# bxlab/bx-python

Measured on AMD Instinct MI355X. Metric: M overlap-queries/s at 100M x 10M intervals (count-only), higher is better.
Workload: dtype int32

## Files before the change

### bx-python_amd/csrc/count_bitmap.hpp

```cpp
#pragma once

namespace bxmi {

constexpr int BM_NB = PT_NB;
constexpr unsigned BM_REC_ESC = 0xFFFFFFFFu;
constexpr int BM_MIN_SHIFT = 5;
constexpr int BM_GROUP_TILES = 64;
constexpr int BM_CHUNK = 65536;
constexpr int BM_HARD = 127;
constexpr int BM_LONG_CAP = 480;

struct BmGeom {
    int32_t cmin;
    int32_t cmax;
    int32_t shift;
    int32_t nce;
    int32_t ncs;
    int32_t stride;
    int32_t f;
    int32_t rshift;
    int32_t dshift;
};

__device__ __forceinline__ unsigned bm_len_esc(const BmGeom &g) { return (1u << (32 - g.rshift)) - 1u; }
// ... 69 lines not shown
    if ((int)threadIdx.x < npar) {
        po.segs[threadIdx.x] = c.seg[threadIdx.x];
        po.totals[threadIdx.x] = c.total[threadIdx.x];
    }
    for (int i = 0; i < npar; i++)
        for (int64_t t = c.seg[i].tile0 + threadIdx.x; t < c.seg[i].tile_end; t += T) po.tile_seg[t] = (unsigned short)i;
}

__global__ __launch_bounds__(256) void bm_params_kernel(BmSegChunk c, int first, BmSeg *__restrict__ segs, unsigned long long **__restrict__ totals,
                                                        unsigned short *__restrict__ tile_seg, unsigned long long *__restrict__ zero_u64, int n_zero,
                                                        int *__restrict__ n_items, unsigned *__restrict__ probe = nullptr,
                                                        unsigned long long *__restrict__ order_host = nullptr, unsigned long long order_seq = 0)
{
    if (first == 0 && blockIdx.x == 0) {
        for (int i = threadIdx.x; i < n_zero; i += 256) zero_u64[i] = 0ull;
        if (threadIdx.x == 0) *n_items = 0;
        if (probe) {
            const bool d = bm_probe_descent(c.seg[0].qs, c.seg[0].nq);
            if (threadIdx.x == 0) {
                if (d) *probe = 1u;
                if (order_host) *order_host = (order_seq << 1) | (d ? 1ull : 0ull);
            }
        }
    }
    const BmSeg &sg = c.seg[blockIdx.x];
    const int id = first + (int)blockIdx.x;
    if (threadIdx.x == 0) {
        segs[id] = sg;
        totals[id] = c.total[blockIdx.x];
    }
    for (int64_t t = sg.tile0 + threadIdx.x; t < sg.tile_end; t += 256) tile_seg[t] = (unsigned short)id;
}

struct OpMin {
    template <typename T>
    __device__ __forceinline__ T operator()(T a, T b) const
    {
        return a < b ? a : b;
    }
};

__device__ __forceinline__ int bm_rank_lt64(const int32_t *__restrict__ a, int n, long long x)
{
    int l = 0, h = n;
    while (l < h) {
        int mid = (int)(((unsigned)l + (unsigned)h) >> 1);
        if ((long long)a[mid] < x)
            l = mid + 1;
        else
            h = mid;
    }
    return l;
}

struct BmBounds {
    unsigned *bounds;
    int cmin, ulog, units;
};
__device__ __forceinline__ int bm_bounds_upto(const BmBounds &B, int x)
{
    if (x < B.cmin) return 0;
    const unsigned u = (((unsigned)x - (unsigned)B.cmin) >> B.ulog) + 1u;
    return u < (unsigned)(B.units + 1) ? (int)u : B.units + 1;
}

constexpr int BM_CHECK_CH = 256 * 16;
template <bool BOUNDS>
__device__ __forceinline__ bool bm_check_chunk(const int32_t *__restrict__ qs, int64_t nq, int64_t c, const BmBounds &B)
{
    const int64_t base = c * BM_CHECK_CH + 16 * (int64_t)threadIdx.x;
    bool descent = false;
    if (base + 17 <= nq) {
        const int4 *p = reinterpret_cast<const int4 *>(qs + base);
        const int4 a = p[0], b = p[1], d = p[2], e = p[3];
        const int nxt = qs[base + 16];
        descent = a.x > a.y || a.y > a.z || a.z > a.w || a.w > b.x || b.x > b.y || b.y > b.z || b.z > b.w || b.w > d.x || d.x > d.y ||
                  d.y > d.z || d.z > d.w || d.w > e.x || e.x > e.y || e.y > e.z || e.z > e.w || e.w > nxt;
        if (BOUNDS && !descent && bm_bounds_upto(B, a.x) != bm_bounds_upto(B, nxt)) {
            const int v[17] = {a.x, a.y, a.z, a.w, b.x, b.y, b.z, b.w, d.x, d.y, d.z, d.w, e.x, e.y, e.z, e.w, nxt};
#pragma unroll
            for (int i = 0; i < 16; i++)
                for (int u = bm_bounds_upto(B, v[i]); u < bm_bounds_upto(B, v[i + 1]); u++) B.bounds[u] = (unsigned)(base + i + 1);
        }
    } else {
        for (int64_t i = base; i + 1 < nq && i < base + 16; i++) {
            descent |= qs[i] > qs[i + 1];
            if (BOUNDS && qs[i] <= qs[i + 1])
                for (int u = bm_bounds_upto(B, qs[i]); u < bm_bounds_upto(B, qs[i + 1]); u++) B.bounds[u] = (unsigned)(i + 1);
        }
    }
    return descent;
}

__device__ __forceinline__ void bm_bounds_outer(const int32_t *__restrict__ qs, int64_t nq, const BmBounds &B)
{
    const int first = bm_bounds_upto(B, qs[0]), last = bm_bounds_upto(B, qs[nq - 1]);
    for (int u = 0; u < first; u++) B.bounds[u] = 0u;
    for (int u = last; u <= B.units; u++) B.bounds[u] = (unsigned)nq;
}

template <bool BOUNDS>
__global__ __launch_bounds__(256) void bm_sorted_check_kernel(const int32_t *__restrict__ qs, int64_t nq, unsigned *__restrict__ unsorted, BmBounds B)
{
    if (BOUNDS && blockIdx.x == 0 && threadIdx.x == 0) bm_bounds_outer(qs, nq, B);
    for (int64_t c = blockIdx.x; c * BM_CHECK_CH < nq; c += gridDim.x) {
        if (__hip_atomic_load(unsorted, __ATOMIC_RELAXED, __HIP_MEMORY_SCOPE_WORKGROUP) != 0) return;
        const bool descent = bm_check_chunk<BOUNDS>(qs, nq, c, B);
        if (__syncthreads_or(descent)) {
            if (threadIdx.x == 0) __hip_atomic_store(unsorted, 1u, __ATOMIC_RELAXED, __HIP_MEMORY_SCOPE_WORKGROUP);
            return;
        }
    }
}

__device__ __forceinline__ unsigned bm_bucket_of(int qs, const BmGeom &g)
{
    if (qs < g.cmin) return 0;
    const unsigned b = ((unsigned)qs - (unsigned)g.cmin) >> g.shift;
    return b < (unsigned)(BM_NB - 1) ? b : (unsigned)(BM_NB - 1);
}

template <int SUB>
__device__ __forceinline__ unsigned bm_sort_key_of(int qs, const BmGeom &g)
{
    if (SUB == 1) return bm_bucket_of(qs, g);
    if (qs < g.cmin) return 0;
    const unsigned b = ((unsigned)qs - (unsigned)g.cmin) >> (g.shift - 1);
    return b < (unsigned)(2 * BM_NB - 1) ? b : (unsigned)(2 * BM_NB - 1);
}

__device__ __forceinline__ unsigned bm_record_of(int qs, int qe, const BmGeom &g)
{
    const unsigned rel = (unsigned)qs - (unsigned)g.cmin;
    const unsigned len = (unsigned)qe - (unsigned)qs;
    const bool ok = qs >= g.cmin && (rel >> g.shift) < (unsigned)BM_NB && qe > qs && len < bm_len_esc(g);
    return ok ? ((rel & ((1u << (g.shift + g.f)) - 1u)) | (len << g.rshift)) : BM_REC_ESC;
}

constexpr int BM_PAD_ROOM = 4096 + 544;
#ifndef BM_TS_EXP
#define BM_TS_EXP 0
#endif

template <int THREADS, int ITEMS, bool PAD = false, int SUB = 1, bool TOT = false>
__global__ __launch_bounds__(THREADS) void bm_tile_sort_kernel(const BmSeg *__restrict__ segs, const unsigned short *__restrict__ tile_seg,
                                                               unsigned *__restrict__ recs ,
                                                               unsigned short *__restrict__ slots ,
                                                               unsigned short *__restrict__ tbl ,
                                                               const unsigned *__restrict__ gate ,
                                                               unsigned *__restrict__ tend ,
                                                               unsigned short *__restrict__ tbl2 ,
                                                               const BmSegChunk par, const int npar , const BmParOut po,
                                                               unsigned *__restrict__ tesc = nullptr )
{
    constexpr int TILE = THREADS * ITEMS;
    if (gate && *gate == 0) return;
    static_assert(!TOT || (PAD && SUB == 1), "total-only batches: the persistent walk on padded runs");
    constexpr int NBK = BM_NB * SUB;
    constexpr int BPT = NBK / THREADS;
    static_assert(NBK % THREADS == 0 && (BPT == 2 || BPT == 4), "2 or 4 buckets per thread");
    static_assert(SUB == 1 || (SUB == 2 && !PAD && BPT == 4), "half buckets: packed runs, 1024-thread shapes");
    constexpr int STAGED = PAD ? TILE + 3 * THREADS : TILE;
    constexpr int STRIDE = PAD ? TILE + BM_PAD_ROOM : TILE;
    extern __shared__ __attribute__((aligned(16))) int32_t dyn[];
    unsigned *staged = reinterpret_cast<unsigned *>(dyn);
    unsigned *cnt = staged + STAGED;
    unsigned short *toff = reinterpret_cast<unsigned short *>(cnt + NBK);
    unsigned *scan_tmp = reinterpret_cast<unsigned *>(toff + NBK);
    const int64_t tile = blockIdx.x;
    BmGeom g;
    const int32_t BX_GLOBAL *__restrict__ qs, *__restrict__ qe;
    int64_t nq, ltile, ntiles_seg;
    if (npar) {
        if (blockIdx.x == 0) bm_write_params(par, npar, po);
        int i = 0;
        while (i + 1 < npar && tile >= par.seg[i].tile_end) i++;
        g = par.seg[i].g;
        ltile = tile - par.seg[i].tile0, ntiles_seg = par.seg[i].ntiles;
        qs = as_global(par.seg[i].qs) + ltile * TILE, qe = as_global(par.seg[i].qe) + ltile * TILE;
        nq = par.seg[i].nq - ltile * TILE;
    } else {
        const BmSeg &sg = segs[tile_seg[tile]];
        g = sg.g;
        ltile = tile - sg.tile0, ntiles_seg = sg.ntiles;
        qs = as_global(sg.qs) + ltile * TILE, qe = as_global(sg.qe) + ltile * TILE;
        nq = sg.nq - ltile * TILE;
    }
    if (ltile >= ntiles_seg) return;
    recs += tile * STRIDE, slots += tile * TILE;
    const int64_t base = 0;
    const int n = (int)(nq < TILE ? nq : TILE);
    int n_out = n;
    for (int i = threadIdx.x; i < NBK; i += THREADS) cnt[i] = 0;
    __syncthreads();
    unsigned br[ITEMS];
    int4 vs[ITEMS / 4], ve[ITEMS / 4];
    if (n == TILE) {
#pragma unroll
        for (int j = 0; j < ITEMS / 4; j++) vs[j] = load_int4(qs + base + 4 * (j * THREADS + (int)threadIdx.x));
#pragma unroll
        for (int j = 0; j < ITEMS / 4; j++) ve[j] = load_int4(qe + base + 4 * (j * THREADS + (int)threadIdx.x));
#pragma unroll
        for (int j = 0; j < ITEMS / 4; j++) {
            const unsigned bx = bm_sort_key_of<SUB>(vs[j].x, g), by = bm_sort_key_of<SUB>(vs[j].y, g), bz = bm_sort_key_of<SUB>(vs[j].z, g),
                           bw = bm_sort_key_of<SUB>(vs[j].w, g);
            const unsigned b0 = (unsigned)__builtin_amdgcn_readfirstlane((int)bx);
            if (__all(bx == b0 && by == b0 && bz == b0 && bw == b0)) {
                unsigned r0 = 0;
                if (lane_id() == 0) r0 = atomicAdd(&cnt[b0], 256u);
                r0 = (unsigned)__builtin_amdgcn_readfirstlane((int)r0) + 4u * (unsigned)lane_id();
                br[4 * j + 0] = (b0 << 16) | (r0 + 0);
                br[4 * j + 1] = (b0 << 16) | (r0 + 1);
                br[4 * j + 2] = (b0 << 16) | (r0 + 2);
                br[4 * j + 3] = (b0 << 16) | (r0 + 3);
            } else {
                if (BM_TS_EXP == 1) {
                    const unsigned fake = 4u * (unsigned)(j * THREADS + (int)threadIdx.x);
                    br[4 * j + 0] = (bx << 16) | (fake + 0u), br[4 * j + 1] = (by << 16) | (fake + 1u);
                    br[4 * j + 2] = (bz << 16) | (fake + 2u), br[4 * j + 3] = (bw << 16) | (fake + 3u);
                } else {
                br[4 * j + 0] = (bx << 16) | atomicAdd(&cnt[bx], 1u);
                br[4 * j + 1] = (by << 16) | atomicAdd(&cnt[by], 1u);
                br[4 * j + 2] = (bz << 16) | atomicAdd(&cnt[bz], 1u);
                br[4 * j + 3] = (bw << 16) | atomicAdd(&cnt[bw], 1u);
                }
            }
        }
    } else {
#pragma unroll
        for (int j = 0; j < ITEMS; j++) {
            const int k = j * THREADS + threadIdx.x;
            if (k < n) {
                const unsigned b = bm_sort_key_of<SUB>(qs[base + k], g);
                br[j] = (b << 16) | atomicAdd(&cnt[b], 1u);
            }
        }
    }
    __syncthreads();
    {
        unsigned c[BPT], sum = 0;
#pragma unroll
        for (int u = 0; u < BPT; u++) {
            c[u] = cnt[BPT * threadIdx.x + u];
            sum += c[u];
        }
        unsigned tot;
        unsigned exc;
        if (PAD) {
            const int lane = lane_id();
            const int lanes = (1 << g.f) / BPT;
            unsigned usum = sum;
            for (int d = 1; d < lanes; d <<= 1) usum += (unsigned)__shfl_xor((int)usum, d, 64);
            const unsigned padded = (usum + 3u) & ~3u;
            const bool leader = (lane & (lanes - 1)) == 0;
            const unsigned before = block_exclusive_scan(leader ? padded : 0u, OpSum(), 0u, scan_tmp, &tot);
            const unsigned ubase = (unsigned)__shfl((int)before, lane & ~(lanes - 1), 64);
            unsigned inc = sum;
            for (int d = 1; d < lanes; d <<= 1) {
                const unsigned up = (unsigned)__shfl_up((int)inc, d, 64);
                if ((lane & (lanes - 1)) >= d) inc += up;
            }
            exc = ubase + inc - sum;
            if (leader)
                for (unsigned k = usum; k < padded; k++) staged[ubase + k] = BM_REC_ESC;
            n_out = BM_TS_EXP == 1 ? n : (int)tot;
            if (threadIdx.x == 0) tend[tile] = tot;
        } else {
            exc = block_exclusive_scan(sum, OpSum(), 0u, scan_tmp, &tot);
        }
        unsigned short o[BPT];
#pragma unroll
        for (int u = 0; u < BPT; u++) {
            o[u] = (unsigned short)exc;
            toff[BPT * threadIdx.x + u] = o[u];
            exc += c[u];
        }
        if (SUB == 2) {
            *reinterpret_cast<unsigned *>(tbl + tile * BM_NB + 2 * threadIdx.x) = (unsigned)o[0] | ((unsigned)o[2 % BPT] << 16);
            *reinterpret_cast<uint2 *>(tbl2 + tile * NBK + BPT * threadIdx.x) =
                make_uint2((unsigned)o[0] | ((unsigned)o[1] << 16), (unsigned)o[2 % BPT] | ((unsigned)o[BPT - 1] << 16));
        } else {
        unsigned short *row = tbl + tile * BM_NB + BPT * threadIdx.x;
        if (BPT == 4)
            *reinterpret_cast<uint2 *>(row) = make_uint2((unsigned)o[0] | ((unsigned)o[1] << 16), (unsigned)o[2] | ((unsigned)o[BPT - 1] << 16));
        else
            *reinterpret_cast<unsigned *>(row) = (unsigned)o[0] | ((unsigned)o[1] << 16);
        }
    }
    __syncthreads();
    bool esc = false;
    if (n == TILE) {
        uint2 *l4 = reinterpret_cast<uint2 *>(slots + base);
#pragma unroll
        for (int j = 0; j < ITEMS / 4; j++) {
            const unsigned s0 = toff[br[4 * j + 0] >> 16] + (br[4 * j + 0] & 0xffffu), s1 = toff[br[4 * j + 1] >> 16] + (br[4 * j + 1] & 0xffffu);
            const unsigned s2 = toff[br[4 * j + 2] >> 16] + (br[4 * j + 2] & 0xffffu), s3 = toff[br[4 * j + 3] >> 16] + (br[4 * j + 3] & 0xffffu);
            if (BM_TS_EXP == 3) {
                if ((s0 ^ s1 ^ s2 ^ s3 ^ (unsigned)vs[j].x ^ (unsigned)ve[j].y) == 0x9e3779b9u) staged[0] = s0;
                continue;
            }
            const unsigned r0 = bm_record_of(vs[j].x, ve[j].x, g), r1 = bm_record_of(vs[j].y, ve[j].y, g);
            const unsigned r2 = bm_record_of(vs[j].z, ve[j].z, g), r3 = bm_record_of(vs[j].w, ve[j].w, g);
            staged[s0] = r0, staged[s1] = r1, staged[s2] = r2, staged[s3] = r3;
            if (TOT)
                esc |= r0 == BM_REC_ESC || r1 == BM_REC_ESC || r2 == BM_REC_ESC || r3 == BM_REC_ESC;
            else
                l4[j * THREADS + threadIdx.x] = make_uint2(s0 | (s1 << 16), s2 | (s3 << 16));
        }
    } else {
#pragma unroll
        for (int j = 0; j < ITEMS; j++) {
            const int k = j * THREADS + threadIdx.x;
            if (k < n) {
                const unsigned s = toff[br[j] >> 16] + (br[j] & 0xffffu);
                const unsigned r = bm_record_of(qs[base + k], qe[base + k], g);
                staged[s] = r;
                if (TOT)
                    esc |= r == BM_REC_ESC;
                else
                    slots[base + k] = (unsigned short)s;
            }
        }
    }
    if (TOT) {
        const int any = __syncthreads_or(esc ? 1 : 0);
        if (threadIdx.x == 0) tesc[tile] = (unsigned)(any != 0);
    } else {
        __syncthreads();
    }
    int4 *out = reinterpret_cast<int4 *>(recs + base);
    const int n4 = BM_TS_EXP == 2 ? 0 : (n_out + 3) >> 2;
    for (int i = threadIdx.x; i < n4; i += THREADS) out[i] = reinterpret_cast<const int4 *>(staged)[i];
}


template <int NBK = BM_NB>
__global__ __launch_bounds__(256) void bm_transpose_kernel(const unsigned short *__restrict__ tbl, const BmSeg *__restrict__ segs,
                                                           const unsigned short *__restrict__ tile_seg, int tile_log2,
                                                           unsigned *__restrict__ runT , int64_t ntp,
                                                           unsigned *__restrict__ grpcnt , const unsigned *__restrict__ gate)
{
    __shared__ unsigned short t[BM_GROUP_TILES][66];
    if (gate && *gate == 0) return;
    const int grp = blockIdx.x, b0 = blockIdx.y * 64;
    {
        const int r = threadIdx.x >> 2, q = threadIdx.x & 3;
        const int64_t tile = (int64_t)grp * BM_GROUP_TILES + r;
        const BmSeg &sg = segs[tile_seg[tile]];
        const bool live = tile - sg.tile0 < sg.ntiles;
        const int64_t left = sg.nq - ((tile - sg.tile0) << tile_log2);
        const unsigned ntile = !live ? 0u : (left < ((int64_t)1 << tile_log2) ? (unsigned)left : 1u << tile_log2);
        const unsigned short *row = tbl + tile * NBK + b0 + 16 * q;
        uint4 a = make_uint4(0, 0, 0, 0), c = a;
        if (live) {
            a = *reinterpret_cast<const uint4 *>(row);
            c = *reinterpret_cast<const uint4 *>(row + 8);
        }
        const unsigned w[8] = {a.x, a.y, a.z, a.w, c.x, c.y, c.z, c.w};
#pragma unroll
        for (int i = 0; i < 8; i++) {
            t[r][16 * q + 2 * i] = (unsigned short)(w[i] & 0xffffu);
            t[r][16 * q + 2 * i + 1] = (unsigned short)(w[i] >> 16);
        }
        if (q == 3) t[r][64] = (unsigned short)(b0 + 64 < NBK ? (live ? row[16] : 0) : ntile);
    }
    __syncthreads();
    {
        const int c = threadIdx.x >> 2, q = threadIdx.x & 3;
        unsigned *dst = runT + (int64_t)(b0 + c) * ntp + (int64_t)grp * BM_GROUP_TILES + 16 * q;
        unsigned sum = 0;
        unsigned v[16];
#pragma unroll
        for (int i = 0; i < 16; i++) {
            const unsigned off = t[16 * q + i][c], len = (unsigned)(unsigned short)(t[16 * q + i][c + 1] - t[16 * q + i][c]);
            v[i] = off | (len << 16);
            sum += len;
        }
#pragma unroll
        for (int i = 0; i < 4; i++) reinterpret_cast<uint4 *>(dst)[i] = make_uint4(v[4 * i], v[4 * i + 1], v[4 * i + 2], v[4 * i + 3]);
        sum += __shfl_xor(sum, 1, 64);
        sum += __shfl_xor(sum, 2, 64);
        if (q == 0 && grpcnt) grpcnt[(int64_t)grp * NBK + b0 + c] = sum;
    }
}

constexpr int BM_PLAN_BATCH = 16;
template <bool EMIT, int UNITS>
__device__ __forceinline__ void bm_plan_walk(const unsigned *__restrict__ grpcnt, int ngroups, const BmSeg *__restrict__ segs,
                                             const unsigned short *__restrict__ tile_seg, int b0, int chunk, int (&cnt)[2], int4 *__restrict__ items,
                                             int out0, int out1)
{
    unsigned acc[2] = {0, 0};
    int g_first[2] = {0, 0};
    int out[2] = {out0, out1};
    int seg = tile_seg[0];
    int64_t t_last = EMIT ? segs[seg].tile0 + segs[seg].ntiles : 0;
    cnt[0] = cnt[1] = 0;
    auto close = [&](int u, int g_end) {
        if (EMIT) {
            const int64_t t_end = (int64_t)g_end * BM_GROUP_TILES;
            items[out[u]++] = make_int4((b0 + u) | (seg << 16), g_first[u] * BM_GROUP_TILES, (int)(t_end < t_last ? t_end : t_last), (int)acc[u]);
        }
        cnt[u]++;
        acc[u] = 0;
    };
    for (int g0 = 0; g0 < ngroups; g0 += BM_PLAN_BATCH) {
        uint2 v[BM_PLAN_BATCH];
        int sg[BM_PLAN_BATCH];
#pragma unroll
        for (int i = 0; i < BM_PLAN_BATCH; i++) {
            const int gi = g0 + i < ngroups ? g0 + i : ngroups - 1;
            v[i] = *reinterpret_cast<const uint2 *>(grpcnt + (int64_t)gi * BM_NB + b0);
            sg[i] = tile_seg[(int64_t)gi * BM_GROUP_TILES];
        }
#pragma unroll
        for (int i = 0; i < BM_PLAN_BATCH; i++) {
            const int gi = g0 + i;
            if (gi >= ngroups) break;
            const unsigned cc[2] = {UNITS == 1 ? v[i].x + v[i].y : v[i].x, v[i].y};
            if (sg[i] != seg) {
#pragma unroll
                for (int u = 0; u < UNITS; u++)
                    if (acc[u] > 0) close(u, gi);
                seg = sg[i];
                if (EMIT) t_last = segs[seg].tile0 + segs[seg].ntiles;
            }
#pragma unroll
            for (int u = 0; u < UNITS; u++) {
                if (acc[u] > 0 && acc[u] + cc[u] > (unsigned)chunk) close(u, gi);
                if (acc[u] == 0) g_first[u] = gi;
                acc[u] += cc[u];
            }
        }
    }
#pragma unroll
    for (int u = 0; u < UNITS; u++)
        if (acc[u] > 0) close(u, ngroups);
}

constexpr int BM_PLAN_BLOCKS = 8, BM_PLAN_THREADS = BM_NB / 2 / BM_PLAN_BLOCKS;

template <int UNITS>
__global__ __launch_bounds__(BM_PLAN_THREADS) void bm_plan_kernel(const unsigned *__restrict__ grpcnt, int ngroups, const BmSeg *__restrict__ segs,
                                                                  const unsigned short *__restrict__ tile_seg, int chunk, int4 *__restrict__ items,
                                                                  int *__restrict__ n_items, const unsigned *__restrict__ gate)
{
    __shared__ int scan_tmp[16];
    __shared__ int s_base;
    if (gate && *gate == 0) return;
    const int b0 = 2 * (int)(blockIdx.x * BM_PLAN_THREADS + threadIdx.x);
    int cnt[2], again[2];
    bm_plan_walk<false, UNITS>(grpcnt, ngroups, segs, tile_seg, b0, chunk, cnt, nullptr, 0, 0);
    int tot;
    const int at = block_exclusive_scan(cnt[0] + cnt[1], OpSum(), 0, scan_tmp, &tot);
    if (threadIdx.x == 0) s_base = atomicAdd(n_items, tot);
    __syncthreads();
    const int base = s_base;
    bm_plan_walk<true, UNITS>(grpcnt, ngroups, segs, tile_seg, b0, chunk, again, items, base + at, base + at + cnt[0]);
}

typedef __attribute__((address_space(3))) const unsigned long long *lds_cell_p;

__device__ __forceinline__ int bm_hard_rank(lds_cell_p cells, unsigned rel, const int32_t *__restrict__ a, int slice_lo, long long lo)
{
    const unsigned c = rel >> 5;
    const int r0 = slice_lo + (int)((unsigned)(cells[c] >> 32) & 0xFFFFFu), r1 = slice_lo + (int)((unsigned)(cells[c + 1] >> 32) & 0xFFFFFu);
    const long long key = lo + (long long)rel;
    if (key > INT_MAX) return r1 - slice_lo;
    return global_rank_lt(a, r0, r1, (int)key) - slice_lo;
}

typedef int bm_v4i __attribute__((ext_vector_type(4)));

template <int U>
struct BmRound {
    unsigned first[U];
    unsigned lens[U];
    unsigned rec[U];
    unsigned lf_at;
    unsigned lf_rec;
    unsigned lf_total;
    unsigned listed;
    bool lf_second;
};

__device__ __forceinline__ int bm_escape_count(const IndexDev &ix, const int32_t *__restrict__ e_sorted, const BmGeom &g, int qs, int qe)
{
    if (qs < qe && (qe <= g.cmin || qs >= g.cmax)) return 0;
    return count_one_global(ix, e_sorted, qs, qe);
}

__device__ __forceinline__ void bm_wave_rank2_lt(const int32_t *__restrict__ a, int keyA, const int32_t *__restrict__ b, int keyB, int n, int &rankA, int &rankB)
{
    const int lane = lane_id();
    int loA = 0, hiA = n, loB = 0, hiB = n;
    while (hiA - loA > 64 || hiB - loB > 64) {
        const int stepA = (hiA - loA + 64) / 65, stepB = (hiB - loB + 64) / 65;
        const long long pA = (long long)loA + (long long)(lane + 1) * stepA - 1, pB = (long long)loB + (long long)(lane + 1) * stepB - 1;
        const bool inA = hiA - loA > 64 && pA < hiA, inB = hiB - loB > 64 && pB < hiB;
        const int vA = inA ? a[pA] : INT_MAX, vB = inB ? b[pB] : INT_MAX;
        const int kA = __popcll(__ballot(inA && vA < keyA)), kB = __popcll(__ballot(inB && vB < keyB));
        if (hiA - loA > 64) {
            const long long probe_k = (long long)loA + (long long)(kA + 1) * stepA - 1;
            if (probe_k < hiA) hiA = (int)probe_k;
            loA += kA * stepA;
        }
        if (hiB - loB > 64) {
            const long long probe_k = (long long)loB + (long long)(kB + 1) * stepB - 1;
            if (probe_k < hiB) hiB = (int)probe_k;
            loB += kB * stepB;
        }
    }
    const bool ltA = loA + lane < hiA && a[loA + lane] < keyA, ltB = loB + lane < hiB && b[loB + lane] < keyB;
    rankA = loA + __popcll(__ballot(ltA)), rankB = loB + __popcll(__ballot(ltB));
}

__global__ __launch_bounds__(1024) void bm_escape_totals_kernel(const BmSeg *__restrict__ segs, const unsigned short *__restrict__ tile_seg,
                                                                const unsigned *__restrict__ tesc, int64_t ntp, int tile_log2,
                                                                unsigned long long *__restrict__ total_slots ,
                                                                const unsigned *__restrict__ gate)
{
    __shared__ long long red[1024 / 64];
    if (gate && *gate == 0) return;
    const int64_t tile = blockIdx.x;
    const int seg = tile_seg[tile];
    const BmSeg &sg = segs[seg];
    const int64_t ltile = tile - sg.tile0;
    if (ltile >= sg.ntiles || tesc[tile] == 0u) return;
    const BmGeom g = sg.g;
    const IndexDev ix = sg.ix;
    const int32_t *__restrict__ e_sorted = sg.e_sorted;
    const int64_t q0 = ltile << tile_log2;
    const int64_t left = sg.nq - q0;
    const int n = (int)(left < ((int64_t)1 << tile_log2) ? left : (int64_t)1 << tile_log2);
    long long acc = 0;
    auto one = [&](bool live, int s, int e) {
        const bool esc = live && bm_record_of(s, e, g) == BM_REC_ESC;
        const unsigned long long m = __ballot(esc);
        if (m == 0ull) return;
        if (__popcll(m) > 8 || __any(esc && s >= e)) {
            if (esc) acc += (long long)bm_escape_count(ix, e_sorted, g, s, e);
            return;
        }
        for (unsigned long long rest = m; rest; rest &= rest - 1ull) {
            const int src = __ffsll((long long)rest) - 1;
            const int S = __shfl(s, src, 64), E = __shfl(e, src, 64);
            if (E <= g.cmin || S >= g.cmax) continue;
            int rS, rE;
            bm_wave_rank2_lt(ix.s_ord, E, e_sorted, S + 1, ix.n, rS, rE);
            if (lane_id() == 0) acc += (long long)(rS - rE);
        }
    };
    const int n4 = n >> 2;
    const int4 *__restrict__ s4 = reinterpret_cast<const int4 *>(sg.qs + q0), *__restrict__ e4 = reinterpret_cast<const int4 *>(sg.qe + q0);
    for (int k0 = 0; k0 < n4; k0 += 8 * 1024) {
        int4 vs[8], ve[8];
#pragma unroll
        for (int u = 0; u < 8; u++) {
            const int k = k0 + u * 1024 + (int)threadIdx.x;
            vs[u] = s4[k < n4 ? k : 0], ve[u] = e4[k < n4 ? k : 0];
        }
#pragma unroll
        for (int u = 0; u < 8; u++) {
            const bool live = k0 + u * 1024 + (int)threadIdx.x < n4;
            one(live, vs[u].x, ve[u].x), one(live, vs[u].y, ve[u].y), one(live, vs[u].z, ve[u].z), one(live, vs[u].w, ve[u].w);
        }
    }
    for (int k0 = 4 * n4; k0 < n; k0 += 1024) {
        const int k = k0 + (int)threadIdx.x;
        const bool live = k < n;
        one(live, live ? sg.qs[q0 + k] : 0, live ? sg.qe[q0 + k] : 0);
    }
    block_accumulate_i64(acc, red, total_slots + (int64_t)seg * PT_SLOTS + (tile & (PT_SLOTS - 1)));
}

constexpr int BM_PART_Q = 1024;
template <int THREADS, int ITEMS, int FIND = 0>
__global__ __launch_bounds__(THREADS) void bm_unpermute_kernel(const unsigned *__restrict__ cnt ,
                                                               const unsigned short *__restrict__ slots, const BmSeg *__restrict__ segs,
                                                               const unsigned short *__restrict__ tile_seg,
                                                               unsigned long long *__restrict__ total_slots ,
                                                               const unsigned *__restrict__ gate, unsigned *__restrict__ loff = nullptr,
                                                               unsigned *__restrict__ svq = nullptr ,
                                                               unsigned long long *__restrict__ parts = nullptr ,
                                                               unsigned long long *__restrict__ tile_tot = nullptr )
{
    constexpr int TILE = THREADS * ITEMS;
    constexpr int PARTS = TILE / BM_PART_Q;
    static_assert(FIND < 2 || (THREADS == 1024 && TILE % BM_PART_Q == 0), "parts of 1024 queries = 256 threads' four-query groups");
    extern __shared__ __attribute__((aligned(16))) int32_t dyn[];
    if (gate && *gate == 0) return;
    unsigned *vals = reinterpret_cast<unsigned *>(dyn);
    __shared__ long long red[THREADS / 64];
    __shared__ unsigned long long s_part[FIND >= 2 ? PARTS : 1];
    if (FIND >= 2 && threadIdx.x < PARTS) s_part[threadIdx.x] = 0ull;
    const int64_t tile = blockIdx.x;
    const int seg_id = tile_seg[tile];
    const BmSeg &sg = segs[seg_id];
    const int64_t ltile = tile - sg.tile0;
    if (ltile >= sg.ntiles) return;
    const IndexDev ix = sg.ix;
    const BmGeom g = sg.g;
    const int32_t *__restrict__ e_sorted = sg.e_sorted;
    const int32_t BX_GLOBAL *__restrict__ qs_arr = as_global(sg.qs) + ltile * TILE, *__restrict__ qe_arr = as_global(sg.qe) + ltile * TILE;
    int32_t BX_GLOBAL *__restrict__ out = as_global(sg.counts) + ltile * TILE;
    cnt += tile * TILE, slots += tile * TILE;
    const int64_t nq = sg.nq - ltile * TILE;
    const int64_t base = 0;
    const int n = (int)(nq < TILE ? nq : TILE);
    {
        const int4 *src = reinterpret_cast<const int4 *>(cnt + base);
        if (n == TILE) {
            int4 v[ITEMS / 4];
#pragma unroll
            for (int j = 0; j < ITEMS / 4; j++) v[j] = src[j * THREADS + threadIdx.x];
#pragma unroll
            for (int j = 0; j < ITEMS / 4; j++) reinterpret_cast<int4 *>(vals)[j * THREADS + threadIdx.x] = v[j];
        } else {
            const int n4 = (n + 3) >> 2;
            for (int i = threadIdx.x; i < n4; i += THREADS) reinterpret_cast<int4 *>(vals)[i] = src[i];
        }
    }
    __syncthreads();
    long long acc = 0;
    if (n == TILE) {
        const uint2 *l4 = reinterpret_cast<const uint2 *>(slots + base);
        int32_t BX_GLOBAL *o4 = out + base;
// ... 123 lines not shown
```

### bx-python_amd/csrc/count_dense.hpp

```cpp
#pragma once
#include "offset_cells.hpp"

namespace bxmi {

constexpr int BD_UNIT_LOG2 = 19;
constexpr int BD_RSHIFT = 19;
constexpr int BD_MARGIN = 8192;
constexpr int BD_MAX_F = 6;
constexpr int BD_MAX_SHIFT = 19;
constexpr int BD_OV_MAX = 32704;
constexpr int BD_TABLE_FROM_FIRST = 2, BD_TABLE_FROM_LAST = 6;
constexpr int BD_THREADS = 1024;
constexpr int BD_LONG_SLOTS = 64;
constexpr int BD_LONG_CAP = 320;
constexpr int BD_HDR_QS = 6;

struct BdLayout {
    int nce, ncs;
    int bitsE, bitsS, metaE, metaS, hdr, ov, bytes;
    int ov_cap;
};

__host__ __device__ inline BdLayout bd_layout(int unit_log2)
{
    BdLayout L;
    const int UW = 1 << unit_log2;
    L.nce = (UW >> 7) + 1;
    L.ncs = ((UW + BD_MARGIN) >> 7) + 1;
    L.bitsE = 0;
    L.bitsS = L.nce * 16;
    L.metaE = L.bitsS + L.ncs * 16;
    L.metaS = L.metaE + ((L.nce * 2 + 15) & ~15);
    L.hdr = L.metaS + ((L.ncs * 2 + 15) & ~15);
    L.ov = L.hdr + 64;
    const int room = (160 * 1024 - 3072  - L.ov) / 2;
    L.ov_cap = (room < BD_OV_MAX ? room : BD_OV_MAX) & ~7;
    L.bytes = L.ov + L.ov_cap * 2;
    return L;
}

__device__ __forceinline__ int bd_lower_bound(const int32_t *__restrict__ a, int lo, int hi, int key)
{
    while (lo < hi) {
        const int mid = (int)(((unsigned)lo + (unsigned)hi) >> 1);
        if (a[mid] < key)
            lo = mid + 1;
        else
            hi = mid;
    }
    return lo;
}

__global__ __launch_bounds__(BD_THREADS) void bd_image_kernel(const int32_t *__restrict__ s_ord, const int32_t *__restrict__ e_sorted, int n,
                                                              BmGeom g, int bshift, unsigned char *__restrict__ images, unsigned *__restrict__ stats, int table_from)
{
    const int bmask = (1 << bshift) - 1;
    extern __shared__ __attribute__((aligned(16))) int32_t dyn[];
    __shared__ int s_r[2];
    __shared__ unsigned scan_tmp[16];
    const int unit = blockIdx.x;
    const int ulog = g.shift + g.f;
    const BdLayout L = bd_layout(ulog);
    const long long UW = 1ll << ulog;
    const long long lo = (long long)g.cmin + (long long)unit * UW;
    unsigned char *__restrict__ img = images + (size_t)unit * L.bytes;
    unsigned *hdr = reinterpret_cast<unsigned *>(img + L.hdr);
    unsigned short *ov = reinterpret_cast<unsigned short *>(img + L.ov);
    unsigned *bits = reinterpret_cast<unsigned *>(dyn);
    unsigned *cnt = bits + 4 * L.ncs, *ecnt = cnt + L.ncs, *ovoff = ecnt + L.ncs, *ecur = ovoff + L.ncs;
    unsigned ov_base = 3;
    unsigned worst_block = 0;
    if (threadIdx.x < 2 * BD_HDR_QS) hdr[threadIdx.x] = 0u;
    if (threadIdx.x < 3) ov[threadIdx.x] = 0;
    for (int arr = 0; arr < 2; arr++) {
        const int32_t *__restrict__ A = arr == 0 ? e_sorted : s_ord;
        const int nc = arr == 0 ? L.nce : L.ncs;
        const long long cover = arr == 0 ? UW : UW + BD_MARGIN;
        if (threadIdx.x < 2) s_r[threadIdx.x] = bm_rank_lt64(A, n, threadIdx.x == 0 ? lo : lo + cover);
        for (int c = threadIdx.x; c < nc; c += BD_THREADS) {
            bits[4 * c] = bits[4 * c + 1] = bits[4 * c + 2] = bits[4 * c + 3] = 0u;
            cnt[c] = ecnt[c] = ecur[c] = 0u;
        }
        __syncthreads();
        const int r0 = s_r[0], r1 = s_r[1];
        if (threadIdx.x == 0) hdr[arr == 0 ? 13 : 14] = (unsigned)r0;
        for (int r = r0 + (int)threadIdx.x; r < r1; r += BD_THREADS) {
            const int k = A[r];
            const unsigned rel = (unsigned)((long long)k - lo);
            const unsigned c = rel >> 7, p = rel & 127u;
            atomicAdd(&cnt[c], 1u);
            const bool first = r == r0 || A[r - 1] != k, last = r + 1 == r1 || A[r + 1] != k;
            if (first) atomicOr(&bits[4 * c + (p >> 5)], 1u << (p & 31u));
            if (last && !first) {
                const unsigned extras = (unsigned)(r - bd_lower_bound(A, r0, r, k));
                atomicAdd(&ecnt[c], (extras + 254u) / 255u);
            }
        }
        __syncthreads();
        const int K = (nc + BD_THREADS - 1) / BD_THREADS;
        const int c_lo = (int)threadIdx.x * K, c_hi = c_lo + K < nc ? c_lo + K : nc;
        auto ov_words = [table_from](unsigned entries, unsigned keys) {
            if (entries == 0u) return 0u;
            if (entries >= (unsigned)table_from) return keys < 256u ? 66u : 130u;
            return 1u + (entries > 2u ? entries : 2u);
        };
        unsigned ksum = 0, osum = 0;
        for (int c = c_lo; c < c_hi; c++) {
            ksum += cnt[c];
            osum += ov_words(ecnt[c], cnt[c]);
        }
        unsigned ktot, otot;
        unsigned kexc = block_exclusive_scan(ksum, OpSum(), 0u, scan_tmp, &ktot);
        unsigned oexc = block_exclusive_scan(osum, OpSum(), 0u, scan_tmp, &otot);
        for (int c = c_lo; c < c_hi; c++) {
            const unsigned k = cnt[c], o = ov_words(ecnt[c], cnt[c]);
            cnt[c] = kexc;
            ovoff[c] = oexc;
            kexc += k;
            oexc += o;
        }
        __syncthreads();
        unsigned short *meta = reinterpret_cast<unsigned short *>(img + (arr == 0 ? L.metaE : L.metaS));
        for (int c = threadIdx.x; c < nc; c += BD_THREADS) {
            const int blk = c >> bshift;
            const unsigned qb = cnt[blk << bshift];
            const unsigned base = cnt[c] - qb;
            if ((c & bmask) == 0) hdr[(arr == 0 ? 0 : BD_HDR_QS) + blk] = qb;
            if ((c & bmask) == bmask || c == nc - 1) {
                const unsigned in_block = base + ((c == nc - 1) ? ktot - cnt[c] : cnt[c + 1] - cnt[c]);
                worst_block = in_block > worst_block ? in_block : worst_block;
            }
            unsigned m = base & 0x7FFFu;
            if (ecnt[c]) {
                const unsigned at = ov_base + ovoff[c];
                m = 0x8000u | (at & 0x7FFFu);
                const unsigned table = ecnt[c] >= (unsigned)table_from ? 0x8000u : 0u;
                if (at < (unsigned)L.ov_cap) ov[at] = (unsigned short)((base & 0x7FFFu) | table);
                if (ecnt[c] == 1u && at + 2u < (unsigned)L.ov_cap) ov[at + 2u] = 0;
            }
            meta[c] = (unsigned short)m;
        }
        for (int c = (int)(threadIdx.x >> 7); c < nc; c += BD_THREADS >> 7) {
            if (ecnt[c] < (unsigned)table_from) continue;
            const unsigned p = threadIdx.x & 127u;
            const int k0 = r0 + (int)cnt[c], k1 = r0 + (int)(c + 1 < nc ? cnt[c + 1] : ktot);
            const long long key = lo + (long long)c * 128 + (long long)p;
            const unsigned below = (unsigned)(key > INT_MAX ? k1 - k0 : bd_lower_bound(A, k0, k1, (int)key) - k0);
            const bool wide = k1 - k0 >= 256;
            const unsigned at = ov_base + ovoff[c] + 1u;
            if (p == 0 && at < (unsigned)L.ov_cap) ov[at] = wide ? 1 : 0;
            if (wide) {
                if (at + 1u + p < (unsigned)L.ov_cap) ov[at + 1u + p] = (unsigned short)below;
            } else {
                const unsigned nb = (unsigned)__shfl_down((int)below, 1, 64);
                if ((p & 1u) == 0u && at + 1u + (p >> 1) < (unsigned)L.ov_cap) ov[at + 1u + (p >> 1)] = (unsigned short)(below | (nb << 8));
            }
        }
        for (int r = r0 + (int)threadIdx.x; r < r1; r += BD_THREADS) {
            const int k = A[r];
            const bool first = r == r0 || A[r - 1] != k, last = r + 1 == r1 || A[r + 1] != k;
            if (last && !first) {
                const unsigned rel = (unsigned)((long long)k - lo);
                const unsigned c = rel >> 7, p = rel & 127u;
                if (ecnt[c] >= (unsigned)table_from) continue;
                unsigned extras = (unsigned)(r - bd_lower_bound(A, r0, r, k));
                const unsigned ne = (extras + 254u) / 255u;
                unsigned j = atomicAdd(&ecur[c], ne);
                const unsigned at0 = ov_base + ovoff[c] + 1u;
                for (unsigned i = 0; i < ne; i++, j++) {
                    const unsigned chunk = extras < 255u ? extras : 255u;
                    extras -= chunk;
                    const unsigned more = j + 1u < ecnt[c] ? 0x8000u : 0u;
                    if (at0 + j < (unsigned)L.ov_cap) ov[at0 + j] = (unsigned short)(p | (chunk << 7) | more);
                }
            }
        }
        {
            int4 *dst = reinterpret_cast<int4 *>(img + (arr == 0 ? L.bitsE : L.bitsS));
            for (int c = threadIdx.x; c < nc; c += BD_THREADS) dst[c] = reinterpret_cast<const int4 *>(bits)[c];
        }
        ov_base += otot;
        __syncthreads();
    }
    if (threadIdx.x == 0) {
        hdr[12] = ov_base;
        hdr[15] = 0u;
        atomicMax(&stats[1], ov_base);
    }
    for (int off = 32; off > 0; off >>= 1) {
        const unsigned o = __shfl_down(worst_block, off, 64);
        worst_block = o > worst_block ? o : worst_block;
    }
    if (lane_id() == 0) atomicMax(&stats[0], worst_block);
}

constexpr int BP_UNIT_LOG2 = 18;
constexpr int BP_RSHIFT = 18;
constexpr int BP_MARGIN = 16384;

constexpr int BP_TABLES = 190;
constexpr unsigned BP_NO_TABLE = 0xFFFFFFFFu;

struct BpLayout {
    int nce, ncs;
    int cellsE, cellsS, hdr, ov, bytes;
};

__host__ __device__ inline BpLayout bp_layout(int unit_log2, int cell_log2 = 5, int bytes16 = 0)
{
    BpLayout L;
    const int UW = 1 << unit_log2;
    const int margin = cell_log2 == 5 ? BP_MARGIN : bo_margin(cell_log2);
    L.nce = (UW >> cell_log2) + 2;
    L.ncs = ((UW + margin) >> cell_log2) + 1;
    L.cellsE = 0;
    L.cellsS = L.nce * 8;
    L.hdr = (L.cellsS + L.ncs * 8 + 15) & ~15;
    L.ov = L.hdr + 16;
    L.bytes = L.ov + (cell_log2 == 5 ? BP_TABLES : BO_TABLES) * 64;
    if (bytes16 && cell_log2 != 5) L.bytes = bytes16 << 4;
    return L;
}

__global__ __launch_bounds__(BD_THREADS) void bp_image_kernel(const int32_t *__restrict__ s_ord, const int32_t *__restrict__ e_sorted, int n,
                                                              BmGeom g, unsigned char *__restrict__ images, unsigned *__restrict__ stats)
{
    extern __shared__ __attribute__((aligned(16))) int32_t dyn[];
    __shared__ int s_r[2];
    __shared__ int scan_tmp[16];
    __shared__ int s_ntab;
    if (threadIdx.x == 0) s_ntab = 0;
    const int unit = blockIdx.x;
    const int ulog = g.shift + g.f;
    const BpLayout L = bp_layout(ulog);
    const long long UW = 1ll << ulog;
    const long long lo = (long long)g.cmin + (long long)unit * UW;
    unsigned char *__restrict__ img = images + (size_t)unit * L.bytes;
    unsigned hard = 0;
    int r0s[2];
    for (int arr = 0; arr < 2; arr++) {
        const int32_t *__restrict__ A = arr == 0 ? e_sorted : s_ord;
        const int nc = arr == 0 ? L.nce : L.ncs;
        const long long span = arr == 0 ? UW + 1 : UW + BP_MARGIN;
        unsigned *bm = reinterpret_cast<unsigned *>(dyn);
        int *first = dyn + nc;
        unsigned *dmask = reinterpret_cast<unsigned *>(dyn + 2 * nc), *dcnt = reinterpret_cast<unsigned *>(dyn + 3 * nc);
        if (threadIdx.x < 2) s_r[threadIdx.x] = bm_rank_lt64(A, n, threadIdx.x == 0 ? lo : lo + span);
        __syncthreads();
        const int r0 = s_r[0], r1 = s_r[1], ns = r1 - r0;
        r0s[arr] = r0;
        for (int c = threadIdx.x; c < nc; c += BD_THREADS) {
            bm[c] = 0u;
            first[c] = ns;
            dmask[c] = 0u;
            dcnt[c] = 0u;
        }
        __syncthreads();
        for (int r = r0 + (int)threadIdx.x; r < r1; r += BD_THREADS) {
            const int k = A[r];
            const unsigned rel = (unsigned)((long long)k - lo);
            const int c = (int)(rel >> 5), p = (int)(rel & 31);
            if (r == r0 || A[r - 1] != k) {
                atomicOr(&bm[c], 1u << p);
                atomicMin(&first[c], r - r0);
            } else {
                atomicAdd(&dcnt[c], 1u);
                atomicOr(&dmask[c], 1u << p);
            }
        }
        __syncthreads();
        const int K = (nc + BD_THREADS - 1) / BD_THREADS;
        const int chunk = BD_THREADS - 1 - (int)threadIdx.x;
        const int c_lo = chunk * K < nc ? chunk * K : nc, c_hi = c_lo + K < nc ? c_lo + K : nc;
        int run = INT_MAX;
        for (int c = c_hi - 1; c >= c_lo; c--) {
            run = first[c] < run ? first[c] : run;
            first[c] = run;
        }
        int tot;
        const int above = block_exclusive_scan(run, OpMin(), INT_MAX, scan_tmp, &tot);
        uint2 *out = reinterpret_cast<uint2 *>(img + (arr == 0 ? L.cellsE : L.cellsS));
        for (int c = c_lo; c < c_hi; c++) {
            const int base = first[c] < above ? first[c] : above;
            unsigned meta = (unsigned)base & 0xFFFFFu;
            unsigned word = bm[c];
            if (dcnt[c] > 0u) {
                if (__popc(dmask[c]) == 1 && dcnt[c] < (unsigned)BM_HARD)
                    meta |= ((unsigned)(__ffs((int)dmask[c]) - 1) << 20) | (dcnt[c] << 25);
                else {
                    meta |= (unsigned)BM_HARD << 25;
                    hard++;
                    int next = c + 1 < c_hi ? (first[c + 1] < above ? first[c + 1] : above) : above;
                    next = next < ns ? next : ns;
                    word = BP_NO_TABLE;
                    if (next - base < 65536) {
                        const int slot = atomicAdd(&s_ntab, 1);
                        if (slot < BP_TABLES) {
                            word = (unsigned)(L.ov + slot * 64);
                            unsigned short *tab = reinterpret_cast<unsigned short *>(img + word);
                            const long long cell0 = lo + (long long)c * 32;
                            for (int p = 0; p < 32; p++) {
                                const long long key = cell0 + p;
                                tab[p] = (unsigned short)(key > INT_MAX ? next - base : bd_lower_bound(A, r0 + base, r0 + next, (int)key) - (r0 + base));
                            }
                        }
                    }
                }
            }
            out[c] = make_uint2(word, meta);
        }
        if (threadIdx.x == 0 && ns >= (1 << 20)) atomicAdd(&stats[1], 1u);
        __syncthreads();
    }
    if (hard) atomicAdd(&stats[0], hard);
    if (threadIdx.x == 0) {
        unsigned *hdr = reinterpret_cast<unsigned *>(img + L.hdr);
        hdr[0] = (unsigned)r0s[0], hdr[1] = (unsigned)r0s[1];
        hdr[2] = (unsigned)(unsigned long long)lo, hdr[3] = (unsigned)((unsigned long long)lo >> 32);
    }
}

constexpr unsigned BO_TABLE = 0x40000000u, BO_TABLE_WIDE = 0x80000000u;
template <bool TABLES = false>
__global__ __launch_bounds__(BD_THREADS) void bo_image_kernel(const int32_t *__restrict__ s_ord, const int32_t *__restrict__ e_sorted, int n,
                                                              BmGeom g, unsigned char *__restrict__ images, unsigned *__restrict__ stats)
{
    extern __shared__ __attribute__((aligned(16))) int32_t dyn[];
    __shared__ int s_r[2];
    __shared__ int scan_tmp[16];
    __shared__ int s_ntab;
    if (threadIdx.x == 0) s_ntab = 0;
    const int unit = blockIdx.x;
    const int k = 5 + g.dshift;
    const int ulog = g.shift + g.f;
    const BpLayout L = bp_layout(ulog, k, TABLES ? g.stride : 0);
    const long long UW = 1ll << ulog;
    const long long lo = (long long)g.cmin + (long long)unit * UW;
    unsigned char *__restrict__ img = images + (size_t)unit * L.bytes;
    unsigned hard = 0, homeless = 0;
    int r0s[2];
    for (int arr = 0; arr < 2; arr++) {
        const int32_t *__restrict__ A = arr == 0 ? e_sorted : s_ord;
        const int nc = arr == 0 ? L.nce : L.ncs;
        const long long span = arr == 0 ? UW + 1 : UW + bo_margin(k);
        unsigned *cnt = reinterpret_cast<unsigned *>(dyn);
        if (threadIdx.x < 2) s_r[threadIdx.x] = bm_rank_lt64(A, n, threadIdx.x == 0 ? lo : lo + span);
        for (int c = threadIdx.x; c < nc; c += BD_THREADS) cnt[c] = 0u;
        __syncthreads();
        const int r0 = s_r[0], r1 = s_r[1], ns = r1 - r0;
        r0s[arr] = r0;
        for (int r = r0 + (int)threadIdx.x; r < r1; r += BD_THREADS) {
            const unsigned rel = (unsigned)((long long)A[r] - lo);
            atomicAdd(&cnt[rel >> k], 1u);
        }
        __syncthreads();
        const int K = (nc + BD_THREADS - 1) / BD_THREADS;
        const int c_lo = (int)threadIdx.x * K < nc ? (int)threadIdx.x * K : nc, c_hi = c_lo + K < nc ? c_lo + K : nc;
        int sum = 0;
        for (int c = c_lo; c < c_hi; c++) sum += (int)cnt[c];
        int tot;
        int base = block_exclusive_scan(sum, OpSum(), 0, scan_tmp, &tot);
        uint2 *out = reinterpret_cast<uint2 *>(img + (arr == 0 ? L.cellsE : L.cellsS));
        for (int c = c_lo; c < c_hi; c++) {
            const int m = (int)cnt[c];
            const long long cell0 = lo + ((long long)c << k);
            const int32_t *keys = A + r0 + base;
            unsigned lo_w, hi_w;
            if (m <= BO_INLINE) {
                unsigned char offs[BO_INLINE];
#pragma unroll
                for (int i = 0; i < BO_INLINE; i++) offs[i] = i < m ? (unsigned char)((long long)keys[i] - cell0) : (unsigned char)0xFF;
                bo_pack(offs, m, (unsigned)base, lo_w, hi_w);
            } else {
                hard++;
                lo_w = BP_NO_TABLE, hi_w = ((unsigned)base & 0xFFFFFu) | BO_HARD;
                if (TABLES) {
                    const bool wide = m >= 256;
                    const int bytes = (wide ? 2 : 1) << k;
                    const int at = m <= 65535 ? atomicAdd(&s_ntab, bytes) : L.bytes;
                    if (L.ov + at + bytes <= L.bytes) {
                        lo_w = (unsigned)(L.ov + at) | BO_TABLE | (wide ? BO_TABLE_WIDE : 0u);
                        int i = 0;
                        for (int p = 0; p < (1 << k); p++) {
                            while (i < m && (long long)keys[i] - cell0 < (long long)p) i++;
                            if (wide)
                                reinterpret_cast<unsigned short *>(img + L.ov + at)[p] = (unsigned short)i;
                            else
                                img[L.ov + at + p] = (unsigned char)i;
                        }
                    } else {
                        homeless++;
                    }
                } else if (m <= BO_LIST) {
                    const int slot = atomicAdd(&s_ntab, 1);
                    if (slot < BO_TABLES) {
                        lo_w = (unsigned)(L.ov + slot * 64);
                        unsigned char *list = img + lo_w;
                        for (int i = 0; i < BO_LIST; i++) list[i] = i < m ? (unsigned char)((long long)keys[i] - cell0) : (unsigned char)0xFF;
                    }
                }
            }
            out[c] = make_uint2(lo_w, hi_w);
            base += m;
        }
        if (threadIdx.x == 0 && ns >= (1 << 20)) atomicAdd(&stats[1], 1u);
        __syncthreads();
    }
    if (hard) atomicAdd(&stats[0], hard);
    if (homeless) atomicAdd(&stats[2], homeless);
    if (threadIdx.x == 0) {
        unsigned *hdr = reinterpret_cast<unsigned *>(img + L.hdr);
        hdr[0] = (unsigned)r0s[0], hdr[1] = (unsigned)r0s[1];
        hdr[2] = (unsigned)(unsigned long long)lo, hdr[3] = (unsigned)((unsigned long long)lo >> 32);
    }
}

__global__ __launch_bounds__(256) void bd_transpose_kernel(const unsigned short *__restrict__ tbl, const BmSeg *__restrict__ segs,
                                                           const unsigned short *__restrict__ tile_seg, int tile_log2,
                                                           unsigned short *__restrict__ unitT , int64_t ntp,
                                                           unsigned *__restrict__ unitcnt , const unsigned *__restrict__ gate,
                                                           const unsigned *__restrict__ tend )
{
    __shared__ unsigned short t[BM_GROUP_TILES][66];
    if (gate && *gate == 0) return;
    const int grp = blockIdx.x, b0 = blockIdx.y * 64;
    const int f = segs[tile_seg[(int64_t)grp * BM_GROUP_TILES]].g.f;
    if (blockIdx.y == 0)
        for (int u = (BM_NB >> f) + (int)threadIdx.x; u < BM_NB; u += 256) unitcnt[(int64_t)grp * BM_NB + u] = 0u;
    {
        const int r = threadIdx.x >> 2, q = threadIdx.x & 3;
        const int64_t tile = (int64_t)grp * BM_GROUP_TILES + r;
        const BmSeg &sg = segs[tile_seg[tile]];
        const bool live = tile - sg.tile0 < sg.ntiles;
        const int64_t left = sg.nq - ((tile - sg.tile0) << tile_log2);
        unsigned ntile = !live ? 0u : (left < ((int64_t)1 << tile_log2) ? (unsigned)left : 1u << tile_log2);
        if (tend && live) ntile = tend[tile];
        const unsigned short *row = tbl + tile * BM_NB + b0 + 16 * q;
        uint4 a = make_uint4(0, 0, 0, 0), c = a;
        if (live) {
            a = *reinterpret_cast<const uint4 *>(row);
            c = *reinterpret_cast<const uint4 *>(row + 8);
        }
        const unsigned w[8] = {a.x, a.y, a.z, a.w, c.x, c.y, c.z, c.w};
#pragma unroll
        for (int i = 0; i < 8; i++) {
            t[r][16 * q + 2 * i] = (unsigned short)(w[i] & 0xffffu);
            t[r][16 * q + 2 * i + 1] = (unsigned short)(w[i] >> 16);
        }
        if (q == 3) {
            t[r][64] = (unsigned short)(b0 + 64 < BM_NB ? (live ? row[16] : 0) : ntile);
            if (b0 + 64 >= BM_NB) unitT[(int64_t)(BM_NB >> f) * ntp + tile] = (unsigned short)ntile;
        }
    }
    __syncthreads();
    {
        const int nu = 64 >> f;
        const int per_unit = 256 / nu;
        const int u = threadIdx.x / per_unit, k = threadIdx.x % per_unit;
        const int tiles_per_thread = 64 / per_unit;
        const int c0 = u << f, c1 = c0 + (1 << f);
        unsigned sum = 0;
        if (tiles_per_thread >= 1) {
            unsigned short *dst = unitT + (int64_t)((b0 >> f) + u) * ntp + (int64_t)grp * BM_GROUP_TILES + k * tiles_per_thread;
            for (int i = 0; i < tiles_per_thread; i++) {
                const int r = k * tiles_per_thread + i;
                dst[i] = t[r][c0];
                sum += (unsigned)(unsigned short)(t[r][c1] - t[r][c0]);
            }
        } else if (k < 64) {
            unitT[(int64_t)((b0 >> f) + u) * ntp + (int64_t)grp * BM_GROUP_TILES + k] = t[k][c0];
            sum = (unsigned)(unsigned short)(t[k][c1] - t[k][c0]);
        }
        __shared__ unsigned s_sum[256];
        s_sum[threadIdx.x] = sum;
        __syncthreads();
        if (k == 0) {
            unsigned tot = 0;
            for (int i = 0; i < per_unit; i++) tot += s_sum[threadIdx.x + i];
            unitcnt[(int64_t)grp * BM_NB + (b0 >> f) + u] = tot;
        }
    }
}

constexpr int BD_PLAN_SEGS = 32;
__global__ __launch_bounds__(1024) void bd_plan_kernel(const unsigned *__restrict__ unitcnt , int n_segs, const BmSeg *__restrict__ segs,
                                                       int chunk, int4 *__restrict__ items, int *__restrict__ n_items, const unsigned *__restrict__ gate)
{
    __shared__ int scan_tmp[16];
    __shared__ int s_first[BD_PLAN_SEGS + 1], s_glo[BD_PLAN_SEGS], s_ghi[BD_PLAN_SEGS], s_tlast[BD_PLAN_SEGS];
    if (gate && *gate == 0) return;
    if (threadIdx.x == 0) {
        int at = 0;
        for (int i = 0; i < n_segs; i++) {
            s_first[i] = at;
            at += segs[i].tile_end > segs[i].tile0 ? (BM_NB >> segs[i].g.f) : 0;
            s_glo[i] = (int)(segs[i].tile0 / BM_GROUP_TILES), s_ghi[i] = (int)(segs[i].tile_end / BM_GROUP_TILES);
            s_tlast[i] = (int)(segs[i].tile0 + segs[i].ntiles);
        }
        s_first[n_segs] = at;
    }
    __syncthreads();
    const int total_units = s_first[n_segs];
    int carry = 0;
    for (int j0 = 0; j0 < total_units; j0 += 1024) {
        const int j = j0 + (int)threadIdx.x;
        const bool live = j < total_units;
        int seg = 0;
        while (seg + 1 < n_segs && (live ? j : 0) >= s_first[seg + 1]) seg++;
        const int u = live ? j - s_first[seg] : 0;
        const int g_lo = s_glo[seg], ng = live ? s_ghi[seg] - g_lo : 0, t_last = s_tlast[seg];
        const unsigned *__restrict__ col = unitcnt + (int64_t)g_lo * BM_NB + u;
        int fb[6], fe[6];
        unsigned fq[6];
        int cnt = 0;
        auto walk = [&](bool emit, int at) {
            unsigned acc = 0;
            int g_first = 0, k = 0;
            auto close = [&](int g_end) {
                if (emit) {
                    const int t_end = (g_lo + g_end) * BM_GROUP_TILES;
                    items[at + k] = make_int4(u | (seg << 16), (g_lo + g_first) * BM_GROUP_TILES, t_end < t_last ? t_end : t_last, (int)acc);
                } else {
#pragma unroll
                    for (int i = 0; i < 6; i++)
                        if (k == i) fb[i] = g_first, fe[i] = g_end, fq[i] = acc;
                }
                k++;
                acc = 0;
            };
            for (int g0 = 0; g0 < ng; g0 += 16) {
                unsigned v[16];
#pragma unroll
                for (int i = 0; i < 16; i++) {
                    const int gi = g0 + i < ng ? g0 + i : ng - 1;
                    v[i] = col[(int64_t)gi * BM_NB];
                }
#pragma unroll
                for (int i = 0; i < 16; i++) {
                    const int gi = g0 + i;
                    if (gi >= ng) break;
                    const unsigned c = v[i];
                    if (acc > 0 && acc + c > (unsigned)chunk) close(gi);
                    if (acc == 0) g_first = gi;
                    acc += c;
                }
            }
            if (acc > 0) close(ng);
            return k;
        };
        cnt = walk(false, 0);
        int tot;
        const int at = carry + block_exclusive_scan(cnt, OpSum(), 0, scan_tmp, &tot);
        if (cnt <= 6) {
#pragma unroll
            for (int i = 0; i < 6; i++)
                if (i < cnt) {
                    const int t_end = (g_lo + fe[i]) * BM_GROUP_TILES;
                    items[at + i] = make_int4(u | (seg << 16), (g_lo + fb[i]) * BM_GROUP_TILES, t_end < t_last ? t_end : t_last, (int)fq[i]);
                }
        } else {
            (void)walk(true, at);
        }
        carry += tot;
    }
    if (threadIdx.x == 0) *n_items = carry;
}

typedef unsigned bd_v4u __attribute__((ext_vector_type(4)));
typedef unsigned bd_v2u __attribute__((ext_vector_type(2)));
typedef __attribute__((address_space(3))) const bd_v4u *lds_v4u_p;
typedef __attribute__((address_space(3))) const unsigned *lds_u32_p;
typedef __attribute__((address_space(3))) const unsigned char *lds_u8_p;

struct BdImage {
    lds_v4u_p bitsE, bitsS;
    lds_u16_p metaE, metaS, ov;
    lds_u32_p qbE, qbS;
    int bias;
    unsigned off_mask;
    lds_cell_p cE, cS;
    lds_u16_p img16;
    lds_u8_p img8;
    int rshift, cell_log2;
    unsigned cell_mask;
    int eLo, sLo;
    long long lo;
    const int32_t *s_ord, *e_sorted;
    SlUnit sl;
    BmGeom g;
};

__device__ __forceinline__ unsigned bp_cell_rank(lds_cell_p cells, unsigned rel, unsigned &meta_out)
{
    const unsigned long long c = cells[rel >> 5];
    const unsigned bits = (unsigned)c, meta = (unsigned)(c >> 32);
    meta_out = meta;
    const unsigned below = ~(0xFFFFFFFFu << (rel & 31u));
    const unsigned dup = __builtin_amdgcn_ubfe(below, (meta >> 20) & 31u, 1u);
    return (meta & 0xFFFFFu) + (unsigned)__popc(bits & below) + (meta >> 25) * dup;
}

__device__ __forceinline__ int bp_hard_rank(const BdImage &I, lds_cell_p cells, unsigned rel, const int32_t *__restrict__ a, int slice_lo)
{
    const bd_v2u c = __builtin_bit_cast(bd_v2u, cells[rel >> 5]);
    if (c.x != BP_NO_TABLE) return (int)(c.y & 0xFFFFFu) + (int)I.img16[(c.x >> 1) + (rel & 31u)];
    return bm_hard_rank(cells, rel, a, slice_lo, I.lo);
}

template <bool RAW = false>
__device__ __forceinline__ unsigned bp_count_record(const BdImage &I, unsigned rec)
{
    const unsigned off = rec & I.off_mask, len = rec >> BP_RSHIFT;
    const unsigned relE = off + 1u, relS = off + len;
    unsigned mE, mS;
    const unsigned rE = bp_cell_rank(I.cE, relE, mE);
    const unsigned rS = bp_cell_rank(I.cS, relS, mS);
    unsigned c = (unsigned)I.bias + (rS - rE);
    if ((mE > mS ? mE : mS) >= ((unsigned)BM_HARD << 25)) {
        int hE = (int)rE, hS = (int)rS;
        if ((mE >> 25) == (unsigned)BM_HARD) hE = bp_hard_rank(I, I.cE, relE, I.e_sorted, I.eLo);
        if ((mS >> 25) == (unsigned)BM_HARD) hS = bp_hard_rank(I, I.cS, relS, I.s_ord, I.sLo);
        c = (unsigned)(I.bias + (hS - hE));
    }
    if (RAW) return rec == BM_REC_ESC ? 0u : c;
    c = c < 0xFFFFu ? c : 0xFFFFu;
    return rec == BM_REC_ESC ? 0xFFFFu : c;
}

template <bool QB>
__device__ __forceinline__ int bd_rank(lds_v4u_p bits, lds_u16_p meta, lds_u32_p qb, lds_u16_p ov, unsigned rel)
{
    const unsigned c = rel >> 7, p = rel & 127u;
    const bd_v4u w = bits[c];
    unsigned m = meta[c];
    unsigned q = 0u;
    if (QB) q = qb[c >> 10];
    const unsigned long long lo = (unsigned long long)w.x | ((unsigned long long)w.y << 32);
    const unsigned long long hi = (unsigned long long)w.z | ((unsigned long long)w.w << 32);
    const bool up = p >= 64u;
    const unsigned long long below = (1ull << (p & 63u)) - 1ull;
    int r = __popcll((up ? hi : lo) & below) + (up ? __popcll(lo) : 0);
    if (m & 0x8000u) {
        unsigned i = m & 0x7FFFu;
        m = ov[i];
        if (m & 0x8000u) {
            m &= 0x7FFFu;
            const unsigned wide = ov[i + 1u];
            const unsigned w = ov[i + 2u + (wide ? p : p >> 1)];
            r = (int)(wide ? w : (w >> ((p & 1u) << 3)) & 255u);
        } else {
            unsigned e;
            do {
                e = ov[++i];
                r += (e & 127u) < p ? (int)((e >> 7) & 255u) : 0;
            } while (e & 0x8000u);
        }
    }
    return (int)(q + m) + r;
}

__device__ __forceinline__ unsigned bd_count16(int bias, int rS, int rE, unsigned rec)
{
    unsigned c = (unsigned)(bias + (rS - rE));
    c = c < 0xFFFFu ? c : 0xFFFFu;
    return rec == BM_REC_ESC ? 0xFFFFu : c;
}

template <int FMT, bool QB, int EXP, bool W8 = false>
__device__ __forceinline__ void bd_answer_slot(const BdImage &I, unsigned short *__restrict__ out, unsigned idx4, unsigned valid, bd_v4u v)
{
    if (valid == 0u) return;
    const unsigned rec[4] = {v.x, v.y, v.z, v.w};
    unsigned c[4];
    if (EXP == 1) {
#pragma unroll
        for (int j = 0; j < 4; j++) c[j] = rec[j] & 0xffu;
    } else if (FMT == 2) {
        sl_count_slot(I.sl, I.g, rec, c);
#pragma unroll
        for (int j = 0; j < 4; j++) c[j] = c[j] < 0xFFFFu ? c[j] : 0xFFFFu;
    } else {
#pragma unroll
        for (int j = 0; j < 4; j++) {
            const unsigned off = rec[j] & I.off_mask;
            const int rE = bd_rank<QB>(I.bitsE, I.metaE, I.qbE, I.ov, off + 1u);
            const int rS = bd_rank<QB>(I.bitsS, I.metaS, I.qbS, I.ov, off + (rec[j] >> BD_RSHIFT));
            c[j] = bd_count16(I.bias, rS, rE, rec[j]);
        }
    }
    unsigned short *p = out + 4 * (size_t)idx4;
    if (EXP == 3) {
        if ((c[0] & c[1] & c[2] & c[3]) == 0x12345u) p[0] = 1;
        return;
    }
    if (W8) {
        unsigned char *p8 = reinterpret_cast<unsigned char *>(out) + 4 * (size_t)idx4;
#pragma unroll
        for (int j = 0; j < 4; j++) c[j] = c[j] < 0xFFu ? c[j] : 0xFFu;
        if (valid == 15u) {
            *reinterpret_cast<unsigned *>(p8) = c[0] | (c[1] << 8) | (c[2] << 16) | (c[3] << 24);
        } else {
#pragma unroll
            for (int j = 0; j < 4; j++)
                if (valid & (1u << j)) p8[j] = (unsigned char)c[j];
        }
        return;
    }
    if (valid == 15u) {
        bd_v2u o;
        o.x = c[0] | (c[1] << 16), o.y = c[2] | (c[3] << 16);
        *reinterpret_cast<bd_v2u *>(p) = o;
    } else {
        if (valid & 1u) p[0] = (unsigned short)c[0];
        if (valid & 2u) p[1] = (unsigned short)c[1];
        if (valid & 4u) p[2] = (unsigned short)c[2];
        if (valid & 8u) p[3] = (unsigned short)c[3];
    }
}

__device__ __forceinline__ unsigned bd_valid_mask(unsigned f0, unsigned ra, unsigned re)
{
    const int lo = max((int)(ra - f0), 0), hi = min((int)(re - f0), 4);
    return ((1u << hi) - 1u) & ~((1u << lo) - 1u);
}

#ifndef BD_LOAD_NT
#define BD_LOAD_NT 0
#endif
__device__ __forceinline__ void bd_issue_load(bd_v4u &v, const unsigned *recs, unsigned idx4)
{
    const bd_v4u *p = reinterpret_cast<const bd_v4u *>(recs) + idx4;
#if BD_LOAD_NT == 1
    asm volatile("global_load_dwordx4 %0, %1, off nt" : "=v"(v) : "v"(p) : "memory");
#elif BD_LOAD_NT == 2
    asm volatile("global_load_dwordx4 %0, %1, off sc1 nt" : "=v"(v) : "v"(p) : "memory");
#elif BD_LOAD_NT == 3
    asm volatile("global_load_dwordx4 %0, %1, off sc0 sc1" : "=v"(v) : "v"(p) : "memory");
#else
    asm volatile("global_load_dwordx4 %0, %1, off" : "=v"(v) : "v"(p) : "memory");
#endif
}

template <int K>
__device__ __forceinline__ void bd_wait(bd_v4u &v)
{
    asm volatile("s_waitcnt vmcnt(%1) ; ring %0" : "+v"(v) : "n"(K) : "memory");
}

__device__ __forceinline__ void bd_dummy_store(unsigned short *slot)
{
    asm volatile("global_store_dword %0, %1, off" : : "v"(slot), "v"(0u) : "memory");
}

template <int FMT, bool QB, int EXP = 0, int DEPTH = 2, bool PIPE = false, bool PAD = false, bool W8 = false>
__global__ __launch_bounds__(BD_THREADS) void bd_search_kernel(const BmSeg *__restrict__ segs, const int4 *__restrict__ items,
                                                               const int *__restrict__ n_items, const unsigned short *__restrict__ unitT, int64_t ntp,
                                                               const unsigned *__restrict__ recs ,
                                                               unsigned short *__restrict__ out , int tile_log2,
                                                               const unsigned *__restrict__ gate)
{
    if (gate && *gate == 0) return;
    extern __shared__ __attribute__((aligned(16))) int32_t dyn[];
    __shared__ uint2 s_long[BD_LONG_CAP];
    __shared__ int s_nlong, s_next;
    __shared__ int s_tmp[20];
    const int nit = *n_items;
    const int per_xcd = (nit + 7) >> 3;
    const int slot = (int)(blockIdx.x >> 3);
    const int it = (int)(blockIdx.x & 7) * per_xcd + slot;
    if (slot >= per_xcd || it >= nit) return;
    const int4 item = items[it];
    const int unit = item.x & 0xffff, t0 = item.y, t1 = item.z;
    const BmSeg &sg = segs[item.x >> 16];
    const BmGeom g = sg.g;
    const BdLayout L = bd_layout(g.shift + g.f);
    const int image_bytes = L.bytes;
    const unsigned short *__restrict__ runs0 = unitT + (int64_t)unit * ntp;
    const unsigned short *__restrict__ runs1 = runs0 + ntp;
    const int lane = lane_id();
    const unsigned tile_slots = ((1u << tile_log2) + (PAD ? (unsigned)BM_PAD_ROOM : 0u)) >> 2;
    int B = 64;
    while (B > 8 && (t1 - t0) < 2 * (BD_THREADS / 64) * B) B >>= 1;
    if (threadIdx.x == 0) s_nlong = 0, s_next = B * (BD_THREADS / 64);
    int tb = t0 + B * (int)(threadIdx.x >> 6);
    unsigned a_nx, e_nx;
    auto load_runs = [&](int tbase) {
        const int t = tbase + lane;
        const int tc = t < t1 && lane < B ? t : t0;
        const unsigned a = runs0[tc];
        const unsigned e = runs1[tc];
        a_nx = t < t1 && lane < B ? a : 0u;
        e_nx = t < t1 && lane < B ? e : 0u;
    };
    load_runs(tb);
    BdImage I;
    if (FMT == 2) {
        I.sl = sl_stage_unit(sg, unit, dyn, s_tmp);
        I.g = g;
    } else {
        const bm_v4i BX_GLOBAL *src = reinterpret_cast<const bm_v4i BX_GLOBAL *>(as_global(sg.dimages) + (size_t)unit * image_bytes);
        const int n4 = L.ov >> 4;
        constexpr int SWEEPS = 5;
        for (int i0 = 0; i0 < n4; i0 += SWEEPS * BD_THREADS) {
            bm_v4i v[SWEEPS];
#pragma unroll
            for (int k = 0; k < SWEEPS; k++) {
                const int i = i0 + k * BD_THREADS + (int)threadIdx.x;
                v[k] = __builtin_nontemporal_load(src + (i < n4 ? i : n4 - 1));
            }
#pragma unroll
            for (int k = 0; k < SWEEPS; k++) {
                const int i = i0 + k * BD_THREADS + (int)threadIdx.x;
                if (i < n4) reinterpret_cast<bm_v4i *>(dyn)[i] = v[k];
            }
        }
    }
    __syncthreads();
    if (FMT == 0) {
        const bm_v4i BX_GLOBAL *src = reinterpret_cast<const bm_v4i BX_GLOBAL *>(as_global(sg.dimages) + (size_t)unit * image_bytes + L.ov);
        const int used = (int)reinterpret_cast<const unsigned *>(reinterpret_cast<unsigned char *>(dyn) + L.hdr)[12];
        const int n4 = (used * 2 + 15) >> 4;
        for (int i = threadIdx.x; i < n4; i += BD_THREADS) reinterpret_cast<bm_v4i *>(reinterpret_cast<unsigned char *>(dyn) + L.ov)[i] = __builtin_nontemporal_load(src + i);
        __syncthreads();
    }
    if (FMT == 2) {
    } else {
        unsigned char *base = reinterpret_cast<unsigned char *>(dyn);
        I.bitsE = (lds_v4u_p) reinterpret_cast<bd_v4u *>(base + L.bitsE);
        I.bitsS = (lds_v4u_p) reinterpret_cast<bd_v4u *>(base + L.bitsS);
        I.metaE = (lds_u16_p) reinterpret_cast<unsigned short *>(base + L.metaE);
        I.metaS = (lds_u16_p) reinterpret_cast<unsigned short *>(base + L.metaS);
        I.ov = (lds_u16_p) reinterpret_cast<unsigned short *>(base + L.ov);
        I.qbE = (lds_u32_p) reinterpret_cast<unsigned *>(base + L.hdr);
        I.qbS = I.qbE + BD_HDR_QS;
        const unsigned *hdr = reinterpret_cast<const unsigned *>(base + L.hdr);
        I.bias = (int)hdr[14] - (int)hdr[13];
        I.off_mask = (1u << (g.shift + g.f)) - 1u;
    }
    while (tb < t1) {
        const int t = tb + lane;
        const unsigned a = a_nx, e = e_nx;
        int tn = 0;
        if (lane == 0) tn = atomicAdd(&s_next, B);
        tn = t0 + __builtin_amdgcn_readfirstlane(tn);
        load_runs(tn);
        unsigned n4 = e > a ? ((e + 3u) >> 2) - (a >> 2) : 0u;
        if (n4 > (unsigned)BD_LONG_SLOTS) {
            const int k = atomicAdd(&s_nlong, 1);
            if (k < BD_LONG_CAP) {
                s_long[k] = make_uint2(((unsigned)t * tile_slots << 2) + a, e - a);
                n4 = 0u;
            }
        }
        const unsigned incl = wave_inclusive_scan(n4, OpSum());
        const unsigned total = (unsigned)__builtin_amdgcn_readlane((int)incl, 63);
        const unsigned delta = ((unsigned)t * tile_slots + (a >> 2)) - (incl - n4);
        const unsigned ae = a | (e << 15);
        bd_v4u ring_v[DEPTH];
        unsigned ring_idx[DEPTH], ring_valid[DEPTH];
        auto prep = [&](unsigned s0, unsigned &idx4, unsigned &valid, bd_v4u &v, bool by_hand = false) {
            unsigned at = 0u, ok = 0u;
            if (!PAD || s0 < total) {
                const unsigned s = s0 + (unsigned)lane;
                int k = (int)__popcll(__ballot(incl <= s0));
                unsigned r = (unsigned)k;
                for (; k < 63; k++) {
                    const unsigned c = (unsigned)__builtin_amdgcn_readlane((int)incl, k);
                    if (c > s0 + 63u) break;
                    r += s >= c ? 1u : 0u;
                }
                r = r < 63u ? r : 63u;
                const unsigned d = (unsigned)__shfl((int)delta, (int)r, 64), x = (unsigned)__shfl((int)ae, (int)r, 64);
                const bool active = s < total;
                at = active ? d + s : 0u;
                if (PAD)
                    ok = active ? 15u : 0u;
                else
                    ok = active ? bd_valid_mask((at & ((1u << (tile_log2 - 2)) - 1u)) << 2, x & 0x7fffu, x >> 15) : 0u;
            }
            idx4 = at, valid = ok;
            if (EXP == 3) {
                const unsigned h = idx4 * 2654435761u;
                v = bd_v4u{(h & 0x3ffffu) | (500u << 18), ((h >> 3) & 0x3ffffu) | (100u << 18), ((h >> 7) & 0x3ffffu) | (900u << 18),
                           ((h >> 11) & 0x3ffffu) | (300u << 18)};
            } else if (by_hand)
                bd_issue_load(v, recs, idx4);
            else
                v = reinterpret_cast<const bd_v4u *>(recs)[idx4];
        };
        if (PIPE && PAD) {
            unsigned short *nobody = W8 ? reinterpret_cast<unsigned short *>(reinterpret_cast<unsigned char *>(out) + (((size_t)tb + 1) * tile_slots << 2) - 4)
                                        : out + (((size_t)tb + 1) * tile_slots << 2) - 2;
#pragma unroll
            for (int d = 0; d < DEPTH; d++) {
                if (d > 0) bd_dummy_store(nobody);
                prep(64u * d, ring_idx[d], ring_valid[d], ring_v[d], true);
            }
            for (unsigned s0 = 0; s0 < total; s0 += 64u * DEPTH) {
#pragma unroll
                for (int d = 0; d < DEPTH; d++) {
                    bd_wait<2 * DEPTH - 2>(ring_v[d]);
                    if (s0 + 64u * d < total)
                        bd_answer_slot<FMT, QB, EXP, W8>(I, out, ring_idx[d], ring_valid[d], ring_v[d]);
                    else
                        bd_dummy_store(nobody);
                    prep(s0 + 64u * (d + DEPTH), ring_idx[d], ring_valid[d], ring_v[d], true);
                }
            }
#pragma unroll
            for (int d = 0; d < DEPTH; d++) bd_wait<0>(ring_v[d]);
        } else if (PIPE) {
            bd_v4u y_v[DEPTH];
            unsigned y_idx[DEPTH], y_valid[DEPTH];
#pragma unroll
            for (int d = 0; d < DEPTH; d++) prep(64u * d, ring_idx[d], ring_valid[d], ring_v[d], true);
            for (unsigned s0 = 0; s0 < total; s0 += 128u * DEPTH) {
#pragma unroll
                for (int d = 0; d < DEPTH; d++) prep(s0 + 64u * (DEPTH + d), y_idx[d], y_valid[d], y_v[d], true);
                if (DEPTH > 0) { bd_wait<2 * DEPTH - 1>(ring_v[0]); bd_answer_slot<FMT, QB, EXP, W8>(I, out, ring_idx[0], ring_valid[0], ring_v[0]); }
                if (DEPTH > 1) { bd_wait<2 * DEPTH - 2>(ring_v[1 % DEPTH]); bd_answer_slot<FMT, QB, EXP, W8>(I, out, ring_idx[1 % DEPTH], ring_valid[1 % DEPTH], ring_v[1 % DEPTH]); }
                if (DEPTH > 2) { bd_wait<2 * DEPTH - 3>(ring_v[2 % DEPTH]); bd_answer_slot<FMT, QB, EXP, W8>(I, out, ring_idx[2 % DEPTH], ring_valid[2 % DEPTH], ring_v[2 % DEPTH]); }
                if (DEPTH > 3) { bd_wait<2 * DEPTH - 4>(ring_v[3 % DEPTH]); bd_answer_slot<FMT, QB, EXP, W8>(I, out, ring_idx[3 % DEPTH], ring_valid[3 % DEPTH], ring_v[3 % DEPTH]); }
#pragma unroll
                for (int d = 0; d < DEPTH; d++) prep(s0 + 64u * (2 * DEPTH + d), ring_idx[d], ring_valid[d], ring_v[d], true);
                if (DEPTH > 0) { bd_wait<2 * DEPTH - 1>(y_v[0]); bd_answer_slot<FMT, QB, EXP, W8>(I, out, y_idx[0], y_valid[0], y_v[0]); }
                if (DEPTH > 1) { bd_wait<2 * DEPTH - 2>(y_v[1 % DEPTH]); bd_answer_slot<FMT, QB, EXP, W8>(I, out, y_idx[1 % DEPTH], y_valid[1 % DEPTH], y_v[1 % DEPTH]); }
                if (DEPTH > 2) { bd_wait<2 * DEPTH - 3>(y_v[2 % DEPTH]); bd_answer_slot<FMT, QB, EXP, W8>(I, out, y_idx[2 % DEPTH], y_valid[2 % DEPTH], y_v[2 % DEPTH]); }
                if (DEPTH > 3) { bd_wait<2 * DEPTH - 4>(y_v[3 % DEPTH]); bd_answer_slot<FMT, QB, EXP, W8>(I, out, y_idx[3 % DEPTH], y_valid[3 % DEPTH], y_v[3 % DEPTH]); }
            }
#pragma unroll
            for (int d = 0; d < DEPTH; d++) bd_wait<0>(ring_v[d]);
        } else
        for (unsigned s0 = 0; s0 < total; s0 += 64u * DEPTH) {
#pragma unroll
            for (int d = 0; d < DEPTH; d++) prep(s0 + 64u * d, ring_idx[d], ring_valid[d], ring_v[d]);
#pragma unroll
            for (int d = 0; d < DEPTH; d++) bd_answer_slot<FMT, QB, EXP, W8>(I, out, ring_idx[d], ring_valid[d], ring_v[d]);
        }
        tb = tn;
    }
    __syncthreads();
    {
        const int nl = s_nlong < BD_LONG_CAP ? s_nlong : BD_LONG_CAP;
        for (int k = 0; k < nl; k++) {
            const uint2 lr = s_long[k];
            const unsigned first = lr.x, end = lr.x + lr.y;
            const unsigned q0 = first >> 2, nq4 = ((end + 3u) >> 2) - q0;
            for (unsigned q = threadIdx.x; q < nq4; q += BD_THREADS) {
                const unsigned idx4 = q0 + q;
                bd_answer_slot<FMT, QB, EXP, W8>(I, out, idx4, bd_valid_mask(4u * idx4, first, end), reinterpret_cast<const bd_v4u *>(recs)[idx4]);
            }
        }
    }
}

constexpr int BW_MASK_WORDS = 128;
constexpr int BW_PF = 9;
constexpr unsigned BW_IDLE = 0xFFFFFFFFu;
#ifndef BW_EXP
#define BW_EXP 0
#endif
#ifndef BW_B
#define BW_B 64
#endif
#ifndef BS_UNROLL
#define BS_UNROLL 1
#endif

__device__ __forceinline__ unsigned bw_wave_inclusive_sum(unsigned v)
{
    v += (unsigned)__builtin_amdgcn_update_dpp(0, (int)v, 0x111, 0xf, 0xf, false);
    v += (unsigned)__builtin_amdgcn_update_dpp(0, (int)v, 0x112, 0xf, 0xf, false);
    v += (unsigned)__builtin_amdgcn_update_dpp(0, (int)v, 0x114, 0xf, 0xf, false);
    v += (unsigned)__builtin_amdgcn_update_dpp(0, (int)v, 0x118, 0xf, 0xf, false);
    v += (unsigned)__builtin_amdgcn_update_dpp(0, (int)v, 0x142, 0xa, 0xf, false);
    v += (unsigned)__builtin_amdgcn_update_dpp(0, (int)v, 0x143, 0xc, 0xf, false);
    return v;
}

template <bool RAW = false>
__device__ __forceinline__ void bp_count_slot(const BdImage &I, bd_v4u v, unsigned (&c)[4])
{
    const unsigned rec[4] = {v.x, v.y, v.z, v.w};
    unsigned relE[4], relS[4];
    unsigned long long cellE[4], cellS[4];
#pragma unroll
    for (int j = 0; j < 4; j++) {
        const unsigned off = rec[j] & I.off_mask;
        relE[j] = off + 1u, relS[j] = off + (rec[j] >> BP_RSHIFT);
        cellE[j] = I.cE[relE[j] >> 5];
        cellS[j] = I.cS[relS[j] >> 5];
    }
    unsigned worst = 0u;
#pragma unroll
    for (int j = 0; j < 4; j++) {
        const bd_v2u ce = __builtin_bit_cast(bd_v2u, cellE[j]), cs = __builtin_bit_cast(bd_v2u, cellS[j]);
        const unsigned bE = ce.x, mE = ce.y, bS = cs.x, mS = cs.y;
        const unsigned geE = 0xFFFFFFFFu << (relE[j] & 31u), geS = 0xFFFFFFFFu << (relS[j] & 31u);
        const unsigned rE = (mE & 0xFFFFFu) + (unsigned)__popc(bE & ~geE) + (mE >> 25) * __builtin_amdgcn_ubfe(~geE, (mE >> 20) & 31u, 1u);
        const unsigned rS = (mS & 0xFFFFFu) + (unsigned)__popc(bS & ~geS) + (mS >> 25) * __builtin_amdgcn_ubfe(~geS, (mS >> 20) & 31u, 1u);
        c[j] = (unsigned)I.bias + (rS - rE);
        const unsigned m = mE > mS ? mE : mS;
        worst = worst > m ? worst : m;
    }
    if (worst >= ((unsigned)BM_HARD << 25)) {
#pragma unroll
        for (int j = 0; j < 4; j++) {
            const unsigned mE = __builtin_bit_cast(bd_v2u, cellE[j]).y, mS = __builtin_bit_cast(bd_v2u, cellS[j]).y;
            if ((mE > mS ? mE : mS) >= ((unsigned)BM_HARD << 25)) c[j] = bp_count_record<RAW>(I, rec[j]);
        }
    }
#pragma unroll
    for (int j = 0; j < 4; j++) {
        if (RAW) {
            c[j] = rec[j] == BM_REC_ESC ? 0u : c[j];
        } else {
            c[j] = c[j] < 0xFFFFu ? c[j] : 0xFFFFu;
            c[j] = rec[j] == BM_REC_ESC ? 0xFFFFu : c[j];
        }
    }
}

__device__ __forceinline__ int bo_hard_rank(const BdImage &I, lds_cell_p cells, unsigned rel, const int32_t *__restrict__ a, int slice_lo)
{
    const unsigned ci = rel >> I.cell_log2, p = rel & I.cell_mask;
    const bd_v2u c = __builtin_bit_cast(bd_v2u, cells[ci]);
    const unsigned base = c.y & 0xFFFFFu, next = (unsigned)(cells[ci + 1u] >> 32) & 0xFFFFFu;
    if (c.x != BP_NO_TABLE && (c.x & BO_TABLE)) {
        const unsigned at = c.x & 0x3FFFFFFFu;
        return (int)(base + ((c.x & BO_TABLE_WIDE) ? (unsigned)I.img16[(at >> 1) + p] : (unsigned)I.img8[at + p]));
    }
    if (c.x != BP_NO_TABLE) {
        unsigned r = base;
        for (unsigned i = 0; i < next - base; i++) r += (unsigned)I.img8[c.x + i] < p ? 1u : 0u;
        return (int)r;
    }
    const long long key = I.lo + (long long)rel;
    if (key > INT_MAX) return (int)next;
    return global_rank_lt(a, slice_lo + (int)base, slice_lo + (int)next, (int)key) - slice_lo;
}

template <bool RAW = false>
__device__ __forceinline__ unsigned bo_count_record(const BdImage &I, unsigned rec)
{
    const unsigned off = rec & I.off_mask, len = rec >> I.rshift;
    const unsigned relE = off + 1u, relS = off + len;
    const bd_v2u ce = __builtin_bit_cast(bd_v2u, I.cE[relE >> I.cell_log2]), cs = __builtin_bit_cast(bd_v2u, I.cS[relS >> I.cell_log2]);
    const int rE = ce.y >= BO_HARD ? bo_hard_rank(I, I.cE, relE, I.e_sorted, I.eLo) : (int)bo_rank(ce.x, ce.y, relE & I.cell_mask);
    const int rS = cs.y >= BO_HARD ? bo_hard_rank(I, I.cS, relS, I.s_ord, I.sLo) : (int)bo_rank(cs.x, cs.y, relS & I.cell_mask);
    unsigned c = (unsigned)(I.bias + (rS - rE));
    if (RAW) return rec == BM_REC_ESC ? 0u : c;
    c = c < 0xFFFFu ? c : 0xFFFFu;
    return rec == BM_REC_ESC ? 0xFFFFu : c;
}

template <bool RAW = false>
__device__ __forceinline__ void bo_count_slot_lists(const BdImage &I, bd_v4u v, unsigned (&c)[4])
{
    const unsigned rec[4] = {v.x, v.y, v.z, v.w};
    unsigned relE[4], relS[4];
    unsigned long long cellE[4], cellS[4];
#pragma unroll
    for (int j = 0; j < 4; j++) {
        const unsigned off = rec[j] & I.off_mask;
        relE[j] = off + 1u, relS[j] = off + (rec[j] >> I.rshift);
        cellE[j] = I.cE[relE[j] >> I.cell_log2];
        cellS[j] = I.cS[relS[j] >> I.cell_log2];
    }
    unsigned worst = 0u;
#pragma unroll
    for (int j = 0; j < 4; j++) {
        const bd_v2u ce = __builtin_bit_cast(bd_v2u, cellE[j]), cs = __builtin_bit_cast(bd_v2u, cellS[j]);
        const unsigned rE = bo_rank(ce.x, ce.y, relE[j] & I.cell_mask), rS = bo_rank(cs.x, cs.y, relS[j] & I.cell_mask);
        c[j] = (unsigned)I.bias + (rS - rE);
        const unsigned m = ce.y > cs.y ? ce.y : cs.y;
        worst = worst > m ? worst : m;
    }
    if (worst >= BO_HARD) {
#pragma unroll
        for (int j = 0; j < 4; j++) {
            const unsigned mE = __builtin_bit_cast(bd_v2u, cellE[j]).y, mS = __builtin_bit_cast(bd_v2u, cellS[j]).y;
            if ((mE > mS ? mE : mS) >= BO_HARD) c[j] = bo_count_record<RAW>(I, rec[j]);
        }
    }
#pragma unroll
    for (int j = 0; j < 4; j++) {
        if (RAW) {
            c[j] = rec[j] == BM_REC_ESC ? 0u : c[j];
        } else {
            c[j] = c[j] < 0xFFFFu ? c[j] : 0xFFFFu;
            c[j] = rec[j] == BM_REC_ESC ? 0xFFFFu : c[j];
        }
    }
}

template <bool RAW = false, bool TAB = false>
__device__ __forceinline__ void bo_count_slot(const BdImage &I, bd_v4u v, unsigned (&c)[4])
{
    if (!TAB) {
        bo_count_slot_lists<RAW>(I, v, c);
        return;
    }
    const unsigned rec[4] = {v.x, v.y, v.z, v.w};
    unsigned relE[4], relS[4];
    unsigned long long cellE[4], cellS[4];
#pragma unroll
    for (int j = 0; j < 4; j++) {
        const unsigned off = rec[j] & I.off_mask;
        relE[j] = off + 1u, relS[j] = off + (rec[j] >> I.rshift);
        cellE[j] = I.cE[relE[j] >> I.cell_log2];
        cellS[j] = I.cS[relS[j] >> I.cell_log2];
    }
    auto rank_of = [&](bd_v2u cell, unsigned p, bool &slow) -> unsigned {
        unsigned r = bo_rank(cell.x, cell.y, p);
        const bool hard = cell.y >= BO_HARD;
        const bool tab = hard && cell.x != BP_NO_TABLE && (cell.x & BO_TABLE) != 0u;
        if (tab) {
            const unsigned at = cell.x & 0x3FFFFFFFu;
            r = (cell.y & 0xFFFFFu) + ((cell.x & BO_TABLE_WIDE) ? (unsigned)I.img16[(at >> 1) + p] : (unsigned)I.img8[at + p]);
        }
        slow |= hard && !tab;
        return r;
    };
    bool any_slow = false;
    bool slow[4];
#pragma unroll
    for (int j = 0; j < 4; j++) {
        const bd_v2u ce = __builtin_bit_cast(bd_v2u, cellE[j]), cs = __builtin_bit_cast(bd_v2u, cellS[j]);
        slow[j] = false;
        const unsigned rE = rank_of(ce, relE[j] & I.cell_mask, slow[j]), rS = rank_of(cs, relS[j] & I.cell_mask, slow[j]);
        c[j] = (unsigned)I.bias + (rS - rE);
        any_slow |= slow[j];
    }
    if (any_slow) {
#pragma unroll
        for (int j = 0; j < 4; j++)
            if (slow[j]) c[j] = bo_count_record<true>(I, rec[j]);
    }
#pragma unroll
    for (int j = 0; j < 4; j++) {
        if (RAW) {
            c[j] = rec[j] == BM_REC_ESC ? 0u : c[j];
        } else {
            c[j] = c[j] < 0xFFFFu ? c[j] : 0xFFFFu;
            c[j] = rec[j] == BM_REC_ESC ? 0xFFFFu : c[j];
        }
    }
}

template <bool W8>
__device__ __forceinline__ void bw_store_slot(unsigned short *__restrict__ out, unsigned idx4, const unsigned (&c)[4])
{
    if (W8) {
        unsigned b[4];
#pragma unroll
        for (int j = 0; j < 4; j++) b[j] = c[j] < 0xFFu ? c[j] : 0xFFu;
        reinterpret_cast<unsigned *>(out)[idx4] = b[0] | (b[1] << 8) | (b[2] << 16) | (b[3] << 24);
    } else {
        bd_v2u o;
        o.x = c[0] | (c[1] << 16), o.y = c[2] | (c[3] << 16);
        reinterpret_cast<bd_v2u *>(out)[idx4] = o;
    }
}

template <bool W8, int DEPTH, bool WIDE = false, int THREADS = BD_THREADS, bool TOT = false>
__global__ __launch_bounds__(THREADS) void bw_search_kernel(const BmSeg *__restrict__ segs, const int4 *__restrict__ items,
                                                               const int *__restrict__ n_items, const unsigned short *__restrict__ unitT, int64_t ntp,
                                                               const unsigned *__restrict__ recs ,
                                                               unsigned short *__restrict__ out , int tile_log2,
                                                               const unsigned *__restrict__ gate, unsigned *__restrict__ xcd_next ,
                                                               unsigned long long *__restrict__ total_slots = nullptr )
{
    if (gate && *gate == 0) return;
    extern __shared__ __attribute__((aligned(16))) int32_t dyn[];
    __shared__ long long s_red[TOT ? THREADS / 64 : 1];
    unsigned long long acc = 0ull;
    int acc_seg = -1;
    constexpr int LONG_CAP = THREADS == BD_THREADS ? BD_LONG_CAP : BD_LONG_CAP / 2;
    constexpr int PF = THREADS == BD_THREADS ? BW_PF : 10;
    __shared__ uint2 s_long[LONG_CAP];
    __shared__ int s_nlong, s_next, s_item_next;
    __shared__ __attribute__((aligned(8))) unsigned s_mask[THREADS / 64][BW_MASK_WORDS];
    const int nit = *n_items;
    const int per_xcd = (nit + 7) >> 3;
    const int xcd = (int)(blockIdx.x & 7);
    const int it_lo = xcd * per_xcd, it_hi = it_lo + per_xcd < nit ? it_lo + per_xcd : nit;
    const int lane = lane_id(), wave = __builtin_amdgcn_readfirstlane((int)(threadIdx.x >> 6));
    unsigned *const wmask = s_mask[wave];
    wmask[lane] = 0u, wmask[64 + lane] = 0u;
    if (threadIdx.x == 0) s_item_next = it_lo + (int)atomicAdd(&xcd_next[xcd], 1u);
    __syncthreads();
    int it = __builtin_amdgcn_readfirstlane(s_item_next);
    __syncthreads();
    const unsigned tile_slots = ((1u << tile_log2) + (unsigned)BM_PAD_ROOM) >> 2;
    while (it < it_hi) {
        const int4 item = items[it];
        const int unit = item.x & 0xffff, t0 = item.y, t1 = item.z;
        const BmSeg &sg = segs[item.x >> 16];
        if (TOT && (item.x >> 16) != acc_seg) {
            if (acc_seg >= 0) {
                block_accumulate_i64((long long)acc, s_red, total_slots + (int64_t)acc_seg * PT_SLOTS + (blockIdx.x & (PT_SLOTS - 1)));
                __syncthreads();
            }
            acc = 0ull, acc_seg = item.x >> 16;
        }
        const BmGeom g = sg.g;
        const int cell_log2 = WIDE ? 5 + g.dshift : 5;
        const BpLayout LP = bp_layout(g.shift + g.f, cell_log2, WIDE ? g.stride : 0);
        const unsigned short *__restrict__ runs0 = unitT + (int64_t)unit * ntp;
        const unsigned short *__restrict__ runs1 = runs0 + ntp;
        int B = BW_B;
        while (B > 8 && (t1 - t0) < 2 * (THREADS / 64) * B) B >>= 1;
        if (WIDE) {
            const int mean4 = item.w / (t1 - t0) / 4 + 2;
            while (B > 8 && B * (mean4 + (mean4 >> 1)) > BW_MASK_WORDS * 32) B >>= 1;
        }
        const unsigned long_slots = WIDE ? (unsigned)(BW_MASK_WORDS * 32 / B) : (unsigned)BD_LONG_SLOTS;
        if (threadIdx.x == 0) {
            s_nlong = 0, s_next = B * (THREADS / 64);
            s_item_next = it_lo + (int)atomicAdd(&xcd_next[xcd], 1u);
        }
        unsigned a_nx = 0u, e_nx = 0u;
        bool nx_in = false;
        auto load_runs = [&](int tbase) {
            const int t = tbase + lane;
            nx_in = t < t1 && lane < B;
            const int tc = nx_in ? t : t0;
            asm volatile("global_load_ushort %0, %1, off" : "=v"(a_nx) : "v"(runs0 + tc) : "memory");
            asm volatile("global_load_ushort %0, %1, off" : "=v"(e_nx) : "v"(runs1 + tc) : "memory");
        };
        int tb_next = t0 + B * wave;
        load_runs(tb_next);
        {
            const bm_v4i BX_GLOBAL *src = reinterpret_cast<const bm_v4i BX_GLOBAL *>(as_global(sg.pimages) + (size_t)unit * LP.bytes);
            const int n4 = LP.bytes >> 4;
            bm_v4i v[PF];
#pragma unroll
            for (int k = 0; k < PF; k++) {
                const int i = k * THREADS + (int)threadIdx.x;
                v[k] = __builtin_nontemporal_load(src + (i < n4 ? i : n4 - 1));
            }
#pragma unroll
            for (int k = 0; k < PF; k++) {
                const int i = k * THREADS + (int)threadIdx.x;
                if (i < n4) reinterpret_cast<bm_v4i *>(dyn)[i] = v[k];
            }
        }
        __syncthreads();
        const int it_nx = __builtin_amdgcn_readfirstlane(s_item_next);
        BdImage I;
        {
            unsigned char *base = reinterpret_cast<unsigned char *>(dyn);
            I.img16 = (lds_u16_p) reinterpret_cast<unsigned short *>(base);
            I.cE = (lds_cell_p) reinterpret_cast<unsigned long long *>(base + LP.cellsE);
            I.cS = (lds_cell_p) reinterpret_cast<unsigned long long *>(base + LP.cellsS);
            const unsigned *hdr = reinterpret_cast<const unsigned *>(base + LP.hdr);
            I.eLo = (int)hdr[0], I.sLo = (int)hdr[1];
            I.bias = I.sLo - I.eLo;
            I.lo = (long long)((unsigned long long)hdr[2] | ((unsigned long long)hdr[3] << 32));
            I.s_ord = sg.ix.s_ord, I.e_sorted = sg.e_sorted;
            I.off_mask = (1u << (g.shift + g.f)) - 1u;
            I.img8 = (lds_u8_p)base;
            I.rshift = g.rshift, I.cell_log2 = cell_log2, I.cell_mask = (1u << cell_log2) - 1u;
        }
        unsigned *const nobody = reinterpret_cast<unsigned *>(reinterpret_cast<unsigned char *>(out) +
                                                              (((size_t)(t0 + (unit * 7 + wave * 64) % (t1 - t0)) + 1) * tile_slots - 1) * (W8 ? 4 : 8));
        unsigned total = 0u, s0 = 0u;
        unsigned delta_c = 0u;
        unsigned win_lo = 0u, win_hi = 0u, win_before = 0u;
        bool live = true;
        auto advance = [&]() -> bool {
            while (tb_next < t1) {
                const int t = tb_next + lane;
                if (((total + 63u) >> 6) < (unsigned)(DEPTH - 1)) asm volatile("s_waitcnt vmcnt(0)" : : : "memory");
                asm volatile("s_waitcnt vmcnt(%2) ; runs %0 %1" : "+v"(a_nx), "+v"(e_nx) : "n"(2 * DEPTH - 2) : "memory");
                const unsigned a = nx_in ? a_nx : 0u, e = nx_in ? e_nx : 0u;
                total = 0u;
                int tn = 0;
                if (lane == 0) tn = atomicAdd(&s_next, B);
                tb_next = t0 + __builtin_amdgcn_readfirstlane(tn);
                load_runs(tb_next);
                unsigned n4 = e > a ? ((e + 3u) >> 2) - (a >> 2) : 0u;
                if (n4 > long_slots) {
                    const int k = atomicAdd(&s_nlong, 1);
                    const unsigned first = ((unsigned)t * tile_slots << 2) + a;
                    if (k < LONG_CAP) {
                        s_long[k] = make_uint2(first, e - a);
                    } else if (TOT) {
                        for (unsigned q = first >> 2; q < ((first + (e - a) + 3u) >> 2); q++) {
                            unsigned c[4];
                            if (WIDE)
                                bo_count_slot<true, THREADS == BD_THREADS>(I, reinterpret_cast<const bd_v4u *>(recs)[q], c);
                            else
                                bp_count_slot<true>(I, reinterpret_cast<const bd_v4u *>(recs)[q], c);
                            acc += (unsigned long long)c[0] + c[1] + c[2] + c[3];
                        }
                    } else {
                        const unsigned esc[4] = {0xFFFFu, 0xFFFFu, 0xFFFFu, 0xFFFFu};
                        for (unsigned q = first >> 2; q < ((first + (e - a) + 3u) >> 2); q++) bw_store_slot<W8>(out, q, esc);
                    }
                    n4 = 0u;
                }
                const unsigned incl = bw_wave_inclusive_sum(n4);
                total = (unsigned)__builtin_amdgcn_readlane((int)incl, 63);
                if (total == 0u) continue;
                const unsigned delta = ((unsigned)t * tile_slots + (a >> 2)) - (incl - n4);
                const bool ne = n4 != 0u;
                const unsigned long long bal = __ballot(ne);
                const unsigned below = __builtin_amdgcn_mbcnt_hi((unsigned)(bal >> 32), __builtin_amdgcn_mbcnt_lo((unsigned)bal, 0u));
                const unsigned dest = ne ? below : 63u - ((unsigned)lane - below);
                delta_c = (unsigned)__builtin_amdgcn_ds_permute((int)(dest << 2), (int)delta);
                if (ne) atomicOr(&wmask[(incl - 1u) >> 5], 1u << ((incl - 1u) & 31u));
                const uint2 w = reinterpret_cast<uint2 *>(wmask)[lane];
                reinterpret_cast<uint2 *>(wmask)[lane] = make_uint2(0u, 0u);
                win_lo = w.x, win_hi = w.y;
                const unsigned ends = (unsigned)__popc(w.x) + (unsigned)__popc(w.y);
                win_before = bw_wave_inclusive_sum(ends) - ends;
                s0 = 0u;
                return true;
            }
            return false;
        };
        bd_v4u ring_v[DEPTH];
        unsigned ring_idx[DEPTH];
        int inflight = 0;
        auto issue = [&](unsigned &idx4, bd_v4u &v) {
            if (live && s0 >= total) live = advance();
            unsigned at = BW_IDLE;
            if (live) {
                const int p = (int)(s0 >> 6);
                const unsigned lo = (unsigned)__builtin_amdgcn_readlane((int)win_lo, p), hi = (unsigned)__builtin_amdgcn_readlane((int)win_hi, p);
                const unsigned before = (unsigned)__builtin_amdgcn_readlane((int)win_before, p);
                const unsigned r = before + __builtin_amdgcn_mbcnt_hi(hi, __builtin_amdgcn_mbcnt_lo(lo, 0u));
                const unsigned dl = (unsigned)__builtin_amdgcn_ds_bpermute((int)(r << 2), (int)delta_c);
                const unsigned s = s0 + (unsigned)lane;
                at = s < total ? dl + s : BW_IDLE;
                s0 += 64u;
            }
            idx4 = at;
            if (live) inflight++;
            bd_issue_load(v, recs, at == BW_IDLE || (BW_EXP & 4) ? 0u : at);
        };
#pragma unroll
        for (int d = 0; d < DEPTH; d++) {
            if (d > 0) bd_dummy_store(reinterpret_cast<unsigned short *>(nobody));
            ring_idx[d] = BW_IDLE;
            bd_issue_load(ring_v[d], recs, 0u);
        }
        for (;;) {
#pragma unroll
            for (int d = 0; d < DEPTH; d++) {
                bd_wait<2 * DEPTH - 2>(ring_v[d]);
                if (__any(ring_idx[d] != BW_IDLE)) {
                    inflight--;
                    if (ring_idx[d] != BW_IDLE) {
                        unsigned c[4];
                        bd_v4u rv = ring_v[d];
                        if (BW_EXP & 4) {
                            const unsigned h = ring_idx[d] * 2654435761u;
                            rv = bd_v4u{(h & 0x3ffffu) | (500u << 18), ((h >> 3) & 0x3ffffu) | (100u << 18), ((h >> 7) & 0x3ffffu) | (900u << 18),
                                        ((h >> 11) & 0x3ffffu) | (300u << 18)};
                        }
                        if (BW_EXP & 1)
                            c[0] = rv.x & 0xffu, c[1] = rv.y & 0xffu, c[2] = rv.z & 0xffu, c[3] = rv.w & 0xffu;
                        else if (WIDE)
                            bo_count_slot<TOT, THREADS == BD_THREADS>(I, rv, c);
                        else
                            bp_count_slot<TOT>(I, rv, c);
                        if (TOT) acc += (unsigned long long)c[0] + c[1] + c[2] + c[3];
                        else if (!(BW_EXP & 2) || (c[0] & c[1] & c[2] & c[3]) == 0x12345u) bw_store_slot<W8>(out, ring_idx[d], c);
                        else bd_dummy_store(reinterpret_cast<unsigned short *>(nobody));
                    }
                    if (TOT) bd_dummy_store(reinterpret_cast<unsigned short *>(nobody));
                } else {
                    bd_dummy_store(reinterpret_cast<unsigned short *>(nobody));
                }
                issue(ring_idx[d], ring_v[d]);
            }
            if (!live && inflight == 0) break;
        }
#pragma unroll
        for (int d = 0; d < DEPTH; d++) bd_wait<0>(ring_v[d]);
        __syncthreads();
        {
            const int nl = s_nlong < LONG_CAP ? s_nlong : LONG_CAP;
            for (int k = 0; k < nl; k++) {
                const uint2 lr = s_long[k];
                const unsigned q0 = lr.x >> 2, nq4 = ((lr.x + lr.y + 3u) >> 2) - q0;
                for (unsigned q = threadIdx.x; q < nq4; q += THREADS) {
                    unsigned c[4];
                    if (WIDE)
                        bo_count_slot<TOT, THREADS == BD_THREADS>(I, reinterpret_cast<const bd_v4u *>(recs)[q0 + q], c);
                    else
                        bp_count_slot<TOT>(I, reinterpret_cast<const bd_v4u *>(recs)[q0 + q], c);
                    if (TOT) acc += (unsigned long long)c[0] + c[1] + c[2] + c[3];
                    else bw_store_slot<W8>(out, q0 + q, c);
                }
            }
        }
        __syncthreads();
        it = it_nx;
    }
    if (TOT && acc_seg >= 0) block_accumulate_i64((long long)acc, s_red, total_slots + (int64_t)acc_seg * PT_SLOTS + (blockIdx.x & (PT_SLOTS - 1)));
}

__global__ __launch_bounds__(1024) void bs_plan_kernel(const unsigned *__restrict__ bounds , int units, unsigned nq, unsigned chunk,
                                                       int4 *__restrict__ items, int *__restrict__ n_items, const unsigned *__restrict__ gate)
{
    __shared__ int scan_tmp[16];
    if (gate && *gate != 0) return;
    int carry = 0;
    for (int s0 = -1; s0 <= units; s0 += 1024) {
        const int s = s0 + (int)threadIdx.x;
        unsigned lo = 0u, hi = 0u;
        if (s <= units) {
            lo = s < 0 ? 0u : bounds[s];
            hi = s == units ? nq : bounds[s + 1];
        }
        const unsigned n = hi > lo ? hi - lo : 0u;
        const int cnt = (int)((n + chunk - 1u) / chunk);
        int tot;
        const int at = carry + block_exclusive_scan(cnt, OpSum(), 0, scan_tmp, &tot);
        for (int k = 0; k < cnt; k++) {
            const unsigned a = lo + (unsigned)k * chunk, b = a + chunk < hi ? a + chunk : hi;
            items[at + k] = make_int4(s >= 0 && s < units ? s : -1, (int)a, (int)b, 0);
        }
        carry += tot;
    }
    if (threadIdx.x == 0) *n_items = carry;
}

constexpr int BS_BOUNDS_ROW = BM_NB + 2;
__global__ __launch_bounds__(256) void bs_check_multi_kernel(const BmSeg *__restrict__ segs, const unsigned short *__restrict__ tile_seg, int64_t ntp, int tile_log2,
                                                             unsigned *__restrict__ unsorted, unsigned *__restrict__ bounds_all)
{
    for (int64_t tile = blockIdx.x; tile < ntp; tile += gridDim.x) {
        if (__hip_atomic_load(unsorted, __ATOMIC_RELAXED, __HIP_MEMORY_SCOPE_WORKGROUP) != 0) return;
        const int seg = tile_seg[tile];
        const BmSeg &sg = segs[seg];
        const int64_t ltile = tile - sg.tile0;
        if (ltile >= sg.ntiles) continue;
        BmBounds B;
        B.bounds = bounds_all + (int64_t)seg * BS_BOUNDS_ROW, B.cmin = sg.g.cmin, B.ulog = sg.g.shift + sg.g.f, B.units = BM_NB >> sg.g.f;
        if (ltile == 0 && threadIdx.x == 0) bm_bounds_outer(sg.qs, sg.nq, B);
        const int64_t c0 = (ltile << tile_log2) / BM_CHECK_CH, c1 = ((ltile + 1) << tile_log2) / BM_CHECK_CH;
        bool descent = false;
        for (int64_t c = c0; c < c1 && c * BM_CHECK_CH < sg.nq; c++) descent |= bm_check_chunk<true>(sg.qs, sg.nq, c, B);
        if (__syncthreads_or(descent)) {
            if (threadIdx.x == 0) __hip_atomic_store(unsorted, 1u, __ATOMIC_RELAXED, __HIP_MEMORY_SCOPE_WORKGROUP);
            return;
        }
    }
}

__global__ __launch_bounds__(1024) void bs_plan_multi_kernel(const BmSeg *__restrict__ segs, const unsigned *__restrict__ bounds_all, unsigned chunk,
                                                             int4 *__restrict__ items, int *__restrict__ n_items, const unsigned *__restrict__ gate)
{
    __shared__ int scan_tmp[16];
    __shared__ int s_at;
    if (gate && *gate != 0) return;
    const int seg = blockIdx.x;
    const BmSeg &sg = segs[seg];
    const int units = BM_NB >> sg.g.f;
    const unsigned nq = (unsigned)sg.nq;
    if (nq == 0u) return;
    const unsigned *bounds = bounds_all + (int64_t)seg * BS_BOUNDS_ROW;
    for (int s0 = -1; s0 <= units; s0 += 1024) {
        const int s = s0 + (int)threadIdx.x;
        unsigned lo = 0u, hi = 0u;
        if (s <= units) {
            lo = s < 0 ? 0u : bounds[s];
            hi = s == units ? nq : bounds[s + 1];
        }
        const unsigned n = hi > lo ? hi - lo : 0u;
        const int cnt = (int)((n + chunk - 1u) / chunk);
        int tot;
        const int rel = block_exclusive_scan(cnt, OpSum(), 0, scan_tmp, &tot);
        if (threadIdx.x == 0) s_at = tot ? atomicAdd(n_items, tot) : 0;
        __syncthreads();
        const int at = s_at + rel;
        for (int k = 0; k < cnt; k++) {
            const unsigned a = lo + (unsigned)k * chunk, b = a + chunk < hi ? a + chunk : hi;
            items[at + k] = make_int4(s >= 0 && s < units ? s : -1, (int)a, (int)b, seg);
        }
        __syncthreads();
    }
}

template <bool WIDE, int THREADS>
__global__ __launch_bounds__(THREADS) void bs_walk_kernel(const BmSeg *__restrict__ segs, const int4 *__restrict__ items, const int *__restrict__ n_items,
                                                          unsigned long long *__restrict__ total_slots , const unsigned *__restrict__ gate,
                                                          unsigned *__restrict__ xcd_next ,
                                                          unsigned long long *__restrict__ order_host, unsigned long long seq)
{
    if (order_host && blockIdx.x == 0 && threadIdx.x == 0) *order_host = (seq << 1) | (*gate != 0 ? 1ull : 0ull);
    if (*gate != 0) return;
    constexpr int PF = THREADS == BD_THREADS ? BW_PF : 10;
    extern __shared__ __attribute__((aligned(16))) int32_t dyn[];
    __shared__ int s_item_next;
    __shared__ long long red[THREADS / 64];
    const int nit = *n_items;
    const int per_xcd = (nit + 7) >> 3;
    const int xcd = (int)(blockIdx.x & 7);
    const int it_lo = xcd * per_xcd, it_hi = it_lo + per_xcd < nit ? it_lo + per_xcd : nit;
    long long acc = 0;
    int acc_seg = -1;
    int loaded = -1;
    if (threadIdx.x == 0) s_item_next = it_lo + (int)atomicAdd(&xcd_next[xcd], 1u);
    __syncthreads();
    int it = s_item_next;
    __syncthreads();
    while (it < it_hi) {
        const int4 item = items[it];
        const int unit = item.x;
        const int seg = item.w;
        if (seg != acc_seg) {
            if (acc_seg >= 0 && total_slots) {
                block_accumulate_i64(acc, red, total_slots + (int64_t)acc_seg * PT_SLOTS + (blockIdx.x & (PT_SLOTS - 1)));
                __syncthreads();
            }
            acc = 0, acc_seg = seg;
        }
        const BmSeg &sg = segs[seg];
        const BmGeom g = sg.g;
        const int cell_log2 = WIDE ? 5 + g.dshift : 5;
        const BpLayout LP = bp_layout(g.shift + g.f, cell_log2, WIDE ? g.stride : 0);
        if (threadIdx.x == 0) s_item_next = it_lo + (int)atomicAdd(&xcd_next[xcd], 1u);
        if (unit >= 0 && ((seg << 16) | unit) != loaded) {
            const bm_v4i BX_GLOBAL *src = reinterpret_cast<const bm_v4i BX_GLOBAL *>(as_global(sg.pimages) + (size_t)unit * LP.bytes);
            const int n4 = LP.bytes >> 4;
            bm_v4i v[PF];
#pragma unroll
            for (int k = 0; k < PF; k++) {
                const int i = k * THREADS + (int)threadIdx.x;
                v[k] = __builtin_nontemporal_load(src + (i < n4 ? i : n4 - 1));
            }
#pragma unroll
            for (int k = 0; k < PF; k++) {
                const int i = k * THREADS + (int)threadIdx.x;
                if (i < n4) reinterpret_cast<bm_v4i *>(dyn)[i] = v[k];
            }
            loaded = (seg << 16) | unit;
        }
        __syncthreads();
        const int it_nx = s_item_next;
        BdImage I;
        {
            unsigned char *base = reinterpret_cast<unsigned char *>(dyn);
            I.img16 = (lds_u16_p) reinterpret_cast<unsigned short *>(base);
            I.cE = (lds_cell_p) reinterpret_cast<unsigned long long *>(base + LP.cellsE);
            I.cS = (lds_cell_p) reinterpret_cast<unsigned long long *>(base + LP.cellsS);
            const unsigned *hdr = reinterpret_cast<const unsigned *>(base + LP.hdr);
            I.eLo = (int)hdr[0], I.sLo = (int)hdr[1];
            I.bias = I.sLo - I.eLo;
            I.lo = (long long)((unsigned long long)hdr[2] | ((unsigned long long)hdr[3] << 32));
            I.s_ord = sg.ix.s_ord, I.e_sorted = sg.e_sorted;
            I.off_mask = (1u << (g.shift + g.f)) - 1u;
            I.img8 = (lds_u8_p)base;
            I.rshift = g.rshift, I.cell_log2 = cell_log2, I.cell_mask = (1u << cell_log2) - 1u;
        }
        const int64_t lo = (unsigned)item.y, hi = (unsigned)item.z;
        const int64_t q0 = lo >> 2, q1 = (hi + 3) >> 2;
        for (int64_t qb = q0 + threadIdx.x; qb < q1; qb += (int64_t)BS_UNROLL * THREADS) {
            int s[BS_UNROLL][4], e[BS_UNROLL][4];
            bool whole[BS_UNROLL];
#pragma unroll
            for (int u = 0; u < BS_UNROLL; u++) {
                const int64_t q = qb + (int64_t)u * THREADS, k0 = 4 * q;
                whole[u] = q < q1 && k0 >= lo && k0 + 4 <= hi;
                if (whole[u]) {
                    const int4 vs = load_int4(as_global(sg.qs) + 4 * q), ve = load_int4(as_global(sg.qe) + 4 * q);
                    s[u][0] = vs.x, s[u][1] = vs.y, s[u][2] = vs.z, s[u][3] = vs.w;
                    e[u][0] = ve.x, e[u][1] = ve.y, e[u][2] = ve.z, e[u][3] = ve.w;
                } else {
#pragma unroll
                    for (int j = 0; j < 4; j++) {
                        const bool in = q < q1 && k0 + j >= lo && k0 + j < hi;
                        s[u][j] = in ? as_global(sg.qs)[k0 + j] : 0, e[u][j] = in ? as_global(sg.qe)[k0 + j] : 0;
                    }
                }
            }
#pragma unroll
            for (int u = 0; u < BS_UNROLL; u++) {
                const int64_t q = qb + (int64_t)u * THREADS, k0 = 4 * q;
                if (q >= q1) break;
                unsigned c[4];
                if (unit >= 0) {
                    bd_v4u rec;
                    rec.x = bm_record_of(s[u][0], e[u][0], g), rec.y = bm_record_of(s[u][1], e[u][1], g);
                    rec.z = bm_record_of(s[u][2], e[u][2], g), rec.w = bm_record_of(s[u][3], e[u][3], g);
                    if (WIDE)
                        bo_count_slot<false, THREADS == BD_THREADS>(I, rec, c);
                    else
                        bp_count_slot(I, rec, c);
                } else {
                    c[0] = c[1] = c[2] = c[3] = 0xFFFFu;
                }
                if (c[0] == 0xFFFFu || c[1] == 0xFFFFu || c[2] == 0xFFFFu || c[3] == 0xFFFFu || !whole[u]) {
#pragma unroll
                    for (int j = 0; j < 4; j++) {
                        const bool in = k0 + j >= lo && k0 + j < hi;
                        if (in && c[j] == 0xFFFFu) c[j] = (unsigned)bm_escape_count(sg.ix, sg.e_sorted, g, s[u][j], e[u][j]);
                        if (!in) c[j] = 0u;
                    }
                }
                if (sg.counts) {
                    if (whole[u]) {
                        store_int4(as_global(sg.counts) + 4 * q, (int)c[0], (int)c[1], (int)c[2], (int)c[3]);
                    } else {
#pragma unroll
                        for (int j = 0; j < 4; j++)
                            if (k0 + j >= lo && k0 + j < hi) as_global(sg.counts)[k0 + j] = (int)c[j];
                    }
                }
                acc += (long long)c[0] + c[1] + c[2] + c[3];
            }
        }
        __syncthreads();
        it = it_nx;
    }
    if (total_slots && acc_seg >= 0) block_accumulate_i64(acc, red, total_slots + (int64_t)acc_seg * PT_SLOTS + (blockIdx.x & (PT_SLOTS - 1)));
}

template <int THREADS, int ITEMS, bool PAD, bool W8>
__device__ __forceinline__ void bd_unpermute_tile(const unsigned short *__restrict__ cnt ,
                                                  const unsigned short *__restrict__ slots, const BmSeg *__restrict__ segs,
                                                  const unsigned short *__restrict__ tile_seg,
                                                  unsigned long long *__restrict__ total_slots ,
                                                  const unsigned *__restrict__ gate, const unsigned *__restrict__ tend,
                                                  unsigned long long *__restrict__ fb_dev ,
                                                  unsigned long long *__restrict__ fb_host )
{
    constexpr int TILE = THREADS * ITEMS;
    constexpr int STRIDE = PAD ? TILE + BM_PAD_ROOM : TILE;
    static_assert(ITEMS % 8 == 0, "whole 16-byte vectors of 16-bit counts per thread");
    extern __shared__ __attribute__((aligned(16))) int32_t dyn[];
    if (gate && *gate == 0) return;
    unsigned short *vals = reinterpret_cast<unsigned short *>(dyn);
    __shared__ long long red[THREADS / 64];
    const int64_t tile = blockIdx.x;
    const int seg_id = tile_seg[tile];
    const BmSeg &sg = segs[seg_id];
    const int64_t ltile = tile - sg.tile0;
    if (ltile >= sg.ntiles) return;
    unsigned long long *const acc_to = total_slots ? total_slots + (int64_t)seg_id * PT_SLOTS + (blockIdx.x & (PT_SLOTS - 1)) : nullptr;
    const IndexDev ix = sg.ix;
    const BmGeom g = sg.g;
    const int32_t *__restrict__ e_sorted = sg.e_sorted;
    const int32_t BX_GLOBAL *__restrict__ qs_arr = as_global(sg.qs) + ltile * TILE, *__restrict__ qe_arr = as_global(sg.qe) + ltile * TILE;
    int32_t BX_GLOBAL *__restrict__ out = as_global(sg.counts) + ltile * TILE;
    static_assert(!W8 || PAD, "8-bit counts come with the padded layout");
    const unsigned char *vals8 = reinterpret_cast<const unsigned char *>(dyn);
    cnt = W8 ? reinterpret_cast<const unsigned short *>(reinterpret_cast<const unsigned char *>(cnt) + tile * STRIDE) : cnt + tile * STRIDE;
    slots += tile * TILE;
    const int64_t nq = sg.nq - ltile * TILE;
    const int n = (int)(nq < TILE ? nq : TILE);
    constexpr unsigned ESC = W8 ? 0xFFu : 0xFFFFu;
    if (PAD) {
        const int n8 = W8 ? ((int)tend[tile] + 15) >> 4 : ((int)tend[tile] + 7) >> 3;
        const int4 *src = reinterpret_cast<const int4 *>(cnt);
        for (int i = threadIdx.x; i < n8; i += THREADS) reinterpret_cast<int4 *>(vals)[i] = src[i];
    } else {
        const int4 *src = reinterpret_cast<const int4 *>(cnt);
        if (n == TILE) {
            int4 v[ITEMS / 8];
#pragma unroll
            for (int j = 0; j < ITEMS / 8; j++) v[j] = src[j * THREADS + threadIdx.x];
#pragma unroll
            for (int j = 0; j < ITEMS / 8; j++) reinterpret_cast<int4 *>(vals)[j * THREADS + threadIdx.x] = v[j];
        } else {
            const int n8 = (n + 7) >> 3;
            for (int i = threadIdx.x; i < n8; i += THREADS) reinterpret_cast<int4 *>(vals)[i] = src[i];
        }
    }
    __syncthreads();
    long long acc = 0;
    unsigned wide = 0;
    if (PAD && W8 && !sg.counts) {
        const int n8 = ((int)tend[tile] + 15) >> 4;
        unsigned sum = 0, nff = 0;
        for (int i = threadIdx.x; i < n8; i += THREADS) {
            const int4 v = reinterpret_cast<const int4 *>(vals)[i];
            const unsigned w[4] = {(unsigned)v.x, (unsigned)v.y, (unsigned)v.z, (unsigned)v.w};
#pragma unroll
            for (int k = 0; k < 4; k++) {
                const int first = 16 * i + 4 * k, used = (int)tend[tile] - first;
                const unsigned keep = used >= 4 ? 0xFFFFFFFFu : (used <= 0 ? 0u : (1u << (8 * used)) - 1u);
                const unsigned x = w[k] & keep;
                const unsigned ff = ((x & 0x7F7F7F7Fu) + 0x01010101u) & x & 0x80808080u;
                const unsigned c = (unsigned)__popc(ff);
                nff += c;
                sum += __builtin_amdgcn_sad_u8(x, 0u, 0u) - 255u * c;
            }
        }
        __shared__ unsigned s_tot[2];
        if (threadIdx.x < 2) s_tot[threadIdx.x] = 0u;
        __syncthreads();
#pragma unroll
        for (int off = 32; off > 0; off >>= 1) {
            sum += (unsigned)__shfl_down((int)sum, off, 64);
            nff += (unsigned)__shfl_down((int)nff, off, 64);
        }
        if (lane_id() == 0) {
            atomicAdd(&s_tot[0], sum);
            atomicAdd(&s_tot[1], nff);
        }
        __syncthreads();
        if (s_tot[1] == tend[tile] - (unsigned)n) {
            if (acc_to && threadIdx.x == 0 && s_tot[0]) atomicAdd(acc_to, (unsigned long long)s_tot[0]);
            return;
        }
    }
    if (n == TILE) {
        const uint2 *l4 = reinterpret_cast<const uint2 *>(slots);
        int32_t BX_GLOBAL *o4 = out;
        uint2 sl[ITEMS / 4];
#pragma unroll
        for (int j = 0; j < ITEMS / 4; j++) sl[j] = l4[j * THREADS + threadIdx.x];
#pragma unroll
        for (int j = 0; j < ITEMS / 4; j++) {
            unsigned c[4];
            if (W8) {
                c[0] = vals8[sl[j].x & 0xffffu], c[1] = vals8[sl[j].x >> 16], c[2] = vals8[sl[j].y & 0xffffu], c[3] = vals8[sl[j].y >> 16];
            } else {
                c[0] = vals[sl[j].x & 0xffffu], c[1] = vals[sl[j].x >> 16], c[2] = vals[sl[j].y & 0xffffu], c[3] = vals[sl[j].y >> 16];
            }
            if (c[0] == ESC || c[1] == ESC || c[2] == ESC || c[3] == ESC) {
                const int64_t k0 = 4 * (int64_t)(j * THREADS + threadIdx.x);
#pragma unroll
                for (int u = 0; u < 4; u++)
                    if (c[u] == ESC) {
                        c[u] = (unsigned)bm_escape_count(ix, e_sorted, g, qs_arr[k0 + u], qe_arr[k0 + u]);
                        wide++;
                    }
            }
            if (sg.counts) store_int4(o4 + 4 * (j * THREADS + (int)threadIdx.x), (int)c[0], (int)c[1], (int)c[2], (int)c[3]);
            acc += (long long)c[0] + c[1] + c[2] + c[3];
        }
    } else {
        for (int k = threadIdx.x; k < n; k += THREADS) {
            unsigned c = W8 ? (unsigned)vals8[slots[k]] : (unsigned)vals[slots[k]];
            if (c == ESC) {
                c = (unsigned)bm_escape_count(ix, e_sorted, g, qs_arr[k], qe_arr[k]);
                wide++;
            }
            if (sg.counts) out[k] = (int)c;
            acc += c;
        }
    }
    if (acc_to) block_accumulate_i64(acc, red, acc_to);
    if (W8 && fb_dev) {
        if (__any(wide != 0u)) {
            unsigned w = wide;
#pragma unroll
            for (int off = 32; off > 0; off >>= 1) w += (unsigned)__shfl_down((int)w, off, 64);
            if (lane_id() == 0 && w) atomicAdd(fb_dev, (unsigned long long)w);
        }
        if (blockIdx.x == 0 && threadIdx.x == 0 && fb_host) *fb_host = __hip_atomic_load(fb_dev, __ATOMIC_RELAXED, __HIP_MEMORY_SCOPE_AGENT);
    }
}

template <int THREADS, int ITEMS, bool PAD = false, bool W8 = false>
__global__ __launch_bounds__(THREADS) void bd_unpermute_kernel(const unsigned short *__restrict__ cnt, const unsigned short *__restrict__ slots,
                                                               const BmSeg *__restrict__ segs, const unsigned short *__restrict__ tile_seg,
                                                               unsigned long long *__restrict__ total_slots, const unsigned *__restrict__ gate,
                                                               const unsigned *__restrict__ tend = nullptr, unsigned long long *__restrict__ fb_dev = nullptr,
                                                               unsigned long long *__restrict__ fb_host = nullptr)
{
    bd_unpermute_tile<THREADS, ITEMS, PAD, W8>(cnt, slots, segs, tile_seg, total_slots, gate, tend, fb_dev, fb_host);
}

}
```

### bx-python_amd/csrc/intervals.hip

```cpp
#include <climits>
#include <vector>
#include <algorithm>
#include <atomic>
#include <condition_variable>
#include <mutex>
#include <thread>

#include "primitives.hpp"

#include "count_direct.hpp"
#include "count_parts.hpp"
#include "count_bitmap.hpp"
#include "count_slices.hpp"
#include "find_exchange.hpp"
#include "count_dense.hpp"
#include "find_sorted.hpp"
#include "find_direct.hpp"
#include "find_neighbors.hpp"
#include "liftover.hpp"
#include "cluster.hpp"

namespace bxmi {

static int64_t g_opt_partition = -1;
// ... 254 lines not shown
    return ivl_count_part_sub(h, 0, 0, qs, qe, nq, counts, total_dev, st);
}


static int sl_ensure_eid(bxmi_ivl *h, hipStream_t st)
{
    if (h->sl_eid_ready) return BXMI_OK;
    BXMI_TRY(h->sl_eid.reserve(((size_t)h->n + SL_WALK) * sizeof(int2)));
    hipLaunchKernelGGL(sl_pack_eid_kernel, dim3((unsigned)div_up(h->n + SL_WALK, 256)), dim3(256), 0, st, h->e_ord.as<int32_t>(), h->idx.as<int32_t>(),
                       (int)h->n, h->sl_eid.as<int2>());
    BXMI_LAUNCH_CHECK();
    h->sl_eid_ready = true;
    return BXMI_OK;
}

static int ivl_find_local(bxmi_ivl *h, const int32_t *qs, const int32_t *qe, int64_t nq, int64_t *offsets, int32_t *hits, int64_t cap,
                          int64_t *total_host, hipStream_t st, const unsigned *gate = nullptr, bool *stood_down = nullptr)
{
    BXMI_TRY(h->p_lo.reserve((size_t)(nq + 4) * 4));
    BXMI_TRY(h->p_hi.reserve((size_t)(nq + 4) * 4));
    BXMI_TRY(h->q_cnt.reserve((size_t)(nq + 4) * 4));
    const bool chunk_scan = ((uintptr_t)offsets & 15) == 0;
    {
        TreeDev S = h->treeS.dev, E = h->treeE.dev;
        S.lds_from = S.nlev, S.lds_ints = 0, E.lds_from = E.nlev, E.lds_ints = 0;
        const int64_t nchunks = div_up(nq, LC_CHUNK);
        if (chunk_scan) BXMI_TRY(h->lf_state.reserve((size_t)(2 * nchunks + 4) * 8));
        hipLaunchKernelGGL(ivl_local_count_kernel, dim3((unsigned)nchunks), dim3(LC_THREADS), 0, st, S, E, index_dev(h),
                           h->e_sorted.as<int32_t>(), qs, qe, nq, h->q_cnt.as<int32_t>(), (unsigned long long *)nullptr, gate,
                           h->p_hi.as<int32_t>(), (unsigned long long *)nullptr, 0ull, chunk_scan ? h->lf_state.as<unsigned long long>() : nullptr);
        if (chunk_scan) {
            long long *chunk_base = h->lf_state.as<long long>() + nchunks;
            hipLaunchKernelGGL(fx_tile_scan_kernel, dim3(1), dim3(1024), 0, st, h->lf_state.as<unsigned long long>(), nchunks, chunk_base,
                               reinterpret_cast<long long *>(offsets) + nq, (long long *)nullptr, gate);
            hipLaunchKernelGGL(lf_offsets_kernel, dim3((unsigned)nchunks), dim3(LC_THREADS), 0, st, h->q_cnt.as<int32_t>(), chunk_base, nq,
                               reinterpret_cast<long long *>(offsets), gate);
        }
    }
    BXMI_LAUNCH_CHECK();
    if (!chunk_scan)
        BXMI_TRY((device_scan<int32_t, long long, OpSum, false>(h->q_cnt.as<int32_t>(), reinterpret_cast<long long *>(offsets), nq, 0ll,
                                                               reinterpret_cast<long long *>(offsets) + nq, h->scan_scratch, st)));
    int64_t total = 0;
    if (hits && cap > 0) {
        BXMI_TRY(sl_ensure_eid(h, st));
        BXMI_TRY(h->fx_work.reserve(128));
        hipLaunchKernelGGL(part_fill_pipe_kernel, dim3(device_props().cus * 8), dim3(FIND_THREADS), 0, st, h->sl_eid.as<int2>() + SL_WALK, qs, nq,
                           h->p_hi.as<int32_t>(), h->q_cnt.as<int32_t>(), reinterpret_cast<const long long *>(offsets), hits, (long long)cap,
                           h->fx_work.as<int32_t>() + 12, gate);
        BXMI_LAUNCH_CHECK();
    }
    unsigned gate_host = 0;
    if (gate) BXMI_HIP(hipMemcpyAsync(&gate_host, gate, sizeof(unsigned), hipMemcpyDeviceToHost, st));
    BXMI_HIP(hipMemcpyAsync(&total, offsets + nq, 8, hipMemcpyDeviceToHost, st));
    BXMI_HIP(hipStreamSynchronize(st));
    if (gate_host) {
        if (stood_down) *stood_down = true;
        return BXMI_OK;
    }
    if (total_host) *total_host = total;
    if (total > cap) return fail(BXMI_ERANGE, "bxmi_ivl_find: %lld hits need a larger buffer than cap=%lld", (long long)total, (long long)cap);
    return BXMI_OK;
}

static int ivl_find_partitioned(bxmi_ivl *h, const int32_t *qs, const int32_t *qe, int64_t nq, int64_t *offsets, int32_t *hits,
                                int64_t cap, int64_t *total_host, hipStream_t st)
{
    if (nq >= ((int64_t)1 << 31)) return fail(BXMI_EINVAL, "bxmi_ivl_find: more than 2^31 queries in one batch");
    BXMI_TRY(part_reserve(h, nq, true));
    BXMI_TRY(h->p_lo.reserve((size_t)(nq + 4) * 4));
    BXMI_TRY(h->p_hi.reserve((size_t)(nq + 4) * 4));
    BXMI_TRY(h->q_cnt.reserve((size_t)(nq + 4) * 4));
    BXMI_TRY(h->p_boffs.reserve((size_t)(nq + 4) * 8));
    PartPlan pp;
    unsigned *unsorted = reinterpret_cast<unsigned *>(h->p_slots.as<unsigned long long>() + PT_SLOTS);
    BXMI_HIP(hipMemsetAsync(unsorted, 0, sizeof(unsigned), st));
    BXMI_TRY(part_prepare(h, 0, 0, qs, qe, nq, true, st, &pp, unsorted, false));
    const int64_t ntiles = pp.ntiles;
    const unsigned tgrid = pp.tgrid;
    unsigned *table = pp.table;
    unsigned short *lpos = pp.lpos;
    const size_t lds_bytes = (size_t)PT_LDS_INTS * 4;
    BXMI_TRY(allow_big_lds(part_window_kernel, lds_bytes));
    const unsigned grid = (unsigned)(div_up(nq, PT_CHUNK) + PT_NB);
    hipLaunchKernelGGL(part_window_kernel, dim3(grid), dim3(PT_THREADS), lds_bytes, st, index_dev(h), h->slice_bounds.as<SliceBound>(), pp.plan,
                       table, pp.bq, nq, h->p_lo.as<int32_t>(), h->p_hi.as<int32_t>(), h->p_cnt.as<int32_t>());
    hipLaunchKernelGGL(part_gather_kernel<int32_t>, dim3(tgrid), dim3(PT_THREADS), 0, st, h->p_cnt.as<int32_t>(), lpos, table, ntiles, nq,
                       h->q_cnt.as<int32_t>(), (const unsigned *)nullptr, index_dev(h), (const int32_t *)nullptr, (const int32_t *)nullptr,
                       (const int32_t *)nullptr);
    BXMI_LAUNCH_CHECK();
    BXMI_TRY((device_scan<int32_t, long long, OpSum, false>(h->q_cnt.as<int32_t>(), reinterpret_cast<long long *>(offsets), nq, 0ll,
                                                           reinterpret_cast<long long *>(offsets) + nq, h->scan_scratch, st)));
    int64_t total = 0;
    BXMI_HIP(hipMemcpyAsync(&total, offsets + nq, 8, hipMemcpyDeviceToHost, st));
    BXMI_HIP(hipStreamSynchronize(st));
    if (total_host) *total_host = total;
    if (total > cap) return fail(BXMI_ERANGE, "bxmi_ivl_find: %lld hits need a larger buffer than cap=%lld", (long long)total, (long long)cap);
    if (total == 0) return BXMI_OK;
    const size_t perm_lds = (size_t)PT_TILE * 8 + (PT_NB + 2) * 2 + PT_NB * 4 + 64;
    BXMI_TRY(allow_big_lds(part_permute_i64_kernel, perm_lds));
    hipLaunchKernelGGL(part_permute_i64_kernel, dim3(tgrid), dim3(PT_THREADS), perm_lds, st, reinterpret_cast<const long long *>(offsets), lpos,
                       table, ntiles, nq, h->p_boffs.as<long long>());
    int fgrid = device_props().cus * 8;
    hipLaunchKernelGGL(part_fill_kernel, dim3(fgrid), dim3(FIND_THREADS), 0, st, index_dev(h), reinterpret_cast<const int32_t *>(pp.bq), 2, nq,
                       h->p_lo.as<int32_t>(),
                       h->p_hi.as<int32_t>(), h->p_cnt.as<int32_t>(), h->p_boffs.as<long long>(), hits);
    BXMI_LAUNCH_CHECK();
    return BXMI_OK;
}

static int bp_prepare_index(bxmi_ivl *h, hipStream_t st)
{
    h->bp_state = -1;
    h->bp_hard_cells = 0;
    const int shift = h->geom.shift;
    if (h->has_reversed || h->n < 4096 || shift > BP_UNIT_LOG2 - 1 || shift < BM_MIN_SHIFT) return BXMI_OK;
    BmGeom g;
    g.cmin = h->geom.cmin;
    g.cmax = h->cmax;
    g.shift = shift;
    const int f = BP_UNIT_LOG2 - shift;
    g.f = f > BD_MAX_F ? BD_MAX_F : f;
    g.rshift = BP_RSHIFT;
    g.dshift = 0;
    const BpLayout L = bp_layout(g.shift + g.f);
    g.nce = L.nce, g.ncs = L.ncs;
    g.stride = L.bytes >> 4;
    const int units = BM_NB >> g.f;
    BXMI_TRY(h->bp_images.reserve((size_t)units * L.bytes));
    BXMI_TRY(h->bp_stats.reserve(64));
    BXMI_HIP(hipMemsetAsync(h->bp_stats.p, 0, 64, st));
    const size_t lds = (size_t)4 * L.ncs * sizeof(int32_t);
    BXMI_TRY(allow_big_lds(bp_image_kernel, lds));
    hipLaunchKernelGGL(bp_image_kernel, dim3((unsigned)units), dim3(BD_THREADS), lds, st, h->s_ord.as<int32_t>(), h->e_sorted.as<int32_t>(), (int)h->n, g,
                       h->bp_images.as<unsigned char>(), h->bp_stats.as<unsigned>());
    BXMI_LAUNCH_CHECK();
    unsigned stats[2] = {0, 0};
    BXMI_HIP(hipMemcpyAsync(stats, h->bp_stats.p, sizeof(stats), hipMemcpyDeviceToHost, st));
    BXMI_HIP(hipStreamSynchronize(st));
    h->bp_geom = g;
    h->bp_hard_cells = stats[0];
    const int64_t cells = 2 * ((((int64_t)h->cmax - (int64_t)h->geom.cmin) >> 5) + 1);
    if (stats[1] == 0 && (int64_t)stats[0] * 1000000 <= cells * g_opt_bm_hard_ppm) h->bp_state = 1;
    return BXMI_OK;
}

static int bo_prepare_index(bxmi_ivl *h, hipStream_t st, bool clumped = false)
{
    h->bo_state = -1;
    h->bo_hard_cells = 0;
    const int shift = h->geom.shift;
    int64_t span = (int64_t)h->cmax - (int64_t)h->geom.cmin + 1;
    const int k = g_opt_bo_cell_log2 ? (int)g_opt_bo_cell_log2 : (clumped ? BO_MIN_K : bo_cell_log2_for(span, h->n));
    if (h->has_reversed || h->n < 4096 || k == 0 || shift > bo_rshift(k) - 1 || shift < BM_MIN_SHIFT) return BXMI_OK;
    BmGeom g;
    g.cmin = h->geom.cmin;
    g.cmax = h->cmax;
    g.shift = shift;
    const int f = bo_rshift(k) - shift;
    g.f = f > BD_MAX_F ? BD_MAX_F : f;
    g.rshift = bo_rshift(k);
    g.dshift = k - 5;
    const int big16 = BW_PF * BD_THREADS;
    const BpLayout L = bp_layout(g.shift + g.f, k, clumped ? big16 : 0);
    if (clumped && L.ov + 4096 > L.bytes) return BXMI_OK;
    g.nce = L.nce, g.ncs = L.ncs;
    g.stride = L.bytes >> 4;
    const int units = BM_NB >> g.f;
    BXMI_TRY(h->bo_images.reserve((size_t)units * L.bytes));
    BXMI_TRY(h->bp_stats.reserve(64));
    BXMI_HIP(hipMemsetAsync(h->bp_stats.p, 0, 64, st));
    const size_t lds = (size_t)L.ncs * sizeof(int32_t);
    if (clumped) {
        BXMI_TRY(allow_big_lds(bo_image_kernel<true>, lds));
        hipLaunchKernelGGL(bo_image_kernel<true>, dim3((unsigned)units), dim3(BD_THREADS), lds, st, h->s_ord.as<int32_t>(), h->e_sorted.as<int32_t>(), (int)h->n, g,
                           h->bo_images.as<unsigned char>(), h->bp_stats.as<unsigned>());
    } else {
        BXMI_TRY(allow_big_lds(bo_image_kernel<false>, lds));
        hipLaunchKernelGGL(bo_image_kernel<false>, dim3((unsigned)units), dim3(BD_THREADS), lds, st, h->s_ord.as<int32_t>(), h->e_sorted.as<int32_t>(), (int)h->n, g,
                           h->bo_images.as<unsigned char>(), h->bp_stats.as<unsigned>());
    }
    BXMI_LAUNCH_CHECK();
    unsigned stats[3] = {0, 0, 0};
    BXMI_HIP(hipMemcpyAsync(stats, h->bp_stats.p, sizeof(stats), hipMemcpyDeviceToHost, st));
    BXMI_HIP(hipStreamSynchronize(st));
    h->bo_geom = g;
    h->bo_hard_cells = stats[0];
    const int64_t cells = 2 * ((span >> k) + 1);
    if (clumped) {
        if (stats[1] == 0 && stats[2] == 0) h->bo_state = 2;
    } else if (stats[1] == 0 && (int64_t)stats[0] * 1000000 <= cells * g_opt_bm_hard_ppm)
        h->bo_state = 1;
    return BXMI_OK;
}

static int bd_prepare_index(bxmi_ivl *h, hipStream_t st)
{
    h->bd_state = -1;
    h->bd_worst[0] = h->bd_worst[1] = 0;
    const int shift = h->geom.shift;
    if (h->has_reversed || h->n < 4096 || shift > BD_MAX_SHIFT || shift < BM_MIN_SHIFT) return BXMI_OK;
    int tried = -1;
    for (int ulog = g_opt_bd_unit_log2 ? (int)g_opt_bd_unit_log2 : BD_UNIT_LOG2; ulog >= 18 || ulog == (int)g_opt_bd_unit_log2; ulog--) {
        BmGeom g;
        g.cmin = h->geom.cmin;
        g.cmax = h->cmax;
        g.shift = shift;
        const int f = ulog - shift;
        g.f = f < 0 ? 0 : (f > BD_MAX_F ? BD_MAX_F : f);
        if (g.shift + g.f == tried) break;
        tried = g.shift + g.f;
        g.rshift = BD_RSHIFT;
        g.dshift = 0;
        const BdLayout L = bd_layout(g.shift + g.f);
        g.nce = L.nce, g.ncs = L.ncs;
        g.stride = L.bytes >> 4;
        const int units = BM_NB >> g.f;
        BXMI_TRY(h->bd_images.reserve((size_t)units * L.bytes));
        BXMI_TRY(h->bd_stats.reserve(64));
        const size_t lds = (size_t)8 * L.ncs * sizeof(int32_t);
        BXMI_TRY(allow_big_lds(bd_image_kernel, lds));
        h->bd_geom = g;
        const int tf_first = g_opt_bd_table_from ? (int)g_opt_bd_table_from : BD_TABLE_FROM_FIRST;
        const int tf_last = g_opt_bd_table_from ? (int)g_opt_bd_table_from : BD_TABLE_FROM_LAST;
        for (int table_from = tf_first; table_from <= tf_last; table_from += BD_TABLE_FROM_LAST - BD_TABLE_FROM_FIRST)
        for (int bshift = g_opt_bd_blocks ? 10 : 13; bshift >= 10; bshift -= 3) {
            BXMI_HIP(hipMemsetAsync(h->bd_stats.p, 0, 64, st));
            hipLaunchKernelGGL(bd_image_kernel, dim3((unsigned)units), dim3(BD_THREADS), lds, st, h->s_ord.as<int32_t>(), h->e_sorted.as<int32_t>(),
                               (int)h->n, g, bshift, h->bd_images.as<unsigned char>(), h->bd_stats.as<unsigned>(), table_from);
            BXMI_LAUNCH_CHECK();
            BXMI_HIP(hipMemcpyAsync(h->bd_worst, h->bd_stats.p, sizeof(h->bd_worst), hipMemcpyDeviceToHost, st));
            BXMI_HIP(hipStreamSynchronize(st));
            h->bd_blocks = bshift == 10;
            if (h->bd_worst[1] > (unsigned)L.ov_cap) break;
            if (h->bd_worst[0] <= 32767u) {
                h->bd_state = 1;
                return BXMI_OK;
            }
        }
        if (g_opt_bd_unit_log2 || g.shift + g.f < ulog) break;
    }
    return BXMI_OK;
}

static int sl_prepare_index(bxmi_ivl *h, hipStream_t st)
{
    h->sl_state = -1;
    for (unsigned &need : h->sl_need) need = 0;
    if (h->has_reversed || h->n < 1) return BXMI_OK;
    BXMI_TRY(h->sl_meta.reserve((size_t)(BM_NB + 1) * sizeof(int4)));
    BXMI_TRY(h->sl_stats.reserve(64));
    BXMI_HIP(hipMemsetAsync(h->sl_stats.p, 0, 64, st));
    hipLaunchKernelGGL(sl_meta_kernel, dim3((BM_NB + 1 + 255) / 256), dim3(256), 0, st, h->s_ord.as<int32_t>(), h->e_sorted.as<int32_t>(), (int)h->n,
                       h->geom.cmin, h->geom.shift, h->sl_meta.as<int4>());
    hipLaunchKernelGGL(sl_fit_kernel, dim3(1), dim3(1024), 0, st, h->sl_meta.as<int4>(), h->sl_stats.as<unsigned>());
    BXMI_LAUNCH_CHECK();
    BXMI_HIP(hipMemcpyAsync(h->sl_need, h->sl_stats.p, sizeof(h->sl_need), hipMemcpyDeviceToHost, st));
    BXMI_HIP(hipStreamSynchronize(st));
    if (h->sl_need[0] <= (unsigned)SL_CAP) h->sl_state = 1;
    return BXMI_OK;
}

static BmGeom sl_geom(const bxmi_ivl *h, int64_t tile, size_t *lds_bytes, int64_t *run_len)
{
    BmGeom g;
    g.cmin = h->geom.cmin, g.cmax = h->cmax, g.shift = h->geom.shift;
    const int64_t span = (int64_t)h->cmax - (int64_t)h->geom.cmin;
    const int64_t nb_used = ((span > 0 ? span : 0) >> g.shift) + 1;
    int f = 0;
    if (g_opt_sl_f >= 0) {
        for (f = (int)g_opt_sl_f; f > 0 && h->sl_need[f] > (unsigned)SL_CAP; f--) {}
    } else {
        for (int k = 1; k <= SL_MAX_F; k++) {
            if (h->sl_need[k] > (unsigned)SL_CAP || g.shift + k > g_opt_sl_rbits || (tile << k) / nb_used > g_opt_sl_run_cap) break;
            f = k;
        }
    }
    g.f = f;
    g.rshift = g.shift + f > 17 ? g.shift + f : 17;
    const int64_t Wu = (int64_t)1 << (g.shift + f);
    int d = 0;
    while (((Wu + SL_MARGIN) >> d) + 1 > SL_DIR_CELLS) d++;
    g.dshift = d;
    g.ncs = (int32_t)((Wu + SL_MARGIN) >> d) + 1;
    g.nce = (int32_t)(Wu >> d) + 1;
    g.stride = 0;
    *lds_bytes = 2 * ((size_t)h->sl_need[f] + 16) + 2 * (size_t)((g.ncs + 2 + 7) & ~7) + 2 * (size_t)(g.nce + 2 + 8);
    *run_len = (tile << f) / nb_used;
    return g;
}

struct BmLaunch {
    const BmSeg *segs;
    const unsigned short *tile_seg;
    bxmi_ivl *owner;
    int64_t ntp;
    int ngroups, tile_log2;
    size_t search_lds;
    const unsigned *gate;
    bool pad = false;
    bool w8 = false;
    bool wide = false;
    bool big = false;
    bool tot = false;
    unsigned long long *tot_slots = nullptr;
    unsigned *descent = nullptr;
    unsigned *xcd_next = nullptr;
    BmSegChunk par;
    int npar = 0;
    BmParOut par_out;
    int n_segs = 1;
};

template <int THREADS, int ITEMS>
static int bm_launch_tiles(const BmLaunch &L, hipStream_t st, bool sub = false)
{
    constexpr int TILE = THREADS * ITEMS;
    bxmi_ivl *h = L.owner;
    if (sub) {
        if (THREADS != 1024 || L.pad) return fail(BXMI_ESTATE, "bm_launch_tiles: half buckets need a 1024-thread shape on packed runs");
        constexpr int T2 = THREADS == 1024 ? THREADS : 1024;
        constexpr int I2 = TILE / T2;
        const size_t lds = (size_t)TILE * 4 + FX_NBK * 4 + FX_NBK * 2 + 64;
        BXMI_TRY(allow_big_lds((bm_tile_sort_kernel<T2, I2, false, 2>), lds));
        hipLaunchKernelGGL((bm_tile_sort_kernel<T2, I2, false, 2>), dim3((unsigned)L.ntp), dim3(T2), lds, st, L.segs, L.tile_seg,
                           h->bm_recs.as<unsigned>(), h->bm_slots.as<unsigned short>(), h->bm_tbl.as<unsigned short>(), L.gate, (unsigned *)nullptr,
                           h->fx_tbl2.as<unsigned short>(), L.par, L.npar, L.par_out);
        BXMI_LAUNCH_CHECK();
        return BXMI_OK;
    }
    if (L.pad && L.tot) {
        const size_t lds = (size_t)(TILE + 3 * THREADS) * 4 + BM_NB * 4 + BM_NB * 2 + 64;
        BXMI_TRY(allow_big_lds((bm_tile_sort_kernel<THREADS, ITEMS, true, 1, true>), lds));
        hipLaunchKernelGGL((bm_tile_sort_kernel<THREADS, ITEMS, true, 1, true>), dim3((unsigned)L.ntp), dim3(THREADS), lds, st, L.segs, L.tile_seg,
                           h->bm_recs.as<unsigned>(), h->bm_slots.as<unsigned short>(), h->bm_tbl.as<unsigned short>(), L.gate, h->bd_tend.as<unsigned>(),
                           (unsigned short *)nullptr, L.par, L.npar, L.par_out, h->bm_tesc.as<unsigned>());
    } else if (L.pad) {
        const size_t lds = (size_t)(TILE + 3 * THREADS) * 4 + BM_NB * 4 + BM_NB * 2 + 64;
        BXMI_TRY(allow_big_lds((bm_tile_sort_kernel<THREADS, ITEMS, true>), lds));
        hipLaunchKernelGGL((bm_tile_sort_kernel<THREADS, ITEMS, true>), dim3((unsigned)L.ntp), dim3(THREADS), lds, st, L.segs, L.tile_seg,
                           h->bm_recs.as<unsigned>(), h->bm_slots.as<unsigned short>(), h->bm_tbl.as<unsigned short>(), L.gate, h->bd_tend.as<unsigned>(),
                           (unsigned short *)nullptr, L.par, L.npar, L.par_out);
    } else {
        const size_t lds = (size_t)TILE * 4 + BM_NB * 4 + BM_NB * 2 + 64;
        BXMI_TRY(allow_big_lds((bm_tile_sort_kernel<THREADS, ITEMS, false>), lds));
        hipLaunchKernelGGL((bm_tile_sort_kernel<THREADS, ITEMS, false>), dim3((unsigned)L.ntp), dim3(THREADS), lds, st, L.segs, L.tile_seg,
                           h->bm_recs.as<unsigned>(), h->bm_slots.as<unsigned short>(), h->bm_tbl.as<unsigned short>(), L.gate, (unsigned *)nullptr,
                           (unsigned short *)nullptr, L.par, L.npar, L.par_out);
    }
    BXMI_LAUNCH_CHECK();
    return BXMI_OK;
}

template <int THREADS, int ITEMS>
static int bm_launch_unpermute(const BmLaunch &L, unsigned long long *slots, hipStream_t st, const unsigned *cnt = nullptr, unsigned *loff = nullptr,
                               int fx = 0 )
{
    bxmi_ivl *h = L.owner;
    const size_t lds = (size_t)THREADS * ITEMS * sizeof(unsigned);
    if (!cnt) cnt = h->bm_recs.as<unsigned>();
    if (loff && fx == 3) {
        BXMI_TRY(allow_big_lds((bm_unpermute_kernel<THREADS, ITEMS, 3>), lds));
        hipLaunchKernelGGL((bm_unpermute_kernel<THREADS, ITEMS, 3>), dim3((unsigned)L.ntp), dim3(THREADS), lds, st, cnt,
                           h->bm_slots.as<unsigned short>(), L.segs, L.tile_seg, slots, L.gate, loff, h->fx_svq.as<unsigned>(),
                           h->fx_parts.as<unsigned long long>(), h->fx_tile_tot.as<unsigned long long>());
    } else if (loff && fx) {
        BXMI_TRY(allow_big_lds((bm_unpermute_kernel<THREADS, ITEMS, 2>), lds));
        hipLaunchKernelGGL((bm_unpermute_kernel<THREADS, ITEMS, 2>), dim3((unsigned)L.ntp), dim3(THREADS), lds, st, cnt,
                           h->bm_slots.as<unsigned short>(), L.segs, L.tile_seg, slots, L.gate, loff, h->fx_svq.as<unsigned>(),
                           h->fx_parts.as<unsigned long long>(), h->fx_tile_tot.as<unsigned long long>());
    } else {
        BXMI_TRY(allow_big_lds((bm_unpermute_kernel<THREADS, ITEMS>), lds));
        hipLaunchKernelGGL((bm_unpermute_kernel<THREADS, ITEMS>), dim3((unsigned)L.ntp), dim3(THREADS), lds, st, cnt,
                           h->bm_slots.as<unsigned short>(), L.segs, L.tile_seg, slots, L.gate, (unsigned *)nullptr);
    }
    BXMI_LAUNCH_CHECK();
    return BXMI_OK;
}

#ifndef SL_FIND_U
#define SL_FIND_U 2
#endif
template <int LANES>
static int sl_launch_search(const BmLaunch &L, unsigned grid, hipStream_t st, unsigned *out, unsigned *hc = nullptr)
{
    bxmi_ivl *h = L.owner;
    if (out != h->bm_recs.as<unsigned>()) {
        BXMI_TRY(allow_big_lds((sl_search_pipe_kernel<LANES, SL_FIND_U, true>), L.search_lds));
        hipLaunchKernelGGL((sl_search_pipe_kernel<LANES, SL_FIND_U, true>), dim3(grid), dim3(SL_THREADS), L.search_lds, st, L.segs, h->bm_items.as<int4>() + 1,
                           h->bm_items.as<int>(), h->bm_runT.as<unsigned>(), L.ntp, h->bm_recs.as<unsigned>(), out, L.tile_log2, L.gate, hc);
    } else {
        BXMI_TRY(allow_big_lds((sl_search_pipe_kernel<LANES, 2, false>), L.search_lds));
        hipLaunchKernelGGL((sl_search_pipe_kernel<LANES, 2, false>), dim3(grid), dim3(SL_THREADS), L.search_lds, st, L.segs, h->bm_items.as<int4>() + 1,
                           h->bm_items.as<int>(), h->bm_runT.as<unsigned>(), L.ntp, h->bm_recs.as<unsigned>(), (unsigned *)nullptr, L.tile_log2, L.gate);
    }
    BXMI_LAUNCH_CHECK();
    return BXMI_OK;
}

struct BmFindCtx {
    BmLaunch L;
    unsigned sgrid;
    int lanes;
    int variant;
    bool sub = false;
    bool direct = false;
    int f = 0;
    int64_t ntiles = 0;
};

static int sl_launch_search_flat(const BmLaunch &L, unsigned grid, hipStream_t st)
{
    bxmi_ivl *h = L.owner;
    BXMI_TRY(allow_big_lds((sl_search_flat_kernel<4>), L.search_lds));
    hipLaunchKernelGGL((sl_search_flat_kernel<4>), dim3(grid), dim3(SL_THREADS), L.search_lds, st, L.segs, h->bm_items.as<int4>() + 1,
                       h->bm_items.as<int>(), h->bm_runT.as<unsigned>(), L.ntp, h->bm_recs.as<unsigned>(), L.tile_log2, L.gate);
    BXMI_LAUNCH_CHECK();
    return BXMI_OK;
}

template <int FMT, bool QB, int EXP, int DEPTH, bool PIPE, bool PAD = false, bool W8 = false>
static int bd_launch_search_t(const BmLaunch &L, unsigned grid, hipStream_t st)
{
    bxmi_ivl *h = L.owner;
    BXMI_TRY(allow_big_lds((bd_search_kernel<FMT, QB, EXP, DEPTH, PIPE, PAD, W8>), L.search_lds));
    hipLaunchKernelGGL((bd_search_kernel<FMT, QB, EXP, DEPTH, PIPE, PAD, W8>), dim3(grid), dim3(BD_THREADS), L.search_lds, st, L.segs,
                       h->bm_items.as<int4>() + 1, h->bm_items.as<int>(), h->bd_unitT.as<unsigned short>(), L.ntp, h->bm_recs.as<unsigned>(),
                       h->bd_cnt16.as<unsigned short>(), L.tile_log2, L.gate);
    BXMI_LAUNCH_CHECK();
    return BXMI_OK;
}

template <bool W8, bool WIDE, bool TOT = false, bool BIG = false>
static int bw_launch_search(const BmLaunch &L, hipStream_t st)
{
    bxmi_ivl *h = L.owner;
    constexpr int THREADS = WIDE && !BIG ? BD_THREADS / 2 : BD_THREADS;
    constexpr int DEPTH = 3;
    BXMI_TRY(allow_big_lds((bw_search_kernel<W8, DEPTH, WIDE, THREADS, TOT>), L.search_lds));
    hipLaunchKernelGGL((bw_search_kernel<W8, DEPTH, WIDE, THREADS, TOT>), dim3(WIDE && !BIG ? 512 : 256), dim3(THREADS), L.search_lds, st, L.segs, h->bm_items.as<int4>() + 1,
                       h->bm_items.as<int>(), h->bd_unitT.as<unsigned short>(), L.ntp, h->bm_recs.as<unsigned>(), h->bd_cnt16.as<unsigned short>(),
                       L.tile_log2, L.gate, L.xcd_next, L.tot_slots);
    BXMI_LAUNCH_CHECK();
    return BXMI_OK;
}

static int bd_launch_search(const BmLaunch &L, unsigned grid, int fmt , bool blocks, hipStream_t st)
{
    if (fmt == 1) {
        if (!L.pad) return fail(BXMI_ESTATE, "bd_launch_search: cell images on packed runs");
        if (L.tot && L.big) return bw_launch_search<false, true, true, true>(L, st);
        if (L.tot) return L.wide ? bw_launch_search<false, true, true>(L, st) : bw_launch_search<false, false, true>(L, st);
        if (L.big) return L.w8 ? bw_launch_search<true, true, false, true>(L, st) : bw_launch_search<false, true, false, true>(L, st);
        if (L.wide) return L.w8 ? bw_launch_search<true, true>(L, st) : bw_launch_search<false, true>(L, st);
        return L.w8 ? bw_launch_search<true, false>(L, st) : bw_launch_search<false, false>(L, st);
    }
    if (fmt == 2) return bd_launch_search_t<2, false, 0, 2, false>(L, grid, st);
#ifndef BD_EXP_V
#define BD_EXP_V 0
#endif
    if (L.pad) return blocks ? bd_launch_search_t<0, true, BD_EXP_V, 3, true, true>(L, grid, st) : bd_launch_search_t<0, false, BD_EXP_V, 3, true, true>(L, grid, st);
    return blocks ? bd_launch_search_t<0, true, BD_EXP_V, 4, true>(L, grid, st) : bd_launch_search_t<0, false, BD_EXP_V, 4, true>(L, grid, st);
}

template <int THREADS, int ITEMS>
static int bd_launch_unpermute(const BmLaunch &L, unsigned long long *slots, hipStream_t st)
{
    bxmi_ivl *h = L.owner;
    if (L.pad && L.w8) {
        const size_t lds = (size_t)(THREADS * ITEMS + BM_PAD_ROOM);
        BXMI_TRY(allow_big_lds((bd_unpermute_kernel<THREADS, ITEMS, true, true>), lds));
        hipLaunchKernelGGL((bd_unpermute_kernel<THREADS, ITEMS, true, true>), dim3((unsigned)L.ntp), dim3(THREADS), lds, st, h->bd_cnt16.as<unsigned short>(),
                           h->bm_slots.as<unsigned short>(), L.segs, L.tile_seg, slots, L.gate, h->bd_tend.as<unsigned>(),
                           h->bd_fb.as<unsigned long long>(), h->bd_fb_host);
    } else if (L.pad) {
        const size_t lds = (size_t)(THREADS * ITEMS + BM_PAD_ROOM) * sizeof(unsigned short);
        BXMI_TRY(allow_big_lds((bd_unpermute_kernel<THREADS, ITEMS, true>), lds));
        hipLaunchKernelGGL((bd_unpermute_kernel<THREADS, ITEMS, true>), dim3((unsigned)L.ntp), dim3(THREADS), lds, st, h->bd_cnt16.as<unsigned short>(),
                           h->bm_slots.as<unsigned short>(), L.segs, L.tile_seg, slots, L.gate, h->bd_tend.as<unsigned>());
    } else {
        const size_t lds = (size_t)THREADS * ITEMS * sizeof(unsigned short);
        BXMI_TRY(allow_big_lds((bd_unpermute_kernel<THREADS, ITEMS, false>), lds));
        hipLaunchKernelGGL((bd_unpermute_kernel<THREADS, ITEMS, false>), dim3((unsigned)L.ntp), dim3(THREADS), lds, st, h->bd_cnt16.as<unsigned short>(),
                           h->bm_slots.as<unsigned short>(), L.segs, L.tile_seg, slots, L.gate, (const unsigned *)nullptr);
    }
    BXMI_LAUNCH_CHECK();
    return BXMI_OK;
}

static int ensure_feedback(bxmi_ivl *h, hipStream_t st)
{
    if (h->bd_fb_host) return BXMI_OK;
    BXMI_HIP(hipHostMalloc(reinterpret_cast<void **>(&h->bd_fb_host), 64, hipHostMallocDefault));
    memset(h->bd_fb_host, 0, 64);
    BXMI_TRY(h->bd_fb.reserve(64));
    BXMI_HIP(hipMemsetAsync(h->bd_fb.p, 0, 64, st));
    return BXMI_OK;
}

static int bm_count_segments(bxmi_ivl *const *hs, int n, const int32_t *const *qs, const int32_t *const *qe, const int64_t *nq,
                             int32_t *const *counts, int64_t *const *totals_dev, hipStream_t st, int kind, BmFindCtx *fx = nullptr)
{
    if (kind < 2 || kind > 5) return fail(BXMI_EINVAL, "bm_count_segments: no such search stage (%d)", kind);
    const bool wide = kind == 5;
    const bool slices = kind == 2, cells = kind == 4 || wide;
    const bool fxsub = fx && fx->sub;
    const bool slices_flat = slices && !fx && g_opt_sl_flat != 0;
    const bool dense = kind == 3 || cells || slices_flat ;
    bxmi_ivl *h = hs[0];
    int64_t nq_all = 0;
    for (int i = 0; i < n; i++) nq_all += nq[i];
    if (nq_all >= ((int64_t)1 << 31)) return fail(BXMI_EINVAL, "bxmi_ivl_count: more than 2^31 queries in one batch");
    if (n > 4096) return fail(BXMI_EINVAL, "bxmi_ivl_count_multi: more than 4096 indexes in one batch");
    int variant = g_opt_bm_variant >= 0 ? (int)g_opt_bm_variant : (nq_all >= ((int64_t)32 << 20) * (n == 1 ? 1 : 2) ? 2 : 0);
    if (cells && variant == 0 && g_opt_bm_variant < 0) variant = 1;
    if (cells && variant == 0)
        for (int i = 0; i < n; i++)
            if ((wide ? hs[i]->bo_geom : hs[i]->bp_geom).f < 2) variant = 1;
    if (fxsub && (n != 1 || !slices)) return fail(BXMI_ESTATE, "bm_count_segments: the half-bucket order serves find() on one index's slices");
    if (fxsub && variant == 0) variant = 1;
    const int tile_log2 = variant == 2 ? 15 : 14;
    const int64_t tile = (int64_t)1 << tile_log2;
    std::vector<BmSeg> segs((size_t)n);
    int64_t ntp = 0;
    size_t max_stride = 0, sl_lds = 0;
    int64_t sl_run = INT64_MAX;
    bool any_total = false, any_blocks = false;
    for (int i = 0; i < n; i++) {
        BmSeg &sg = segs[(size_t)i];
        any_blocks |= kind == 3 && hs[i]->bd_blocks;
        if (slices) {
            size_t lds = 0;
            int64_t run_len = 0;
            sg.g = sl_geom(hs[i], tile, &lds, &run_len);
            if (lds > sl_lds) sl_lds = lds;
            if (run_len < sl_run) sl_run = run_len;
        } else if (cells) {
            sg.g = wide ? hs[i]->bo_geom : hs[i]->bp_geom;
        } else {
            sg.g = hs[i]->bd_geom;
        }
        sg.qs = qs[i], sg.qe = qe[i], sg.counts = counts[i];
        sg.nq = nq[i];
        sg.tile0 = ntp;
        sg.ntiles = div_up(nq[i], tile);
        sg.dimages = hs[i]->bd_images.as<unsigned char>();
        sg.pimages = wide ? hs[i]->bo_images.as<unsigned char>() : hs[i]->bp_images.as<unsigned char>();
        sg.smeta = slices ? hs[i]->sl_meta.as<int4>() : nullptr;
        sg.ix = index_dev(hs[i]);
        sg.e_sorted = hs[i]->e_sorted.as<int32_t>();
        ntp += div_up(sg.ntiles, BM_GROUP_TILES) * BM_GROUP_TILES;
        sg.tile_end = ntp;
        if ((size_t)sg.g.stride > max_stride) max_stride = (size_t)sg.g.stride;
        any_total |= totals_dev && totals_dev[i];
    }
    if (ntp == 0) return BXMI_OK;
    const int ngroups = (int)(ntp / BM_GROUP_TILES);
    int chunk = dense ? (g_opt_bd_chunk ? (int)g_opt_bd_chunk : (cells || slices_flat ? 2 : 4) * BM_CHUNK) : g_opt_bm_chunk ? (int)g_opt_bm_chunk : BM_CHUNK;
    if (!(dense ? g_opt_bd_chunk : g_opt_bm_chunk) && !(kind == 3 || cells) && nq_all / chunk < 160) {
        const int64_t c = nq_all / 512;
        chunk = (int)(c < 16384 ? 16384 : c);
    }
    int64_t max_items = (int64_t)n * (BM_NB + 2) + 2 * (nq_all / chunk) + 2;
    if (dense) {
        int64_t pad_slots = 0;
        for (int i = 0; i < n; i++) pad_slots += 3 * (int64_t)(BM_NB >> segs[(size_t)i].g.f) * (segs[(size_t)i].tile_end - segs[(size_t)i].tile0);
        max_items = 2 * ((nq_all + pad_slots) / chunk) + 2;
        for (int i = 0; i < n; i++) max_items += (BM_NB >> segs[(size_t)i].g.f) + 2;
    }
    bool pad = kind == 3 || cells;
    for (int i = 0; i < n && pad; i++) pad = (1 << segs[(size_t)i].g.f) >= (variant == 0 ? 4 : 2);
    const int64_t tile_stride = tile + (pad ? BM_PAD_ROOM : 0);
    bool tot_walk = g_opt_tot_walk != 0 && cells && pad && !fx && any_total;
    for (int i = 0; i < n && tot_walk; i++) tot_walk = counts[i] == nullptr;
    if (tot_walk) BXMI_TRY(h->bm_tesc.reserve((size_t)ntp * 4));
    BXMI_TRY(h->bm_recs.reserve((size_t)ntp * tile_stride * 4));
    if (pad) BXMI_TRY(h->bd_tend.reserve((size_t)ntp * 4));
    BXMI_TRY(h->bm_slots.reserve((size_t)ntp * tile * 2));
    BXMI_TRY(h->bm_tbl.reserve((size_t)ntp * BM_NB * 2));
    if (!dense) BXMI_TRY(h->bm_runT.reserve((size_t)ntp * BM_NB * 4));
    if (dense) BXMI_TRY(h->bd_unitT.reserve((size_t)ntp * (BM_NB + 1) * 2));
    BXMI_TRY(h->bm_grpcnt.reserve((size_t)ngroups * BM_NB * 4));
    BXMI_TRY(h->sl_unitcnt.reserve((size_t)ngroups * BM_NB * 4));
    if (dense && !fxsub) BXMI_TRY(h->bd_cnt16.reserve((size_t)ntp * tile_stride * 2));
    BXMI_TRY(h->bm_items.reserve((size_t)(max_items + 2) * sizeof(int4)));
    if (fx) {
        BXMI_TRY(h->sl_cnt.reserve((size_t)ntp * tile * 4));
        BXMI_TRY(h->sl_loff.reserve((size_t)ntp * tile * 4));
    }
    if (fxsub) {
        BXMI_TRY(h->fx_tbl2.reserve((size_t)ntp * FX_NBK * 2));
        BXMI_TRY(h->fx_runT2.reserve((size_t)ntp * FX_NBK * 4));
        BXMI_TRY(h->fx_hc.reserve((size_t)ntp * tile * 4));
        BXMI_TRY(h->fx_svq.reserve((size_t)ntp * tile * 4));
        BXMI_TRY(h->fx_parts.reserve((size_t)ntp * (tile / BM_PART_Q) * 8));
        BXMI_TRY(h->fx_tile_tot.reserve((size_t)ntp * 8));
        BXMI_TRY(h->fx_tile_base.reserve((size_t)(ntp + 2) * 8));
        fx->f = segs[0].g.f;
        fx->ntiles = segs[0].ntiles;
    }
    unsigned *search_out = fx ? h->sl_cnt.as<unsigned>() : h->bm_recs.as<unsigned>();
    const size_t seg_bytes = (size_t)n * sizeof(BmSeg), tot_bytes = (size_t)n * sizeof(void *);
    const size_t tile_off = (seg_bytes + tot_bytes + 15) & ~(size_t)15, par_bytes = tile_off + (size_t)ntp * sizeof(unsigned short);
    BXMI_TRY(h->bm_params.reserve(par_bytes));
    BXMI_TRY(h->p_slots.reserve(((size_t)n * PT_SLOTS + 8) * sizeof(unsigned long long)));
    unsigned long long *slots = h->p_slots.as<unsigned long long>();
    bool multi_sorted = n > 1 && !fx && g_opt_sorted_path && g_opt_sorted_cells != 0 && cells && pad;
    for (int i = 0; i < n && multi_sorted; i++) multi_sorted = nq[i] < ((int64_t)1 << 32) - 8;
    unsigned *unsorted = g_opt_sorted_path && (n == 1 || multi_sorted) && !fx ? reinterpret_cast<unsigned *>(slots + (size_t)n * PT_SLOTS) : nullptr;
    unsigned *descent = nullptr;
    unsigned long long order_seq = 0;
    if (unsorted) {
        BXMI_TRY(ensure_feedback(h, st));
        const unsigned long long seen = reinterpret_cast<volatile unsigned long long *>(h->bd_fb_host)[1];
        if ((seen >> 1) > h->order_seen) {
            h->unsorted_streak = (seen & 1ull) ? h->unsorted_streak + 1 : 0;
            h->order_seen = seen >> 1;
            h->order_skip = h->unsorted_streak >= 2;
        }
        if (h->order_seq == 0 && g_opt_order_skip != 0) {
            hipLaunchKernelGGL(bm_probe_kernel, dim3(1), dim3(256), 0, st, qs[0], nq[0], unsorted);
            unsigned seen_descent = 0;
            BXMI_HIP(hipMemcpyAsync(&seen_descent, unsorted, sizeof(unsigned), hipMemcpyDeviceToHost, st));
            BXMI_HIP(hipStreamSynchronize(st));
            if (seen_descent) h->unsorted_streak = 2, h->order_skip = true;
        }
        order_seq = ++h->order_seq;
        if (h->order_skip && g_opt_order_skip != 0) descent = unsorted, unsorted = nullptr;
    }
    BmLaunch L;
    memset(&L.par, 0, sizeof(L.par));
    const bool fold_params = n <= BM_PAR_CHUNK && !unsorted;
    const int n_zero = n * PT_SLOTS + 8;
    if (fold_params) {
        for (int i = 0; i < n; i++) {
            L.par.seg[i] = segs[(size_t)i];
            L.par.total[i] = totals_dev ? reinterpret_cast<unsigned long long *>(totals_dev[i]) : nullptr;
        }
        L.npar = n;
        L.par_out.segs = h->bm_params.as<BmSeg>();
        L.par_out.totals = reinterpret_cast<unsigned long long **>(h->bm_params.as<unsigned char>() + seg_bytes);
        L.par_out.tile_seg = reinterpret_cast<unsigned short *>(h->bm_params.as<unsigned char>() + tile_off);
        L.par_out.zero_u64 = slots, L.par_out.n_zero = n_zero;
        L.par_out.n_items = h->bm_items.as<int>();
        L.par_out.probe = descent;
        L.par_out.order_host = descent ? h->bd_fb_host + 1 : nullptr, L.par_out.order_seq = order_seq;
    }
    for (int first = 0; first < n && !fold_params; first += BM_PAR_CHUNK) {
        BmSegChunk c;
        memset(&c, 0, sizeof(c));
        const int cnt = n - first < BM_PAR_CHUNK ? n - first : BM_PAR_CHUNK;
        for (int i = 0; i < cnt; i++) {
            c.seg[i] = segs[(size_t)(first + i)];
            c.total[i] = totals_dev ? reinterpret_cast<unsigned long long *>(totals_dev[first + i]) : nullptr;
        }
        hipLaunchKernelGGL(bm_params_kernel, dim3((unsigned)cnt), dim3(256), 0, st, c, first, h->bm_params.as<BmSeg>(),
                           reinterpret_cast<unsigned long long **>(h->bm_params.as<unsigned char>() + seg_bytes),
                           reinterpret_cast<unsigned short *>(h->bm_params.as<unsigned char>() + tile_off), slots, n_zero,
                           h->bm_items.as<int>(), first == 0 ? descent : (unsigned *)nullptr, descent ? h->bd_fb_host + 1 : (unsigned long long *)nullptr,
                           order_seq);
    }
    BXMI_LAUNCH_CHECK();
    unsigned long long *tslots = any_total ? slots : nullptr;
    L.segs = h->bm_params.as<BmSeg>();
    L.tile_seg = reinterpret_cast<const unsigned short *>(h->bm_params.as<unsigned char>() + tile_off);
    L.owner = h;
    L.ntp = ntp, L.ngroups = ngroups, L.tile_log2 = tile_log2;
    L.search_lds = slices ? sl_lds : max_stride * 16;
    if (slices_flat && L.search_lds < 4096) L.search_lds = 4096;
    L.gate = unsorted;
    L.descent = descent;
    L.pad = pad;
    L.wide = wide;
    L.xcd_next = reinterpret_cast<unsigned *>(slots + (size_t)n * PT_SLOTS + 4);
    L.n_segs = n;
    L.tot = tot_walk, L.tot_slots = slots;
    L.big = wide && max_stride * 16 > (size_t)10 * (BD_THREADS / 2) * 16;
    L.w8 = false;
    if (pad && cells && g_opt_bd_w8 != 0 && !tot_walk) {
        BXMI_TRY(ensure_feedback(h, st));
        const unsigned long long wide_counts = *reinterpret_cast<volatile unsigned long long *>(h->bd_fb_host);
        if ((int64_t)wide_counts * 64 > h->w8_queries && wide_counts > 4096) h->w8_off = true;
        bool narrow = true;
        for (int i = 0; i < n; i++) {
            const int64_t span = (int64_t)hs[i]->cmax - (int64_t)hs[i]->geom.cmin + 1;
            narrow = narrow && !hs[i]->w8_off && (int64_t)hs[i]->n * 2048 < span * 128;
            if (wide && hs[i]->bo_state == 2) narrow = false;
        }
        L.w8 = g_opt_bd_w8 > 0 || narrow;
        if (L.w8) h->w8_queries += nq_all;
    }
    if (unsorted) {
        const bool sorted_on_cells = cells && pad && g_opt_sorted_cells != 0 && nq[0] < ((int64_t)1 << 32) - 8;
        if (multi_sorted) {
            const unsigned chunk = (unsigned)(g_opt_bd_chunk ? g_opt_bd_chunk : (wide ? 1 : 2) * BM_CHUNK);
            size_t max_sorted_items = 4;
            for (int i = 0; i < n; i++) max_sorted_items += (size_t)(BM_NB >> segs[(size_t)i].g.f) + 4 + (size_t)(nq[i] / chunk);
            const size_t bounds_bytes = ((size_t)n * BS_BOUNDS_ROW * 4 + 16 + 15) & ~(size_t)15;
            BXMI_TRY(h->bs_plan.reserve(bounds_bytes + (max_sorted_items + 1) * sizeof(int4)));
            unsigned *bounds_all = h->bs_plan.as<unsigned>();
            int *n_sorted = reinterpret_cast<int *>(bounds_all + (size_t)n * BS_BOUNDS_ROW);
            int4 *sorted_items = reinterpret_cast<int4 *>(h->bs_plan.as<unsigned char>() + bounds_bytes);
            BXMI_HIP(hipMemsetAsync(n_sorted, 0, sizeof(int), st));
            hipLaunchKernelGGL(bs_check_multi_kernel, dim3((unsigned)(ntp < 2048 ? ntp : 2048)), dim3(256), 0, st, L.segs, L.tile_seg, ntp, tile_log2, unsorted, bounds_all);
            hipLaunchKernelGGL(bs_plan_multi_kernel, dim3((unsigned)n), dim3(1024), 0, st, L.segs, bounds_all, chunk, sorted_items, n_sorted, unsorted);
            if (wide && L.big) {
                BXMI_TRY(allow_big_lds((bs_walk_kernel<true, BD_THREADS>), L.search_lds));
                hipLaunchKernelGGL((bs_walk_kernel<true, BD_THREADS>), dim3(256), dim3(BD_THREADS), L.search_lds, st, L.segs, sorted_items, n_sorted, tslots,
                                   unsorted, L.xcd_next, h->bd_fb_host + 1, order_seq);
            } else if (wide) {
                BXMI_TRY(allow_big_lds((bs_walk_kernel<true, BD_THREADS / 2>), L.search_lds));
                hipLaunchKernelGGL((bs_walk_kernel<true, BD_THREADS / 2>), dim3(512), dim3(BD_THREADS / 2), L.search_lds, st, L.segs, sorted_items, n_sorted, tslots,
                                   unsorted, L.xcd_next, h->bd_fb_host + 1, order_seq);
            } else {
                BXMI_TRY(allow_big_lds((bs_walk_kernel<false, BD_THREADS>), L.search_lds));
                hipLaunchKernelGGL((bs_walk_kernel<false, BD_THREADS>), dim3(256), dim3(BD_THREADS), L.search_lds, st, L.segs, sorted_items, n_sorted, tslots,
                                   unsorted, L.xcd_next, h->bd_fb_host + 1, order_seq);
            }
            BXMI_LAUNCH_CHECK();
        } else if (sorted_on_cells) {
            const BmGeom &g0 = segs[0].g;
            const int units = BM_NB >> g0.f;
            const unsigned chunk = (unsigned)(g_opt_bd_chunk ? g_opt_bd_chunk : (wide ? 1 : 2) * BM_CHUNK);
            const size_t max_sorted_items = (size_t)units + 4 + (size_t)(nq[0] / chunk);
            BXMI_TRY(h->bs_plan.reserve((size_t)(units + 2) * 4 + 16 + (max_sorted_items + 1) * sizeof(int4)));
            BmBounds B;
            B.bounds = h->bs_plan.as<unsigned>(), B.cmin = g0.cmin, B.ulog = g0.shift + g0.f, B.units = units;
            int *n_sorted = reinterpret_cast<int *>(B.bounds + units + 2);
            int4 *sorted_items = reinterpret_cast<int4 *>(h->bs_plan.as<unsigned char>() + (((size_t)(units + 2) * 4 + 16 + 15) & ~(size_t)15));
            hipLaunchKernelGGL(bm_sorted_check_kernel<true>, dim3(2048), dim3(256), 0, st, qs[0], nq[0], unsorted, B);
            hipLaunchKernelGGL(bs_plan_kernel, dim3(1), dim3(1024), 0, st, B.bounds, units, (unsigned)nq[0], chunk, sorted_items, n_sorted, unsorted);
            if (wide && L.big) {
                BXMI_TRY(allow_big_lds((bs_walk_kernel<true, BD_THREADS>), L.search_lds));
                hipLaunchKernelGGL((bs_walk_kernel<true, BD_THREADS>), dim3(256), dim3(BD_THREADS), L.search_lds, st, L.segs, sorted_items, n_sorted, tslots,
                                   unsorted, L.xcd_next, h->bd_fb_host + 1, order_seq);
            } else if (wide) {
                BXMI_TRY(allow_big_lds((bs_walk_kernel<true, BD_THREADS / 2>), L.search_lds));
                hipLaunchKernelGGL((bs_walk_kernel<true, BD_THREADS / 2>), dim3(512), dim3(BD_THREADS / 2), L.search_lds, st, L.segs, sorted_items, n_sorted, tslots,
                                   unsorted, L.xcd_next, h->bd_fb_host + 1, order_seq);
            } else {
                BXMI_TRY(allow_big_lds((bs_walk_kernel<false, BD_THREADS>), L.search_lds));
                hipLaunchKernelGGL((bs_walk_kernel<false, BD_THREADS>), dim3(256), dim3(BD_THREADS), L.search_lds, st, L.segs, sorted_items, n_sorted, tslots,
                                   unsorted, L.xcd_next, h->bd_fb_host + 1, order_seq);
            }
            BXMI_LAUNCH_CHECK();
        } else {
        hipLaunchKernelGGL(bm_sorted_check_kernel<false>, dim3(2048), dim3(256), 0, st, qs[0], nq[0], unsorted, BmBounds{nullptr, 0, 0, 0});
        TreeDev S = h->treeS.dev, E = h->treeE.dev;
        S.lds_from = S.nlev, S.lds_ints = 0, E.lds_from = E.nlev, E.lds_ints = 0;
        const int64_t nchunks = div_up(nq[0], LC_CHUNK);
        hipLaunchKernelGGL(ivl_local_count_kernel, dim3((unsigned)nchunks), dim3(LC_THREADS), 0, st, S, E, index_dev(h), h->e_sorted.as<int32_t>(),
                           qs[0], qe[0], nq[0], counts[0], tslots, unsorted, (int32_t *)nullptr, h->bd_fb_host + 1, order_seq);
        BXMI_LAUNCH_CHECK();
        }
    }
    if (variant == 2)
        BXMI_TRY((bm_launch_tiles<1024, 32>(L, st, fxsub)));
    else if (variant == 1)
        BXMI_TRY((bm_launch_tiles<1024, 16>(L, st, fxsub)));
    else
        BXMI_TRY((bm_launch_tiles<512, 32>(L, st)));
    if (tot_walk) {
        hipLaunchKernelGGL(bm_escape_totals_kernel, dim3((unsigned)ntp), dim3(1024), 0, st, L.segs, L.tile_seg, h->bm_tesc.as<unsigned>(), ntp, tile_log2, slots,
                           unsorted);
        BXMI_LAUNCH_CHECK();
    }
    if (fxsub) {
        hipLaunchKernelGGL(bm_transpose_kernel<FX_NBK>, dim3((unsigned)ngroups, FX_NBK / 64), dim3(256), 0, st, h->fx_tbl2.as<unsigned short>(), L.segs,
                           L.tile_seg, tile_log2, h->fx_runT2.as<unsigned>(), ntp, (unsigned *)nullptr, unsorted);
        BXMI_LAUNCH_CHECK();
    }
    if (dense) {
        hipLaunchKernelGGL(bd_transpose_kernel, dim3((unsigned)ngroups, BM_NB / 64), dim3(256), 0, st, h->bm_tbl.as<unsigned short>(), L.segs, L.tile_seg,
                           tile_log2, h->bd_unitT.as<unsigned short>(), ntp, h->sl_unitcnt.as<unsigned>(), unsorted,
                           pad ? h->bd_tend.as<unsigned>() : (const unsigned *)nullptr);
        if (n <= BD_PLAN_SEGS)
            hipLaunchKernelGGL(bd_plan_kernel, dim3(1), dim3(1024), 0, st, h->sl_unitcnt.as<unsigned>(), n, L.segs, chunk, h->bm_items.as<int4>() + 1,
                               h->bm_items.as<int>(), unsorted);
        else
            hipLaunchKernelGGL(bm_plan_kernel<2>, dim3(BM_PLAN_BLOCKS), dim3(BM_PLAN_THREADS), 0, st, h->sl_unitcnt.as<unsigned>(), ngroups, L.segs, L.tile_seg,
                               chunk, h->bm_items.as<int4>() + 1, h->bm_items.as<int>(), unsorted);
    } else {
    hipLaunchKernelGGL(bm_transpose_kernel<BM_NB>, dim3((unsigned)ngroups, BM_NB / 64), dim3(256), 0, st, h->bm_tbl.as<unsigned short>(), L.segs, L.tile_seg,
                       tile_log2, h->bm_runT.as<unsigned>(), ntp, h->bm_grpcnt.as<unsigned>(), unsorted);
    hipLaunchKernelGGL(sl_unit_sums_kernel, dim3((unsigned)ngroups), dim3(1024), 0, st, h->bm_grpcnt.as<unsigned>(), L.segs, L.tile_seg,
                       h->sl_unitcnt.as<unsigned>(), unsorted);
    if (n <= BD_PLAN_SEGS)
        hipLaunchKernelGGL(bd_plan_kernel, dim3(1), dim3(1024), 0, st, h->sl_unitcnt.as<unsigned>(), n, L.segs, chunk, h->bm_items.as<int4>() + 1,
                           h->bm_items.as<int>(), unsorted);
    else
        hipLaunchKernelGGL(bm_plan_kernel<2>, dim3(BM_PLAN_BLOCKS), dim3(BM_PLAN_THREADS), 0, st, h->sl_unitcnt.as<unsigned>(), ngroups, L.segs, L.tile_seg,
                           chunk, h->bm_items.as<int4>() + 1, h->bm_items.as<int>(), unsorted);
    }
    BXMI_LAUNCH_CHECK();
    const unsigned sgrid = (unsigned)(div_up(max_items, 8) * 8);
    if (slices_flat)
        BXMI_TRY(bd_launch_search(L, sgrid, 2, false, st));
    else if (slices) {
        int lanes = g_opt_sl_lanes < 0 ? 0 : (g_opt_sl_lanes ? (int)g_opt_sl_lanes : (sl_run >= 96 ? 0 : (sl_run >= 40 ? 64 : 16)));
        if (fx && lanes == 0) lanes = 64;
        if (lanes == 0)
            BXMI_TRY(sl_launch_search_flat(L, sgrid, st));
        else if (lanes == 64)
            BXMI_TRY(sl_launch_search<64>(L, sgrid, st, search_out, fxsub ? h->fx_hc.as<unsigned>() : nullptr));
        else
            BXMI_TRY(sl_launch_search<16>(L, sgrid, st, search_out, fxsub ? h->fx_hc.as<unsigned>() : nullptr));
        if (fx) fx->L = L, fx->sgrid = sgrid, fx->lanes = lanes, fx->variant = variant;
    } else
        BXMI_TRY(bd_launch_search(L, sgrid, cells ? 1 : 0, any_blocks, st));
    unsigned *loff = fx ? h->sl_loff.as<unsigned>() : nullptr;
    if (tot_walk) {
    } else if (dense && !fxsub) {
        if (variant == 2)
            BXMI_TRY((bd_launch_unpermute<1024, 32>(L, tslots, st)));
        else
            BXMI_TRY((bd_launch_unpermute<1024, 16>(L, tslots, st)));
    } else if (variant == 2)
        BXMI_TRY((bm_launch_unpermute<1024, 32>(L, tslots, st, search_out, loff, fxsub ? (fx->direct ? 3 : 2) : 0)));
    else
        BXMI_TRY((bm_launch_unpermute<1024, 16>(L, tslots, st, search_out, loff, fxsub ? (fx->direct ? 3 : 2) : 0)));
    if (any_total) {
        hipLaunchKernelGGL(bm_fold_totals_kernel, dim3((unsigned)n), dim3(64), 0, st, slots,
                           reinterpret_cast<unsigned long long *const *>(h->bm_params.as<unsigned char>() + seg_bytes));
        BXMI_LAUNCH_CHECK();
    }
    return BXMI_OK;
}

static int fx_prepare_index(bxmi_ivl *h, hipStream_t st)
{
    h->fx_state = -1;
    if (h->has_reversed || h->n < 1 || h->geom.shift < 1) return BXMI_OK;
    BXMI_TRY(h->fx_meta2.reserve((size_t)(FX_NBK + 1) * sizeof(int2)));
    BXMI_TRY(h->fx_work.reserve(128));
    hipLaunchKernelGGL(fx_meta_kernel, dim3((FX_NBK + 1 + 255) / 256), dim3(256), 0, st, h->s_ord.as<int32_t>(), (int)h->n, h->geom.cmin, h->geom.shift,
                       h->fx_meta2.as<int2>());
    BXMI_LAUNCH_CHECK();
    h->fx_meta2_host.resize((size_t)FX_NBK + 1);
    BXMI_HIP(hipMemcpyAsync(h->fx_meta2_host.data(), h->fx_meta2.p, (size_t)(FX_NBK + 1) * sizeof(int2), hipMemcpyDeviceToHost, st));
    BXMI_HIP(hipStreamSynchronize(st));
    h->fx_pieces_f = -1;
    h->fx_state = 1;
    return BXMI_OK;
}

static int fx_ensure_pieces(bxmi_ivl *h, int f, hipStream_t st)
{
    if (h->fx_pieces_f == f) return BXMI_OK;
    const std::vector<int2> &m = h->fx_meta2_host;
    std::vector<FxPiece> &out = h->fx_pieces_host;
    out.clear();
    const int per_unit = 1 << (f + 1);
    for (int u0 = 0; u0 < FX_NBK; u0 += per_unit) {
        const int u1 = u0 + per_unit < FX_NBK ? u0 + per_unit : FX_NBK;
        int sb = u0;
        while (sb < u1) {
            const int lo = m[(size_t)sb].x > FX_BACK ? m[(size_t)sb].x - FX_BACK : 0;
            int e = sb + 1;
            while (e < u1 && m[(size_t)e + 1].y - lo <= FX_CAPW) e++;
            FxPiece pc;
            pc.sb0 = sb, pc.sb1 = e;
            pc.whi = m[(size_t)e].y;
            pc.wlo = pc.whi - lo > FX_CAPW ? pc.whi - FX_CAPW : lo;
            out.push_back(pc);
            sb = e;
        }
    }
    BXMI_TRY(h->fx_pieces.reserve(out.size() * sizeof(FxPiece)));
    BXMI_HIP(hipMemcpyAsync(h->fx_pieces.p, out.data(), out.size() * sizeof(FxPiece), hipMemcpyHostToDevice, st));
    h->fx_pieces_f = f;
    return BXMI_OK;
}

static int ivl_find_fx(bxmi_ivl *h, const int32_t *qs, const int32_t *qe, int64_t nq, int64_t *offsets, int32_t *hits, int64_t cap,
                       int64_t *total_host, hipStream_t st)
{
    BXMI_TRY(h->q_cnt.reserve((size_t)(nq + 4) * 4));
    BmFindCtx fx;
    fx.sub = true;
    {
        const double per_q = h->fx_hits_per_q >= 0.0 ? h->fx_hits_per_q : 5.0;
        fx.direct = g_opt_fx_direct < 0 ? per_q * (double)nq * 4.0 <= 400e6 : g_opt_fx_direct != 0;
    }
    int32_t *counts = h->q_cnt.as<int32_t>();
    int64_t *no_total = nullptr;
    BXMI_TRY(bm_count_segments(&h, 1, &qs, &qe, &nq, &counts, &no_total, st, 2, &fx));
    const int64_t ntp = fx.L.ntp;
    hipLaunchKernelGGL(fx_tile_scan_kernel, dim3(1), dim3(1024), 0, st, h->fx_tile_tot.as<unsigned long long>(), fx.ntiles, h->fx_tile_base.as<long long>(),
                       reinterpret_cast<long long *>(offsets) + nq, h->fx_tile_base.as<long long>() + fx.ntiles + 1);
    BXMI_LAUNCH_CHECK();
    BXMI_TRY(fx_ensure_pieces(h, fx.f, st));
    BXMI_HIP(hipMemsetAsync(h->fx_work.p, 0, 64, st));
    if (fx.direct) {
        hipLaunchKernelGGL(fx_offsets_kernel, dim3((unsigned)div_up(nq, 1024)), dim3(256), 0, st, fx.L.segs, h->fx_svq.as<unsigned>(),
                           h->fx_tile_base.as<long long>(), fx.ntiles, fx.L.tile_log2, reinterpret_cast<long long *>(offsets), hits, cap);
        BXMI_LAUNCH_CHECK();
    }
    int64_t total = 0;
    BXMI_HIP(hipMemcpyAsync(&total, offsets + nq, 8, hipMemcpyDeviceToHost, st));
    BXMI_HIP(hipStreamSynchronize(st));
    if (total_host) *total_host = total;
    h->fx_hits_per_q = (double)total / (double)nq;
    if (total >= ((int64_t)1 << 31)) {
        long long max_tile = 0;
        BXMI_HIP(hipMemcpyAsync(&max_tile, h->fx_tile_base.as<long long>() + fx.ntiles + 1, 8, hipMemcpyDeviceToHost, st));
        BXMI_HIP(hipStreamSynchronize(st));
        if (max_tile >= ((long long)1 << 31)) return ivl_find_partitioned(h, qs, qe, nq, offsets, hits, cap, total_host, st);
    }
    if (total > cap && fx.direct) return fail(BXMI_ERANGE, "bxmi_ivl_find: %lld hits need a larger buffer than cap=%lld", (long long)total, (long long)cap);
    if (total > cap) {
        BXMI_TRY((device_scan<int32_t, long long, OpSum, false>(h->q_cnt.as<int32_t>(), reinterpret_cast<long long *>(offsets), nq, 0ll,
                                                               reinterpret_cast<long long *>(offsets) + nq, h->scan_scratch, st)));
        BXMI_HIP(hipStreamSynchronize(st));
        return fail(BXMI_ERANGE, "bxmi_ivl_find: %lld hits need a larger buffer than cap=%lld", (long long)total, (long long)cap);
    }
    if (total == 0) {
        if (!fx.direct) BXMI_HIP(hipMemsetAsync(offsets, 0, (size_t)(nq + 1) * 8, st));
        return BXMI_OK;
    }
    if (!fx.direct) BXMI_TRY(h->sl_hits.reserve((size_t)(total + 16) * 4));
    BXMI_TRY(sl_ensure_eid(h, st));
    const int npieces = (int)h->fx_pieces_host.size();
    int64_t nchunks = div_up(2048, npieces);
    if (nchunks > div_up(fx.ntiles, 64)) nchunks = div_up(fx.ntiles, 64);
    if (nchunks < 1) nchunks = 1;
    const int64_t tiles_per_chunk = div_up(div_up(fx.ntiles, nchunks), 64) * 64;
    nchunks = div_up(fx.ntiles, tiles_per_chunk);
    BXMI_TRY(allow_big_lds(fx_fill_kernel, FX_LDS_BYTES));
    hipLaunchKernelGGL(fx_fill_kernel, dim3((unsigned)device_props().cus), dim3(FX_THREADS), FX_LDS_BYTES, st, fx.L.segs, h->fx_pieces.as<FxPiece>(), npieces,
                       (int)nchunks, (int)tiles_per_chunk, h->fx_runT2.as<unsigned>(), ntp, h->bm_recs.as<unsigned>(), h->fx_hc.as<unsigned>(),
                       h->sl_cnt.as<unsigned>(), h->sl_loff.as<unsigned>(), h->fx_tile_base.as<long long>(), h->sl_eid.as<int2>() + SL_WALK,
                       h->fx_meta2.as<int2>(), fx.direct ? hits : h->sl_hits.as<int32_t>(), fx.L.tile_log2, h->fx_work.as<unsigned>(), h->fx_work.as<int32_t>() + 16);
    BXMI_LAUNCH_CHECK();
    if (fx.direct) return BXMI_OK;
    const unsigned cgrid = (unsigned)(div_up(ntp, 8) * 8 * (((int64_t)1 << fx.L.tile_log2) / BM_PART_Q));
    {
        auto launch = [&](auto kern) {
            hipLaunchKernelGGL(kern, dim3(cgrid), dim3(BM_PART_Q / 2), 0, st, fx.L.segs, h->fx_svq.as<unsigned>(), h->fx_tile_base.as<long long>(),
                               h->fx_parts.as<unsigned long long>(), h->sl_hits.as<int32_t>(), reinterpret_cast<long long *>(offsets), hits, ntp);
        };
        if (fx.variant == 2) launch(fx_hits_copy2_kernel<32768, 2>); else launch(fx_hits_copy2_kernel<16384, 2>);
    }
    BXMI_LAUNCH_CHECK();
    return BXMI_OK;
}

static int bm_choose_stage(bxmi_ivl *h, hipStream_t st, int *kind, int64_t nq)
{
    *kind = 0;
    if (h->has_reversed || h->n < 4096) return BXMI_OK;
    int64_t span = (int64_t)h->cmax - (int64_t)h->geom.cmin;
    if (span < 0) span = 0;
    if ((g_opt_sparse > 0 || (g_opt_sparse < 0 && g_opt_flat < 0 && g_opt_dense < 1 && g_opt_slice < 1)) &&
        (g_opt_bo_cell_log2 || bo_cell_log2_for(span + 1, h->n))) {
        if (h->bo_state == 0) BXMI_TRY(bo_prepare_index(h, st));
        if (h->bo_state == 1) {
            const int64_t units = (span >> (h->bo_geom.shift + h->bo_geom.f)) + 1;
            if (g_opt_sparse > 0 || nq >= units * g_opt_bo_min_per_unit) {
                *kind = 5;
                return BXMI_OK;
            }
        }
    }
    auto try_clumped = [&]() -> int {
        if (h->bo_state == 0 || (h->bo_state == -1 && !h->bo_tried_clumped)) {
            h->bo_tried_clumped = true;
            BXMI_TRY(bo_prepare_index(h, st, true));
        }
        if (h->bo_state == 2) *kind = 5;
        return BXMI_OK;
    };
    if (g_opt_clumped > 0 && g_opt_dense != 1) {
        BXMI_TRY(try_clumped());
        if (*kind) return BXMI_OK;
    }
    const bool slices_first = g_opt_dense != 1 && g_opt_flat != 1 && (g_opt_slice == 1 || (g_opt_slice < 0 && (span / h->n >= 64 || h->geom.shift > BD_MAX_SHIFT)));
    if (slices_first) {
        if (h->sl_state == 0) BXMI_TRY(sl_prepare_index(h, st));
        if (h->sl_state == 1) {
// ... 1039 lines not shown
```

Before: 152,800.

## Fold end-rank offset into image metadata and move escape handling to per-tile flags

The dense bitmap image now stores end ranks shifted by one position and folds the start/end rank difference into cell metadata, so counting a record no longer adds a bias or increments the offset. The sort kernel writes a per-tile escape flag whenever padding is on, and a new non-escape search variant drops the per-record escape check and clamp, leaving unpermute to recompute escaped records in flagged tiles. Rank computation is rewritten with inline v_bfm/v_mad_u32_u24 and a cell-address helper to shorten the inner instruction sequence. This adds complexity and an overflow check on the folded metadata, and flagged tiles pay extra record recomputation.

```diff
diff --git a/bx-python_amd/csrc/count_bitmap.hpp b/bx-python_amd/csrc/count_bitmap.hpp
--- a/bx-python_amd/csrc/count_bitmap.hpp
+++ b/bx-python_amd/csrc/count_bitmap.hpp
@@ -395,10 +395,8 @@
             const unsigned r0 = bm_record_of(vs[j].x, ve[j].x, g), r1 = bm_record_of(vs[j].y, ve[j].y, g);
             const unsigned r2 = bm_record_of(vs[j].z, ve[j].z, g), r3 = bm_record_of(vs[j].w, ve[j].w, g);
             staged[s0] = r0, staged[s1] = r1, staged[s2] = r2, staged[s3] = r3;
-            if (TOT)
-                esc |= r0 == BM_REC_ESC || r1 == BM_REC_ESC || r2 == BM_REC_ESC || r3 == BM_REC_ESC;
-            else
-                l4[j * THREADS + threadIdx.x] = make_uint2(s0 | (s1 << 16), s2 | (s3 << 16));
+            if (PAD) esc |= r0 == BM_REC_ESC || r1 == BM_REC_ESC || r2 == BM_REC_ESC || r3 == BM_REC_ESC;
+            if (!TOT) l4[j * THREADS + threadIdx.x] = make_uint2(s0 | (s1 << 16), s2 | (s3 << 16));
         }
     } else {
 #pragma unroll
@@ -408,14 +406,12 @@
                 const unsigned s = toff[br[j] >> 16] + (br[j] & 0xffffu);
                 const unsigned r = bm_record_of(qs[base + k], qe[base + k], g);
                 staged[s] = r;
-                if (TOT)
-                    esc |= r == BM_REC_ESC;
-                else
-                    slots[base + k] = (unsigned short)s;
-            }
-        }
-    }
-    if (TOT) {
+                if (PAD) esc |= r == BM_REC_ESC;
+                if (!TOT) slots[base + k] = (unsigned short)s;
+            }
+        }
+    }
+    if (PAD) {
         const int any = __syncthreads_or(esc ? 1 : 0);
         if (threadIdx.x == 0) tesc[tile] = (unsigned)(any != 0);
     } else {
diff --git a/bx-python_amd/csrc/count_dense.hpp b/bx-python_amd/csrc/count_dense.hpp
--- a/bx-python_amd/csrc/count_dense.hpp
+++ b/bx-python_amd/csrc/count_dense.hpp
@@ -234,14 +234,15 @@
     const int ulog = g.shift + g.f;
     const BpLayout L = bp_layout(ulog);
     const long long UW = 1ll << ulog;
-    const long long lo = (long long)g.cmin + (long long)unit * UW;
+    const long long lo_unit = (long long)g.cmin + (long long)unit * UW;
     unsigned char *__restrict__ img = images + (size_t)unit * L.bytes;
     unsigned hard = 0;
     int r0s[2];
     for (int arr = 0; arr < 2; arr++) {
         const int32_t *__restrict__ A = arr == 0 ? e_sorted : s_ord;
         const int nc = arr == 0 ? L.nce : L.ncs;
-        const long long span = arr == 0 ? UW + 1 : UW + BP_MARGIN;
+        const long long lo = lo_unit + (arr == 0 ? 1 : 0);
+        const long long span = arr == 0 ? UW : UW + BP_MARGIN;
         unsigned *bm = reinterpret_cast<unsigned *>(dyn);
         int *first = dyn + nc;
         unsigned *dmask = reinterpret_cast<unsigned *>(dyn + 2 * nc), *dcnt = reinterpret_cast<unsigned *>(dyn + 3 * nc);
@@ -249,6 +250,7 @@
         __syncthreads();
         const int r0 = s_r[0], r1 = s_r[1], ns = r1 - r0;
         r0s[arr] = r0;
+        const int fold = arr == 0 ? 0 : r0s[1] - r0s[0];
         for (int c = threadIdx.x; c < nc; c += BD_THREADS) {
             bm[c] = 0u;
             first[c] = ns;
@@ -282,7 +284,7 @@
         uint2 *out = reinterpret_cast<uint2 *>(img + (arr == 0 ? L.cellsE : L.cellsS));
         for (int c = c_lo; c < c_hi; c++) {
             const int base = first[c] < above ? first[c] : above;
-            unsigned meta = (unsigned)base & 0xFFFFFu;
+            unsigned meta = (unsigned)(base + fold) & 0xFFFFFu;
             unsigned word = bm[c];
             if (dcnt[c] > 0u) {
                 if (__popc(dmask[c]) == 1 && dcnt[c] < (unsigned)BM_HARD)
@@ -309,14 +311,14 @@
             }
             out[c] = make_uint2(word, meta);
         }
-        if (threadIdx.x == 0 && ns >= (1 << 20)) atomicAdd(&stats[1], 1u);
+        if (threadIdx.x == 0 && (fold < 0 || (long long)ns + fold >= (1 << 20))) atomicAdd(&stats[1], 1u);
         __syncthreads();
     }
     if (hard) atomicAdd(&stats[0], hard);
     if (threadIdx.x == 0) {
         unsigned *hdr = reinterpret_cast<unsigned *>(img + L.hdr);
         hdr[0] = (unsigned)r0s[0], hdr[1] = (unsigned)r0s[1];
-        hdr[2] = (unsigned)(unsigned long long)lo, hdr[3] = (unsigned)((unsigned long long)lo >> 32);
+        hdr[2] = (unsigned)(unsigned long long)lo_unit, hdr[3] = (unsigned)((unsigned long long)lo_unit >> 32);
     }
 }
 
@@ -578,6 +580,7 @@
     lds_u32_p qbE, qbS;
     int bias;
     unsigned off_mask;
+    unsigned cell_bits;
     lds_cell_p cE, cS;
     lds_u16_p img16;
     lds_u8_p img8;
@@ -590,41 +593,52 @@
     BmGeom g;
 };
 
+__device__ __forceinline__ unsigned bp_rank_of(unsigned bits, unsigned meta, unsigned rel)
+{
+    unsigned low;
+    asm("v_bfm_b32 %0, %1, 0" : "=v"(low) : "v"(rel));
+    unsigned r = (unsigned)__popc(bits & low) + (meta & 0xFFFFFu);
+    const unsigned x = meta >> 20;
+    asm("v_mad_u32_u24 %0, %1, %2, %0" : "+v"(r) : "v"(__builtin_amdgcn_ubfe(low, x, 1u)), "v"(x >> 5));
+    return r;
+}
+
+__device__ __forceinline__ lds_cell_p bp_cell_at(lds_cell_p cells, unsigned cell)
+{
+    unsigned at;
+    asm("v_lshl_add_u32 %0, %1, 3, %2" : "=v"(at) : "v"(cell), "s"((unsigned)(__UINTPTR_TYPE__)cells));
+    return (lds_cell_p)(__UINTPTR_TYPE__)at;
+}
+
 __device__ __forceinline__ unsigned bp_cell_rank(lds_cell_p cells, unsigned rel, unsigned &meta_out)
 {
     const unsigned long long c = cells[rel >> 5];
-    const unsigned bits = (unsigned)c, meta = (unsigned)(c >> 32);
-    meta_out = meta;
-    const unsigned below = ~(0xFFFFFFFFu << (rel & 31u));
-    const unsigned dup = __builtin_amdgcn_ubfe(below, (meta >> 20) & 31u, 1u);
-    return (meta & 0xFFFFFu) + (unsigned)__popc(bits & below) + (meta >> 25) * dup;
-}
-
-__device__ __forceinline__ int bp_hard_rank(const BdImage &I, lds_cell_p cells, unsigned rel, const int32_t *__restrict__ a, int slice_lo)
+    meta_out = (unsigned)(c >> 32);
+    return bp_rank_of((unsigned)c, (unsigned)(c >> 32), rel);
+}
+
+__device__ __forceinline__ int bp_hard_rank(const BdImage &I, lds_cell_p cells, unsigned rel, const int32_t *__restrict__ a, long long lo)
 {
     const bd_v2u c = __builtin_bit_cast(bd_v2u, cells[rel >> 5]);
     if (c.x != BP_NO_TABLE) return (int)(c.y & 0xFFFFFu) + (int)I.img16[(c.x >> 1) + (rel & 31u)];
-    return bm_hard_rank(cells, rel, a, slice_lo, I.lo);
-}
-
-template <bool RAW = false>
+    return bm_hard_rank(cells, rel, a, I.eLo, lo);
+}
+
 __device__ __forceinline__ unsigned bp_count_record(const BdImage &I, unsigned rec)
 {
     const unsigned off = rec & I.off_mask, len = rec >> BP_RSHIFT;
-    const unsigned relE = off + 1u, relS = off + len;
+    const unsigned relE = off, relS = off + len;
     unsigned mE, mS;
     const unsigned rE = bp_cell_rank(I.cE, relE, mE);
     const unsigned rS = bp_cell_rank(I.cS, relS, mS);
-    unsigned c = (unsigned)I.bias + (rS - rE);
+    unsigned c = rS - rE;
     if ((mE > mS ? mE : mS) >= ((unsigned)BM_HARD << 25)) {
         int hE = (int)rE, hS = (int)rS;
-        if ((mE >> 25) == (unsigned)BM_HARD) hE = bp_hard_rank(I, I.cE, relE, I.e_sorted, I.eLo);
-        if ((mS >> 25) == (unsigned)BM_HARD) hS = bp_hard_rank(I, I.cS, relS, I.s_ord, I.sLo);
-        c = (unsigned)(I.bias + (hS - hE));
-    }
-    if (RAW) return rec == BM_REC_ESC ? 0u : c;
-    c = c < 0xFFFFu ? c : 0xFFFFu;
-    return rec == BM_REC_ESC ? 0xFFFFu : c;
+        if ((mE >> 25) == (unsigned)BM_HARD) hE = bp_hard_rank(I, I.cE, relE, I.e_sorted, I.lo + 1);
+        if ((mS >> 25) == (unsigned)BM_HARD) hS = bp_hard_rank(I, I.cS, relS, I.s_ord, I.lo);
+        c = (unsigned)(hS - hE);
+    }
+    return c;
 }
 
 template <bool QB>
@@ -978,7 +992,7 @@
     return v;
 }
 
-template <bool RAW = false>
+template <bool RAW = false, bool ESCT = true>
 __device__ __forceinline__ void bp_count_slot(const BdImage &I, bd_v4u v, unsigned (&c)[4])
 {
     const unsigned rec[4] = {v.x, v.y, v.z, v.w};
@@ -986,30 +1000,25 @@
     unsigned long long cellE[4], cellS[4];
 #pragma unroll
     for (int j = 0; j < 4; j++) {
-        const unsigned off = rec[j] & I.off_mask;
-        relE[j] = off + 1u, relS[j] = off + (rec[j] >> BP_RSHIFT);
-        cellE[j] = I.cE[relE[j] >> 5];
-        cellS[j] = I.cS[relS[j] >> 5];
+        relE[j] = rec[j] & I.off_mask, relS[j] = relE[j] + (rec[j] >> BP_RSHIFT);
+        cellE[j] = *bp_cell_at(I.cE, __builtin_amdgcn_ubfe(rec[j], 5u, I.cell_bits));
+        cellS[j] = *bp_cell_at(I.cS, relS[j] >> 5);
     }
     unsigned worst = 0u;
 #pragma unroll
     for (int j = 0; j < 4; j++) {
         const bd_v2u ce = __builtin_bit_cast(bd_v2u, cellE[j]), cs = __builtin_bit_cast(bd_v2u, cellS[j]);
-        const unsigned bE = ce.x, mE = ce.y, bS = cs.x, mS = cs.y;
-        const unsigned geE = 0xFFFFFFFFu << (relE[j] & 31u), geS = 0xFFFFFFFFu << (relS[j] & 31u);
-        const unsigned rE = (mE & 0xFFFFFu) + (unsigned)__popc(bE & ~geE) + (mE >> 25) * __builtin_amdgcn_ubfe(~geE, (mE >> 20) & 31u, 1u);
-        const unsigned rS = (mS & 0xFFFFFu) + (unsigned)__popc(bS & ~geS) + (mS >> 25) * __builtin_amdgcn_ubfe(~geS, (mS >> 20) & 31u, 1u);
-        c[j] = (unsigned)I.bias + (rS - rE);
-        const unsigned m = mE > mS ? mE : mS;
-        worst = worst > m ? worst : m;
+        c[j] = bp_rank_of(cs.x, cs.y, relS[j]) - bp_rank_of(ce.x, ce.y, relE[j]);
+        worst = max(max(worst, ce.y), cs.y);
     }
     if (worst >= ((unsigned)BM_HARD << 25)) {
 #pragma unroll
         for (int j = 0; j < 4; j++) {
             const unsigned mE = __builtin_bit_cast(bd_v2u, cellE[j]).y, mS = __builtin_bit_cast(bd_v2u, cellS[j]).y;
-            if ((mE > mS ? mE : mS) >= ((unsigned)BM_HARD << 25)) c[j] = bp_count_record<RAW>(I, rec[j]);
-        }
-    }
+            if ((mE > mS ? mE : mS) >= ((unsigned)BM_HARD << 25)) c[j] = bp_count_record(I, rec[j]);
+        }
+    }
+    if (!RAW && !ESCT) return;
 #pragma unroll
     for (int j = 0; j < 4; j++) {
         if (RAW) {
@@ -1157,13 +1166,16 @@
         for (int j = 0; j < 4; j++) b[j] = c[j] < 0xFFu ? c[j] : 0xFFu;
         reinterpret_cast<unsigned *>(out)[idx4] = b[0] | (b[1] << 8) | (b[2] << 16) | (b[3] << 24);
     } else {
+        unsigned b[4];
+#pragma unroll
+        for (int j = 0; j < 4; j++) b[j] = c[j] < 0xFFFFu ? c[j] : 0xFFFFu;
         bd_v2u o;
-        o.x = c[0] | (c[1] << 16), o.y = c[2] | (c[3] << 16);
+        o.x = b[0] | (b[1] << 16), o.y = b[2] | (b[3] << 16);
         reinterpret_cast<bd_v2u *>(out)[idx4] = o;
     }
 }
 
-template <bool W8, int DEPTH, bool WIDE = false, int THREADS = BD_THREADS, bool TOT = false>
+template <bool W8, int DEPTH, bool WIDE = false, int THREADS = BD_THREADS, bool TOT = false, bool ESCT = true>
 __global__ __launch_bounds__(THREADS) void bw_search_kernel(const BmSeg *__restrict__ segs, const int4 *__restrict__ items,
                                                                const int *__restrict__ n_items, const unsigned short *__restrict__ unitT, int64_t ntp,
                                                                const unsigned *__restrict__ recs ,
@@ -1260,6 +1272,7 @@
             I.lo = (long long)((unsigned long long)hdr[2] | ((unsigned long long)hdr[3] << 32));
             I.s_ord = sg.ix.s_ord, I.e_sorted = sg.e_sorted;
             I.off_mask = (1u << (g.shift + g.f)) - 1u;
+            I.cell_bits = (unsigned)(g.shift + g.f) - 5u;
             I.img8 = (lds_u8_p)base;
             I.rshift = g.rshift, I.cell_log2 = cell_log2, I.cell_mask = (1u << cell_log2) - 1u;
         }
@@ -1366,7 +1379,7 @@
                         else if (WIDE)
                             bo_count_slot<TOT, THREADS == BD_THREADS>(I, rv, c);
                         else
-                            bp_count_slot<TOT>(I, rv, c);
+                            bp_count_slot<TOT, ESCT>(I, rv, c);
                         if (TOT) acc += (unsigned long long)c[0] + c[1] + c[2] + c[3];
                         else if (!(BW_EXP & 2) || (c[0] & c[1] & c[2] & c[3]) == 0x12345u) bw_store_slot<W8>(out, ring_idx[d], c);
                         else bd_dummy_store(reinterpret_cast<unsigned short *>(nobody));
@@ -1392,7 +1405,7 @@
                     if (WIDE)
                         bo_count_slot<TOT, THREADS == BD_THREADS>(I, reinterpret_cast<const bd_v4u *>(recs)[q0 + q], c);
                     else
-                        bp_count_slot<TOT>(I, reinterpret_cast<const bd_v4u *>(recs)[q0 + q], c);
+                        bp_count_slot<TOT, ESCT>(I, reinterpret_cast<const bd_v4u *>(recs)[q0 + q], c);
                     if (TOT) acc += (unsigned long long)c[0] + c[1] + c[2] + c[3];
                     else bw_store_slot<W8>(out, q0 + q, c);
                 }
@@ -1556,6 +1569,7 @@
             I.lo = (long long)((unsigned long long)hdr[2] | ((unsigned long long)hdr[3] << 32));
             I.s_ord = sg.ix.s_ord, I.e_sorted = sg.e_sorted;
             I.off_mask = (1u << (g.shift + g.f)) - 1u;
+            I.cell_bits = (unsigned)(g.shift + g.f) - 5u;
             I.img8 = (lds_u8_p)base;
             I.rshift = g.rshift, I.cell_log2 = cell_log2, I.cell_mask = (1u << cell_log2) - 1u;
         }
@@ -1629,7 +1643,8 @@
                                                   unsigned long long *__restrict__ total_slots ,
                                                   const unsigned *__restrict__ gate, const unsigned *__restrict__ tend,
                                                   unsigned long long *__restrict__ fb_dev ,
-                                                  unsigned long long *__restrict__ fb_host )
+                                                  unsigned long long *__restrict__ fb_host ,
+                                                  const unsigned *__restrict__ tesc )
 {
     constexpr int TILE = THREADS * ITEMS;
     constexpr int STRIDE = PAD ? TILE + BM_PAD_ROOM : TILE;
@@ -1656,6 +1671,7 @@
     const int64_t nq = sg.nq - ltile * TILE;
     const int n = (int)(nq < TILE ? nq : TILE);
     constexpr unsigned ESC = W8 ? 0xFFu : 0xFFFFu;
+    const bool flagged = tesc != nullptr && tesc[tile] != 0u;
     if (PAD) {
         const int n8 = W8 ? ((int)tend[tile] + 15) >> 4 : ((int)tend[tile] + 7) >> 3;
         const int4 *src = reinterpret_cast<const int4 *>(cnt);
@@ -1725,11 +1741,11 @@
             } else {
                 c[0] = vals[sl[j].x & 0xffffu], c[1] = vals[sl[j].x >> 16], c[2] = vals[sl[j].y & 0xffffu], c[3] = vals[sl[j].y >> 16];
             }
-            if (c[0] == ESC || c[1] == ESC || c[2] == ESC || c[3] == ESC) {
+            if (c[0] == ESC || c[1] == ESC || c[2] == ESC || c[3] == ESC || flagged) {
                 const int64_t k0 = 4 * (int64_t)(j * THREADS + threadIdx.x);
 #pragma unroll
                 for (int u = 0; u < 4; u++)
-                    if (c[u] == ESC) {
+                    if (c[u] == ESC || (flagged && bm_record_of(qs_arr[k0 + u], qe_arr[k0 + u], g) == BM_REC_ESC)) {
                         c[u] = (unsigned)bm_escape_count(ix, e_sorted, g, qs_arr[k0 + u], qe_arr[k0 + u]);
                         wide++;
                     }
@@ -1740,7 +1756,7 @@
     } else {
         for (int k = threadIdx.x; k < n; k += THREADS) {
             unsigned c = W8 ? (unsigned)vals8[slots[k]] : (unsigned)vals[slots[k]];
-            if (c == ESC) {
+            if (c == ESC || (flagged && bm_record_of(qs_arr[k], qe_arr[k], g) == BM_REC_ESC)) {
                 c = (unsigned)bm_escape_count(ix, e_sorted, g, qs_arr[k], qe_arr[k]);
                 wide++;
             }
@@ -1765,9 +1781,9 @@
                                                                const BmSeg *__restrict__ segs, const unsigned short *__restrict__ tile_seg,
                                                                unsigned long long *__restrict__ total_slots, const unsigned *__restrict__ gate,
                                                                const unsigned *__restrict__ tend = nullptr, unsigned long long *__restrict__ fb_dev = nullptr,
-                                                               unsigned long long *__restrict__ fb_host = nullptr)
-{
-    bd_unpermute_tile<THREADS, ITEMS, PAD, W8>(cnt, slots, segs, tile_seg, total_slots, gate, tend, fb_dev, fb_host);
-}
-
-}
+                                                               unsigned long long *__restrict__ fb_host = nullptr, const unsigned *__restrict__ tesc = nullptr)
+{
+    bd_unpermute_tile<THREADS, ITEMS, PAD, W8>(cnt, slots, segs, tile_seg, total_slots, gate, tend, fb_dev, fb_host, tesc);
+}
+
+}
diff --git a/bx-python_amd/csrc/intervals.hip b/bx-python_amd/csrc/intervals.hip
--- a/bx-python_amd/csrc/intervals.hip
+++ b/bx-python_amd/csrc/intervals.hip
@@ -580,6 +580,7 @@
     bool w8 = false;
     bool wide = false;
     bool big = false;
+    bool noesc = false;
     bool tot = false;
     unsigned long long *tot_slots = nullptr;
     unsigned *descent = nullptr;
@@ -618,7 +619,7 @@
         BXMI_TRY(allow_big_lds((bm_tile_sort_kernel<THREADS, ITEMS, true>), lds));
         hipLaunchKernelGGL((bm_tile_sort_kernel<THREADS, ITEMS, true>), dim3((unsigned)L.ntp), dim3(THREADS), lds, st, L.segs, L.tile_seg,
                            h->bm_recs.as<unsigned>(), h->bm_slots.as<unsigned short>(), h->bm_tbl.as<unsigned short>(), L.gate, h->bd_tend.as<unsigned>(),
-                           (unsigned short *)nullptr, L.par, L.npar, L.par_out);
+                           (unsigned short *)nullptr, L.par, L.npar, L.par_out, h->bm_tesc.as<unsigned>());
     } else {
         const size_t lds = (size_t)TILE * 4 + BM_NB * 4 + BM_NB * 2 + 64;
         BXMI_TRY(allow_big_lds((bm_tile_sort_kernel<THREADS, ITEMS, false>), lds));
@@ -709,14 +710,14 @@
     return BXMI_OK;
 }
 
-template <bool W8, bool WIDE, bool TOT = false, bool BIG = false>
+template <bool W8, bool WIDE, bool TOT = false, bool BIG = false, bool ESCT = true>
 static int bw_launch_search(const BmLaunch &L, hipStream_t st)
 {
     bxmi_ivl *h = L.owner;
     constexpr int THREADS = WIDE && !BIG ? BD_THREADS / 2 : BD_THREADS;
     constexpr int DEPTH = 3;
-    BXMI_TRY(allow_big_lds((bw_search_kernel<W8, DEPTH, WIDE, THREADS, TOT>), L.search_lds));
-    hipLaunchKernelGGL((bw_search_kernel<W8, DEPTH, WIDE, THREADS, TOT>), dim3(WIDE && !BIG ? 512 : 256), dim3(THREADS), L.search_lds, st, L.segs, h->bm_items.as<int4>() + 1,
+    BXMI_TRY(allow_big_lds((bw_search_kernel<W8, DEPTH, WIDE, THREADS, TOT, ESCT>), L.search_lds));
+    hipLaunchKernelGGL((bw_search_kernel<W8, DEPTH, WIDE, THREADS, TOT, ESCT>), dim3(WIDE && !BIG ? 512 : 256), dim3(THREADS), L.search_lds, st, L.segs, h->bm_items.as<int4>() + 1,
                        h->bm_items.as<int>(), h->bd_unitT.as<unsigned short>(), L.ntp, h->bm_recs.as<unsigned>(), h->bd_cnt16.as<unsigned short>(),
                        L.tile_log2, L.gate, L.xcd_next, L.tot_slots);
     BXMI_LAUNCH_CHECK();
@@ -731,6 +732,7 @@
         if (L.tot) return L.wide ? bw_launch_search<false, true, true>(L, st) : bw_launch_search<false, false, true>(L, st);
         if (L.big) return L.w8 ? bw_launch_search<true, true, false, true>(L, st) : bw_launch_search<false, true, false, true>(L, st);
         if (L.wide) return L.w8 ? bw_launch_search<true, true>(L, st) : bw_launch_search<false, true>(L, st);
+        if (L.noesc) return L.w8 ? bw_launch_search<true, false, false, false, false>(L, st) : bw_launch_search<false, false, false, false, false>(L, st);
         return L.w8 ? bw_launch_search<true, false>(L, st) : bw_launch_search<false, false>(L, st);
     }
     if (fmt == 2) return bd_launch_search_t<2, false, 0, 2, false>(L, grid, st);
@@ -750,12 +752,13 @@
         BXMI_TRY(allow_big_lds((bd_unpermute_kernel<THREADS, ITEMS, true, true>), lds));
         hipLaunchKernelGGL((bd_unpermute_kernel<THREADS, ITEMS, true, true>), dim3((unsigned)L.ntp), dim3(THREADS), lds, st, h->bd_cnt16.as<unsigned short>(),
                            h->bm_slots.as<unsigned short>(), L.segs, L.tile_seg, slots, L.gate, h->bd_tend.as<unsigned>(),
-                           h->bd_fb.as<unsigned long long>(), h->bd_fb_host);
+                           h->bd_fb.as<unsigned long long>(), h->bd_fb_host, L.noesc ? h->bm_tesc.as<unsigned>() : (const unsigned *)nullptr);
     } else if (L.pad) {
         const size_t lds = (size_t)(THREADS * ITEMS + BM_PAD_ROOM) * sizeof(unsigned short);
         BXMI_TRY(allow_big_lds((bd_unpermute_kernel<THREADS, ITEMS, true>), lds));
         hipLaunchKernelGGL((bd_unpermute_kernel<THREADS, ITEMS, true>), dim3((unsigned)L.ntp), dim3(THREADS), lds, st, h->bd_cnt16.as<unsigned short>(),
-                           h->bm_slots.as<unsigned short>(), L.segs, L.tile_seg, slots, L.gate, h->bd_tend.as<unsigned>());
+                           h->bm_slots.as<unsigned short>(), L.segs, L.tile_seg, slots, L.gate, h->bd_tend.as<unsigned>(), (unsigned long long *)nullptr,
+                           (unsigned long long *)nullptr, L.noesc ? h->bm_tesc.as<unsigned>() : (const unsigned *)nullptr);
     } else {
         const size_t lds = (size_t)THREADS * ITEMS * sizeof(unsigned short);
         BXMI_TRY(allow_big_lds((bd_unpermute_kernel<THREADS, ITEMS, false>), lds));
@@ -851,7 +854,9 @@
     const int64_t tile_stride = tile + (pad ? BM_PAD_ROOM : 0);
     bool tot_walk = g_opt_tot_walk != 0 && cells && pad && !fx && any_total;
     for (int i = 0; i < n && tot_walk; i++) tot_walk = counts[i] == nullptr;
-    if (tot_walk) BXMI_TRY(h->bm_tesc.reserve((size_t)ntp * 4));
+    if (pad) BXMI_TRY(h->bm_tesc.reserve((size_t)ntp * 4));
+    bool noesc = kind == 4 && pad && !tot_walk && !fx;
+    for (int i = 0; i < n && noesc; i++) noesc = counts[i] != nullptr;
     BXMI_TRY(h->bm_recs.reserve((size_t)ntp * tile_stride * 4));
     if (pad) BXMI_TRY(h->bd_tend.reserve((size_t)ntp * 4));
     BXMI_TRY(h->bm_slots.reserve((size_t)ntp * tile * 2));
@@ -953,6 +958,7 @@
     L.xcd_next = reinterpret_cast<unsigned *>(slots + (size_t)n * PT_SLOTS + 4);
     L.n_segs = n;
     L.tot = tot_walk, L.tot_slots = slots;
+    L.noesc = noesc;
     L.big = wide && max_stride * 16 > (size_t)10 * (BD_THREADS / 2) * 16;
     L.w8 = false;
     if (pad && cells && g_opt_bd_w8 != 0 && !tot_walk) {
```

Result: slower. 150,000 (-1.8%).
